# skeskinen/bert.cpp

Measured on AMD Instinct MI355X. Metric: sentences/sec (seq_len=128), higher is better.
Workload: dtype f16; 1 GPU; all-MiniLM-L6-v2 f16, batch=256 seq_len=128; per_gpu_batch=256, global_batch=256, seq_len=128, weights=f16, parallelism=dp1 (replicated weights, sharded sentences)

## Files before the change

bert.cpp_amd/csrc/engine.h:

```cpp
#pragma once
#include <hip/hip_runtime.h>

#include <cstdint>
#include <functional>
#include <memory>
#include <string>
#include <vector>

#include "kernels.h"
#include "model_file.h"
#include "options.h"
#include "profiler.h"
#include "weights.h"

namespace bert_hip {

class Engine {
public:
    static Engine *create(const ModelFile &mf, int device, std::string &err);
    ~Engine();

    int eval_packed_host(const int32_t *tokens, const int32_t *cu_seqlens, int n_sentences, float *embeddings,
                         std::string &err, float *d_embeddings = nullptr, int pool_mode = -1);
    int eval_packed_device(const int32_t *d_tokens, const int32_t *d_cu, int n_sentences, int n_tokens, int max_len,
                           float *d_out, hipStream_t stream, float *d_hidden, std::string &err,
                           const int2 *d_windows = nullptr, int n_windows = 0, int window_slots = 0,
                           int pool_mode = -1,
                           void *d_token_rows = nullptr, int token_flags = 0);
    int eval_packed_tokens_host(const int32_t *tokens, const int32_t *cu_seqlens, int n_sentences, int flags, float *rows, float *embeddings,
                                std::string &err);
    static void build_windows(const int32_t *cu_seqlens, int n_sentences, std::vector<int2> &windows, int slots);
    int eval_hidden(const int32_t *tokens, int n_tokens, float *hidden, float *embedding, std::string &err);

    int eval_packed_grouped_host(const int32_t *tokens, const int32_t *cu_seqlens, int n_sentences, const int32_t *group_cu, int n_groups,
                                 float *embeddings, float *d_embeddings, std::string &err, const float *h_raw_rows = nullptr, int pool_mode = -1);
    int eval_packed_grouped_device(const int32_t *d_tokens, const int32_t *d_cu, int n_sentences, int n_tokens, int max_len,
                                   const int32_t *d_group_cu, int n_groups, float *d_out, hipStream_t stream, std::string &err);

    bool reserve(int n_tokens, int n_sentences, std::string &err);
    int check(std::string &err);
    void set_option(const std::string &key, const std::string &value);
    void profile_enable(bool on) { prof_.enable(on); }
    std::string profile_report();
    void timed_launch(const char *name, double flops, hipStream_t s, const std::function<void()> &f);

    struct StreamOp { hipStream_t s = nullptr; hipEvent_t busy = nullptr; bool capturing = false; };
    bool op_begin(hipStream_t s, hipEvent_t busy, StreamOp &op, std::string &err);
    bool op_end(const StreamOp &op, std::string &err);

    const HParams &hparams() const { return hp_; }
    const EngineOptions &options() const { return opt_; }
    int device() const { return device_; }
    hipStream_t stream() const { return stream_; }

private:
    Engine() = default;
    bool ensure_workspace(int t_pad, int n_sentences, std::string &err);

    enum class Route { F32, LATENCY, ONE_LAUNCH, FOLDED, LAYERED };
    enum class Family { GEMM256, MFMA, NAIVE, F32 };
    struct LayerPlan {
        bool qkv2 = false;
        bool tail = false;
        bool planes = false;
        Family qkv = Family::NAIVE, o = Family::NAIVE, ffi = Family::NAIVE, ffo = Family::NAIVE;
    };
    struct Plan {
        const int32_t *tokens, *cu;
        int B, T, max_len, t_pad, slots, pool_mode;
        float *out, *hidden;
        void *token_rows;
        hipStream_t s;
        const int2 *windows;
        int n_windows;
        Route route = Route::LAYERED;
        bool build_windows = false;
        const int *n_windows_dev = nullptr;
        std::vector<LayerPlan> layers;
    };
    Plan plan(const int32_t *d_tokens, const int32_t *d_cu, int B, int T, int max_len, float *d_out, hipStream_t s, float *d_hidden,
              const int2 *d_windows, int n_windows, int slots, int pool_mode, void *d_token_rows = nullptr) const;
    bool forward_f32(const Plan &p, std::string &err);
    void forward_latency(const Plan &p);
    void forward_one_launch(const Plan &p);
    bool forward_folded(const Plan &p, std::string &err);
    bool forward_layers(const Plan &p, std::string &err);
    bool gemm(const Plan &p, const char *name, Family f, const GemmWeightStore &W, const void *A, const float *bias, const void *resid, void *C,
              int epi, std::string &err, const GemmLnFold *ln = nullptr);
    void attention(const Plan &p);
    void tap(const Plan &p, int idx);
    int group_pool(const int32_t *d_cu, int n_sentences, const int32_t *d_group_cu, int n_groups, float *d_out, int pool_mode, const StreamOp &op, std::string &err);
    template <class F> void timed(const char *name, double flops, hipStream_t s, F &&f) { prof_.timed(name, flops, s, f); }

    HParams hp_;
    int device_ = 0;
    EngineOptions opt_;
    std::unique_ptr<ModelWeights> w_;
    LaunchProfiler prof_;

    DevBuf x_, qkv_, ctx_, y_, ff_, v32_, d_tokens_, d_cu_, d_out_, d_hidden_, status_, windows_;
    DevBuf tok_in_, tok_rows_;
    DevBuf raw_rows_, group_in_, group_out_;
    DevBuf ln_stats1_, ln_stats2_, ln_rows1_, ln_rows2_;
    hipStream_t stream_ = nullptr;
    hipEvent_t busy_ = nullptr;
    struct HostSlot {
        char *h_in = nullptr, *d_in_host = nullptr;
        float *h_out = nullptr, *d_out_host = nullptr;
        size_t h_in_cap = 0, h_out_cap = 0;
        DevBuf d_in, d_out;
        hipEvent_t done = nullptr;
    } slot_[2];
};

}
```

bert.cpp_amd/csrc/engine.hip:

```cpp
#include "engine.h"

#include <algorithm>
#include <cstdio>
#include <cstdlib>
#include <chrono>
#include <cstring>
#include <system_error>
#include <thread>

namespace bert_hip {

Engine *Engine::create(const ModelFile &mf, int device, std::string &err) {
    int ndev = 0;
    if (hipGetDeviceCount(&ndev) != hipSuccess || ndev <= 0) {
        err = "no HIP device available (this library needs an AMD GPU; there is no CPU fallback)";
        return nullptr;
    }
    if (device < 0 || device >= ndev) { err = "HIP device ordinal " + std::to_string(device) + " out of range"; return nullptr; }
    std::unique_ptr<Engine> e(new Engine);
    e->hp_ = mf.hp;
    e->device_ = device;
    if (hipSetDevice(e->device_) != hipSuccess) { err = "hipSetDevice failed"; return nullptr; }
    hipDeviceProp_t prop;
    if (hipGetDeviceProperties(&prop, e->device_) != hipSuccess) { err = "hipGetDeviceProperties failed"; return nullptr; }
    if (strncmp(prop.gcnArchName, "gfx950", 6) != 0) {
        err = std::string("unsupported GPU architecture '") + prop.gcnArchName + "' (kernels are built for gfx950 / MI355X only)";
        return nullptr;
    }
    e->opt_ = EngineOptions::from_env(mf.hp);
    LoadOptions lo;
    lo.naive = e->opt_.gemm_naive; lo.expand_q4 = e->opt_.q4_expand; lo.ln_fold = e->opt_.ln_fold;
    e->w_ = ModelWeights::load(mf, lo, err);
    if (!e->w_ || !e->status_.alloc(16, err)) return nullptr;
    if (hipStreamCreateWithFlags(&e->stream_, hipStreamNonBlocking) != hipSuccess) { err = "hipStreamCreate failed"; return nullptr; }
    if (hipEventCreateWithFlags(&e->busy_, hipEventDisableTiming) != hipSuccess) { err = "hipEventCreate failed"; return nullptr; }
    return e.release();
}

Engine::~Engine() {
    (void)hipSetDevice(device_);
    (void)hipDeviceSynchronize();
    for (auto &sl : slot_) {
        if (sl.h_in) (void)hipHostFree(sl.h_in);
        if (sl.h_out) (void)hipHostFree(sl.h_out);
        if (sl.done) (void)hipEventDestroy(sl.done);
    }
    if (busy_) (void)hipEventDestroy(busy_);
    if (stream_) (void)hipStreamDestroy(stream_);
}

bool Engine::reserve(int n_tokens, int n_sentences, std::string &err) {
    HIP_OK(hipSetDevice(device_), err, false);
    if (n_tokens <= 0 || n_sentences <= 0) return true;
    return ensure_workspace((n_tokens + 255) / 256 * 256, n_sentences, err);
}

int Engine::check(std::string &err) {
    HIP_OK(hipSetDevice(device_), err, -1);
    HIP_OK(hipDeviceSynchronize(), err, -1);
    int st = 0;
    HIP_OK(hipMemcpy(&st, status_.p, sizeof(int), hipMemcpyDeviceToHost), err, -1);
    if (st) HIP_OK(hipMemset(status_.p, 0, sizeof(int)), err, -1);
    return st;
}

void Engine::set_option(const std::string &key, const std::string &value) {
    if (key == "profile_replay") { prof_.set_replay(value); return; }
    (void)hipSetDevice(device_);
    if (!test_poison_option(key, ctx_, y_, {&x_, &qkv_, &ctx_, &y_, &ff_, &v32_, &ln_stats1_, &ln_stats2_, &ln_rows1_, &ln_rows2_, &d_hidden_})) opt_.set(key, value, w_->naive_images(), w_->fold_images);
}

bool Engine::ensure_workspace(int t_pad, int n_sentences, std::string &err) {
    const size_t H = hp_.n_embd, I = hp_.n_intermediate, tp = (size_t)t_pad;
    const size_t es = w_->f32_file ? 4 : 2;
    return x_.ensure(tp * H * es, err) && qkv_.ensure(tp * 3 * H * es, err) && ctx_.ensure(tp * H * es, err) &&
           y_.ensure(tp * H * es, err) && ff_.ensure(tp * I * es, err) && v32_.ensure((size_t)std::max(128, std::min(t_pad, (opt_.latency_tokens + 255) / 256 * 256)) * H * 4, err) &&
           d_out_.ensure((size_t)n_sentences * H * 4, err) &&
           windows_.ensure((size_t)n_sentences * sizeof(int2), err) &&
           (!(H > 384 && H % 256 == 0) || (ln_stats1_.ensure(tp * (2 * H / 256) * 8, err) && ln_stats2_.ensure(tp * (2 * H / 256) * 8, err) &&
                                           ln_rows1_.ensure(tp * 16, err) && ln_rows2_.ensure(tp * 16, err)));
}

void Engine::timed_launch(const char *name, double flops, hipStream_t s, const std::function<void()> &f) { timed(name, flops, s, f); }

bool Engine::op_begin(hipStream_t s, hipEvent_t busy, StreamOp &op, std::string &err) {
    hipStreamCaptureStatus st = hipStreamCaptureStatusNone;
    HIP_OK(hipStreamIsCapturing(s, &st), err, false);
    op.s = s; op.busy = busy; op.capturing = st == hipStreamCaptureStatusActive;
    if (!op.capturing) {
        if (busy) HIP_OK(hipStreamWaitEvent(s, busy, 0), err, false);
        return true;
    }
    if (prof_.enabled()) { err = "the stream is capturing while the context profiles: a timed launch cannot be captured (bert_hip_profile_enable(ctx, 0) first)"; return false; }
    return true;
}

bool Engine::op_end(const StreamOp &op, std::string &err) {
    if (!op.capturing && op.busy) HIP_OK(hipEventRecord(op.busy, op.s), err, false);
    return true;
}

std::string Engine::profile_report() {
    (void)hipSetDevice(device_);
    (void)hipDeviceSynchronize();
    return prof_.report();
}

void Engine::build_windows(const int32_t *cu, int B, std::vector<int2> &windows, int slot) {
    windows.clear();
    int first = 0, fill = 0;
    for (int b = 0; b < B; ++b) {
        const int n = cu[b + 1] - cu[b];
        if (b > first && fill + n > 128) {
            windows.push_back(make_int2(first, b - first));
            first = b; fill = 0;
        }
        fill = (fill + n + slot - 1) & ~(slot - 1);
    }
    if (B > first) windows.push_back(make_int2(first, B - first));
}

int Engine::eval_packed_device(const int32_t *d_tokens, const int32_t *d_cu, int B, int T, int max_len, float *d_out,
                               hipStream_t s, float *d_hidden, std::string &err, const int2 *d_windows, int n_windows, int slots_in,
                               int pool_mode_in, void *d_token_rows, int token_flags) {
    if (B <= 0 || T <= 0) return 0;
    const int slots = slots_in ? slots_in : window_slots();
    const int pool_mode = pool_mode_in >= 0 ? pool_mode_in : opt_.pool_mode();
    HIP_OK(hipSetDevice(device_), err, -1);
    StreamOp op;
    if (!op_begin(s, busy_, op, err)) return -1;
    if (!ensure_workspace((T + 255) / 256 * 256, B, err)) return -1;
    prof_.begin_pass();
    if (!d_out) d_out = d_out_.as<float>();
    const Plan p = plan(d_tokens, d_cu, B, T, max_len, d_out, s, d_hidden, d_windows, n_windows, slots, pool_mode, d_token_rows);
    bool ok = true;
    if (p.route == Route::F32) ok = forward_f32(p, err);
    else {
        const int H = hp_.n_embd;
        timed("embed_ln", 0.0, s, [&] { launch_embed_ln(w_->word_emb.p, w_->type_emb.p, w_->pos_emb.p, w_->table_type, w_->ln_e_w.as<float>(), w_->ln_e_b.as<float>(),
                                                        d_tokens, d_cu, B, T, H, hp_.n_vocab, max_len, x_.as<half_t>(), s); });
        tap(p, 0);
        if (p.build_windows)
            timed("build_windows", 0.0, s, [&] { launch_build_windows(d_cu, B, windows_.as<int2>(), status_.as<int>() + 1, slots, s); });
        switch (p.route) {
            case Route::LATENCY: forward_latency(p); break;
            case Route::ONE_LAUNCH: forward_one_launch(p); break;
            case Route::FOLDED: ok = forward_folded(p, err); break;
            default: ok = forward_layers(p, err); break;
        }
        if (ok && p.route != Route::ONE_LAUNCH)
            timed("pool_normalize", 2.0 * T * H, s, [&] { launch_pool_normalize(x_.as<half_t>(), d_cu, B, H, max_len, status_.as<int>(), d_out, p.pool_mode, s); });
    }
    if (!ok) return -1;
    if (d_token_rows)
        timed("token_rows", 0.0, s, [&] { launch_token_rows(x_.p, p.route == Route::F32, T, hp_.n_embd, d_cu, B, max_len, token_flags, d_token_rows, s); });
    HIP_OK(hipGetLastError(), err, -1);
    return op_end(op, err) ? 0 : -1;
}

Engine::Plan Engine::plan(const int32_t *d_tokens, const int32_t *d_cu, int B, int T, int max_len, float *d_out, hipStream_t s,
                          float *d_hidden, const int2 *d_windows, int n_windows, int slots, int pool_mode, void *d_token_rows) const {
    Plan p{d_tokens, d_cu, B, T, max_len, (T + 255) / 256 * 256, slots, pool_mode, d_out, d_hidden, d_token_rows, s, d_windows, n_windows};
    if (w_->f32_file && opt_.f32_exact) { p.route = Route::F32; return p; }
    const int H = hp_.n_embd, nh = hp_.n_head, dh = H / nh, Lz = hp_.n_layer;
    auto family = [&](const GemmWeightStore &W) {
        if (W.mfma_ok && opt_.gemm256 && !opt_.gemm_naive && gemm256_supported(W.w, p.t_pad)) return Family::GEMM256;
        return W.mfma_ok && (!opt_.gemm_naive || !W.w.naive16) ? Family::MFMA : Family::NAIVE;
    };
    p.layers.resize(Lz);
    bool qkv2_shape0 = false, one_launch = true, fold = opt_.ln_fold && H > 384 && H % 256 == 0 && ln_rows2_.p;
    for (int il = 0; il < Lz; ++il) {
        const LayerWeights &L = w_->layers[il];
        LayerPlan &lp = p.layers[il];
        const bool qkv2_shape = qkv_attention2_supported(L.qkv.w, nh, dh, max_len), tail_shape = layer_tail_supported(L.o.w, L.ffi.w, L.ffo.w);
        if (il == 0) qkv2_shape0 = qkv2_shape;
        lp.qkv2 = opt_.qkv2 && !opt_.gemm_naive && !opt_.attn_naive && L.qkv.mfma_ok && qkv2_shape;
        lp.tail = opt_.tail && !opt_.gemm_naive && L.o.mfma_ok && L.ffi.mfma_ok && L.ffo.mfma_ok && tail_shape;
        lp.planes = L.qkv_q4.w.qs && family(L.qkv_q4) == Family::GEMM256;
        lp.qkv = family(lp.planes ? L.qkv_q4 : L.qkv), lp.o = family(L.o), lp.ffi = family(L.ffi), lp.ffo = family(L.ffo);
        one_launch = one_launch && L.qkv.mfma_ok && L.o.mfma_ok && L.ffi.mfma_ok && L.ffo.mfma_ok && L.ffi.w.w16p && L.ffo.w.w16p &&
                     model_kernel_supported(L.qkv.w, L.o.w, L.ffi.w, L.ffo.w, Lz, nh, dh, max_len);
        fold = fold && L.fold_ok && (il ? family(L.qkv_fold) : lp.qkv) == Family::GEMM256 && lp.o == Family::GEMM256 &&
               family(L.ffi_fold) == Family::GEMM256 && lp.ffo == Family::GEMM256 && !(opt_.qkv2 && qkv2_shape) && !(opt_.tail && tail_shape);
    }
    if (d_hidden) one_launch = fold = false;
    if (d_token_rows) one_launch = false;
    const bool fused_windows = p.layers[0].qkv2, latency_call = opt_.latency && T <= opt_.latency_tokens;
    one_launch = one_launch && fused_windows && opt_.one_launch && opt_.tail && !latency_call;
    const bool full_windows = (long long)B * 128 == T;
    const int spw = qkv_attention2_sentences_per_window(max_len, slots);
    if (!d_windows && fused_windows &&
        (4ll * ((B + spw - 1) / spw) * 128 > 5 * ((long long)T + (long long)(slots / 2) * B) || (one_launch && opt_.one_launch == 2 && spw > 1 && !full_windows))) {
        p.build_windows = true;
        p.windows = windows_.as<int2>();
        p.n_windows_dev = status_.as<int>() + 1;
        p.n_windows = qkv_attention2_max_windows(B, T, slots);
    }
    bool one_launch_pays = full_windows || opt_.one_launch == 2;
    if (!one_launch_pays && !p.build_windows) one_launch_pays = (d_windows || spw == 1) && 100ll * T >= 95ll * 128 * (d_windows ? n_windows : B);
    const LayerWeights &L0 = w_->layers[0];
    const bool skinny = latency_call && opt_.tail && opt_.qkv2 && !opt_.gemm_naive && !opt_.attn_naive && max_len <= 128 && (dh == 32 || dh == 64) &&
                        skinny_layer_supported(L0.qkv.w, L0.o.w, L0.ffi.w, L0.ffo.w) && qkv2_shape0;
    p.route = skinny ? Route::LATENCY : one_launch && one_launch_pays ? Route::ONE_LAUNCH : fold ? Route::FOLDED : Route::LAYERED;
    return p;
}

bool Engine::gemm(const Plan &p, const char *name, Family f, const GemmWeightStore &W, const void *A, const float *bias, const void *resid,
                  void *C, int epi, std::string &err, const GemmLnFold *ln) {
    static const char *const kernel[] = {"gemm256", "gemm_mfma", "gemm_naive", "gemm_f32"};
    prof_.count_family(std::string("family:") + kernel[(int)f] + (f == Family::GEMM256 || f == Family::MFMA ? (W.w.type == GW_F16 ? "_f16" : "_q4") : ""));
    const half_t *a = (const half_t *)A, *r = (const half_t *)resid;
    bool ok = !(ln && ln->flags) || f == Family::GEMM256;
    if (ok)
        timed(name, 2.0 * p.T * W.w.N * W.w.K, p.s, [&] {
            if (f == Family::F32) launch_f32_gemm((const float *)A, W.w.w32, bias, (const float *)resid, (float *)C, p.T, W.w.N, W.w.K, epi, p.s);
            else if (f == Family::GEMM256) ok = launch_gemm256(W.w, a, bias, r, (half_t *)C, p.t_pad, epi, p.s, ln);
            else if (f == Family::MFMA) launch_gemm_mfma(W.w, a, bias, r, (half_t *)C, p.t_pad, epi, p.s);
            else launch_gemm_naive(W.w, a, bias, r, (half_t *)C, p.T, epi, p.s);
        });
    if (!ok) err = std::string(name) + ": no " + kernel[(int)f] + " kernel for LayerNorm-folding flags " + std::to_string(ln->flags) + ", epilogue " + std::to_string(epi);
    return ok;
}

void Engine::attention(const Plan &p) {
    const int H = hp_.n_embd, nh = hp_.n_head, dh = H / nh;
    half_t *qkv = qkv_.as<half_t>(), *ctx = ctx_.as<half_t>();
    timed("attention", 4.0 * p.T * p.max_len * H, p.s, [&] {
        if (opt_.attn_naive || !launch_attention_mfma(qkv, p.cu, p.B, nh, dh, p.max_len, ctx, p.s)) launch_attention_naive(qkv, p.cu, p.B, nh, dh, p.max_len, ctx, p.s);
    });
}

void Engine::tap(const Plan &p, int idx) {
    const size_t n = (size_t)p.T * hp_.n_embd;
    if (p.hidden && p.route == Route::F32) (void)hipMemcpyAsync(p.hidden + idx * n, x_.p, n * 4, hipMemcpyDeviceToDevice, p.s);
    else if (p.hidden) launch_f16_to_f32(x_.as<half_t>(), p.hidden + idx * n, n, p.s);
}

void Engine::forward_latency(const Plan &p) {
    const int H = hp_.n_embd, I = hp_.n_intermediate, tb = (p.T + 31) / 32, Lz = hp_.n_layer;
    half_t *x = x_.as<half_t>(), *qkv = qkv_.as<half_t>(), *ctx = ctx_.as<half_t>(), *y = y_.as<half_t>(), *ff = ff_.as<half_t>();
    float *v32 = v32_.as<float>();
    for (int il = 0; il < Lz; ++il) {
        const LayerWeights &L = w_->layers[il];
        const LayerWeights *P = il ? &w_->layers[il - 1] : nullptr;
        timed("skinny_qkv", 2.0 * p.T * 3 * H * H, p.s, [&] {
            launch_skinny_gemm(0, L.qkv.w, x, P ? v32 : nullptr, P ? P->ln_out_w.as<float>() : nullptr, P ? P->ln_out_b.as<float>() : nullptr,
                               x, L.qkv_b.as<float>(), nullptr, qkv, nullptr, tb, p.s);
        });
        attention(p);
        timed("skinny_proj", 2.0 * p.T * H * H, p.s, [&] {
            launch_skinny_gemm(1, L.o.w, ctx, nullptr, nullptr, nullptr, nullptr, L.o_b.as<float>(), x, nullptr, v32, tb, p.s);
        });
        timed("skinny_ffn_up", 2.0 * p.T * H * I, p.s, [&] {
            launch_skinny_gemm(2, L.ffi.w, nullptr, v32, L.ln_att_w.as<float>(), L.ln_att_b.as<float>(), y, L.ffi_b.as<float>(), nullptr, ff, nullptr, tb, p.s);
        });
        timed("skinny_ffn_down", 2.0 * p.T * H * I, p.s, [&] {
            launch_skinny_gemm(3, L.ffo.w, ff, nullptr, nullptr, nullptr, nullptr, L.ffo_b.as<float>(), y, nullptr, v32, tb, p.s);
        });
        if (il + 1 == Lz || p.hidden)
            timed("skinny_layernorm", 0.0, p.s, [&] { launch_skinny_layernorm(v32, L.ln_out_w.as<float>(), L.ln_out_b.as<float>(), x, tb, H, p.s); });
        tap(p, il + 1);
    }
}

void Engine::forward_one_launch(const Plan &p) {
    const int H = hp_.n_embd, I = hp_.n_intermediate;
    ModelLayerWeights mw[MODEL_MAX_LAYERS];
    for (int il = 0; il < hp_.n_layer; ++il) {
        const LayerWeights &L = w_->layers[il];
        mw[il] = {&L.qkv.w, &L.o.w, &L.ffi.w, &L.ffo.w, L.qkv_b.as<float>(), L.o_b.as<float>(), L.ln_att_w.as<float>(), L.ln_att_b.as<float>(),
                  L.ffi_b.as<float>(), L.ffo_b.as<float>(), L.ln_out_w.as<float>(), L.ln_out_b.as<float>()};
    }
    timed("model_kernel", hp_.n_layer * (2.0 * p.T * 3 * H * H + 4.0 * p.T * p.max_len * H + 2.0 * p.T * H * H + 4.0 * p.T * H * I), p.s, [&] {
        launch_model_kernel(mw, hp_.n_layer, x_.as<half_t>(), ctx_.as<half_t>(), y_.as<half_t>(), p.cu, p.B, p.T, p.windows, p.n_windows, p.n_windows_dev, hp_.n_head,
                            p.out, p.max_len, status_.as<int>(), p.pool_mode, p.slots, p.s);
    });
}

bool Engine::forward_folded(const Plan &p, std::string &err) {
    const int H = hp_.n_embd, P = 2 * H / 256;
    const Family G = Family::GEMM256;
    half_t *x = x_.as<half_t>(), *qkv = qkv_.as<half_t>(), *ctx = ctx_.as<half_t>(), *y = y_.as<half_t>(), *ff = ff_.as<half_t>();
    float2 *st1 = ln_stats1_.as<float2>(), *st2 = ln_stats2_.as<float2>();
    float4 *rows1 = ln_rows1_.as<float4>(), *rows2 = ln_rows2_.as<float4>();
    for (int il = 0; il < hp_.n_layer; ++il) {
        const LayerWeights &L = w_->layers[il];
        GemmLnFold ln;
        if (il == 0) {
            if (!gemm(p, "gemm_qkv", G, p.layers[0].planes ? L.qkv_q4 : L.qkv, x, L.qkv_b.as<float>(), nullptr, qkv, EPI_BIAS, err)) return false;
        } else {
            ln.flags = GemmLnFold::IN; ln.rows_in = rows2; ln.waug = L.qkv_waug.as<half_t>();
            if (!gemm(p, "gemm_qkv", G, L.qkv_fold, x, nullptr, nullptr, qkv, EPI_BIAS, err, &ln)) return false;
        }
        attention(p);
        ln = GemmLnFold(); ln.flags = GemmLnFold::STATS | (il ? GemmLnFold::RES : 0); ln.stats = st1; ln.rows_res = rows2; ln.gb = L.o_gb.as<unsigned>();
        if (!gemm(p, "gemm_attn_out", G, L.o, ctx, L.o_b.as<float>(), x, y, EPI_BIAS_RESID, err, &ln)) return false;
        timed("ln_rows_finalize", 0.0, p.s, [&] { launch_ln_rows_finalize(st1, P, p.t_pad, H, rows1, p.s); });
        ln = GemmLnFold(); ln.flags = GemmLnFold::IN; ln.rows_in = rows1; ln.waug = L.ffi_waug.as<half_t>();
        if (!gemm(p, "gemm_ffn_up", G, L.ffi_fold, y, nullptr, nullptr, ff, EPI_BIAS_GELU, err, &ln)) return false;
        ln = GemmLnFold(); ln.flags = GemmLnFold::STATS | GemmLnFold::RES; ln.stats = st2; ln.rows_res = rows1; ln.gb = L.ffo_gb.as<unsigned>();
        if (!gemm(p, "gemm_ffn_down", G, L.ffo, ff, L.ffo_b.as<float>(), y, x, EPI_BIAS_RESID, err, &ln)) return false;
        timed("ln_rows_finalize", 0.0, p.s, [&] { launch_ln_rows_finalize(st2, P, p.t_pad, H, rows2, p.s); });
        if (il + 1 == hp_.n_layer)
            timed("layernorm", 0.0, p.s, [&] { launch_layernorm(x, L.ln_out_w.as<float>(), L.ln_out_b.as<float>(), p.T, H, p.s); });
    }
    return true;
}

bool Engine::forward_layers(const Plan &p, std::string &err) {
    const int H = hp_.n_embd, I = hp_.n_intermediate;
    half_t *x = x_.as<half_t>(), *qkv = qkv_.as<half_t>(), *ctx = ctx_.as<half_t>(), *y = y_.as<half_t>(), *ff = ff_.as<half_t>();
    for (int il = 0; il < hp_.n_layer; ++il) {
        const LayerWeights &L = w_->layers[il];
        const LayerPlan &lp = p.layers[il];
        if (lp.qkv2) {
            timed("qkv_attention2", 2.0 * p.T * L.qkv.w.N * L.qkv.w.K + 4.0 * p.T * p.max_len * H, p.s, [&] {
                launch_qkv_attention2(L.qkv.w, x, L.qkv_b.as<float>(), p.cu, p.B, p.windows, p.n_windows, p.n_windows_dev, p.max_len, hp_.n_head, p.slots, ctx, p.s);
            });
        } else {
            if (!gemm(p, "gemm_qkv", lp.qkv, lp.planes ? L.qkv_q4 : L.qkv, x, L.qkv_b.as<float>(), nullptr, qkv, EPI_BIAS, err)) return false;
            attention(p);
        }
        if (lp.tail) {
            timed("layer_tail", 2.0 * p.T * H * H + 4.0 * p.T * H * I, p.s, [&] {
                launch_layer_tail(L.o.w, L.ffi.w, L.ffo.w, ctx, x, L.o_b.as<float>(), L.ln_att_w.as<float>(), L.ln_att_b.as<float>(), L.ffi_b.as<float>(),
                                  L.ffo_b.as<float>(), L.ln_out_w.as<float>(), L.ln_out_b.as<float>(), x, p.t_pad, p.s);
            });
        } else {
            if (!gemm(p, "gemm_attn_out", lp.o, L.o, ctx, L.o_b.as<float>(), x, y, EPI_BIAS_RESID, err)) return false;
            timed("layernorm", 0.0, p.s, [&] { launch_layernorm(y, L.ln_att_w.as<float>(), L.ln_att_b.as<float>(), p.T, H, p.s); });
            if (!gemm(p, "gemm_ffn_up", lp.ffi, L.ffi, y, L.ffi_b.as<float>(), nullptr, ff, EPI_BIAS_GELU, err) ||
                !gemm(p, "gemm_ffn_down", lp.ffo, L.ffo, ff, L.ffo_b.as<float>(), y, x, EPI_BIAS_RESID, err)) return false;
            timed("layernorm", 0.0, p.s, [&] { launch_layernorm(x, L.ln_out_w.as<float>(), L.ln_out_b.as<float>(), p.T, H, p.s); });
        }
        tap(p, il + 1);
    }
    return true;
}

bool Engine::forward_f32(const Plan &p, std::string &err) {
    const int H = hp_.n_embd, nh = hp_.n_head, dh = H / nh;
    const Family F = Family::F32;
    float *x = x_.as<float>(), *qkv = qkv_.as<float>(), *ctx = ctx_.as<float>(), *y = y_.as<float>(), *ff = ff_.as<float>();
    timed("embed_ln", 0.0, p.s, [&] {
        launch_f32_embed_ln(w_->word_emb.as<float>(), w_->type_emb.as<float>(), w_->pos_emb.as<float>(), w_->ln_e_w.as<float>(), w_->ln_e_b.as<float>(), p.tokens,
                            p.cu, p.B, p.T, H, hp_.n_vocab, p.max_len, x, p.s);
    });
    tap(p, 0);
    for (int il = 0; il < hp_.n_layer; ++il) {
        const LayerWeights &L = w_->layers[il];
        if (!gemm(p, "gemm_qkv", F, L.qkv, x, L.qkv_b.as<float>(), nullptr, qkv, EPI_BIAS, err)) return false;
        bool launched = true;
        timed("attention", 4.0 * p.T * p.max_len * H, p.s, [&] { launched = launch_f32_attention(qkv, p.cu, p.B, nh, dh, p.max_len, ctx, p.s); });
        if (!launched) {
            err = "f32 route: the attention kernel keeps the scores of max_len = " + std::to_string(p.max_len) + " keys per wave in LDS, " +
                  std::to_string(f32_attention_lds_bytes(p.max_len)) + " bytes a workgroup; this device's limit is " +
                  std::to_string(f32_attention_lds_limit()) + " bytes (set_option \"f32\" = \"f16\" selects the f16 kernels)";
            return false;
        }
        if (!gemm(p, "gemm_attn_out", F, L.o, ctx, L.o_b.as<float>(), x, y, EPI_BIAS_RESID, err)) return false;
        timed("layernorm", 0.0, p.s, [&] { launch_f32_layernorm(y, L.ln_att_w.as<float>(), L.ln_att_b.as<float>(), p.T, H, p.s); });
        if (!gemm(p, "gemm_ffn_up", F, L.ffi, y, L.ffi_b.as<float>(), nullptr, ff, EPI_BIAS_GELU, err) ||
            !gemm(p, "gemm_ffn_down", F, L.ffo, ff, L.ffo_b.as<float>(), y, x, EPI_BIAS_RESID, err)) return false;
        timed("layernorm", 0.0, p.s, [&] { launch_f32_layernorm(x, L.ln_out_w.as<float>(), L.ln_out_b.as<float>(), p.T, H, p.s); });
        tap(p, il + 1);
    }
    timed("pool_normalize", 2.0 * p.T * H, p.s, [&] { launch_f32_pool_normalize(x, p.cu, p.B, H, p.max_len, status_.as<int>(), p.out, p.pool_mode, p.s); });
    return true;
}

static bool ensure_pinned(void **p, size_t *cap, size_t need, std::string &err) {
    if (need <= *cap) return true;
    if (*p) (void)hipHostFree(*p);
    *p = nullptr; *cap = 0;
    need += need / 4;
    HIP_OK(hipHostMalloc(p, need, hipHostMallocDefault), err, false);
    *cap = need;
    return true;
}

static void copy_rows_out(float *dst, const float *src, size_t bytes) {
    constexpr size_t PART_MIN = (size_t)1 << 20;
    constexpr int MAX_PARTS = 4;
    const int parts = (int)std::min<size_t>(MAX_PARTS, bytes / PART_MIN);
    if (parts <= 1) { memcpy(dst, src, bytes); return; }
    const size_t each = (bytes / parts + 4095) & ~(size_t)4095;
    std::thread helpers[MAX_PARTS - 1];
    size_t inline_from = each;
    for (int k = 1; k < parts; ++k) {
        const size_t off = (size_t)k * each, n = std::min(each, bytes - std::min(bytes, off));
        if (n == 0) break;
        try {
            helpers[k - 1] = std::thread([=] { memcpy((char *)dst + off, (const char *)src + off, n); });
            inline_from = off + n;
        } catch (const std::system_error &) {
            break;
        }
    }
    memcpy(dst, src, std::min(each, bytes));
    if (inline_from < bytes) memcpy((char *)dst + inline_from, (const char *)src + inline_from, bytes - inline_from);
    for (auto &h : helpers)
        if (h.joinable()) h.join();
}

int Engine::eval_packed_host(const int32_t *tokens, const int32_t *cu, int B, float *embeddings, std::string &err,
                             float *d_embeddings, int pool_mode_in) {
    if (B <= 0) return 0;
#ifdef BERT_HIP_HOST_TRACE
    auto now = [] { return std::chrono::duration<double, std::milli>(std::chrono::steady_clock::now().time_since_epoch()).count(); };
    const double t_call = now();
    double t_mark = t_call;
    auto lap = [&](const char *what, size_t i) { const double t = now(); fprintf(stderr, "[host] chunk %zu %-10s %.3f ms\n", i, what, t - t_mark); t_mark = t; };
#define HOST_LAP(what, i) lap(what, i)
#else
#define HOST_LAP(what, i) do { } while (0)
#endif
    HIP_OK(hipSetDevice(device_), err, -1);
    const int H = hp_.n_embd;
    struct Chunk { int b0, b1, max_len; };
    std::vector<Chunk> chunks;
    size_t max_T = 0, max_nb = 0;
    for (int b0 = 0; b0 < B;) {
        int b1 = b0 + 1, max_len = cu[b0 + 1] - cu[b0];
        while (b1 < B && cu[b1 + 1] - cu[b0] <= opt_.chunk_tokens) { max_len = std::max(max_len, cu[b1 + 1] - cu[b1]); ++b1; }
        chunks.push_back({b0, b1, max_len});
        max_T = std::max(max_T, (size_t)(cu[b1] - cu[b0]));
        max_nb = std::max(max_nb, (size_t)(b1 - b0));
        b0 = b1;
    }
    const int n_slots = chunks.size() > 1 ? 2 : 1;
    auto pad16 = [](size_t n) { return (n + 15) & ~(size_t)15; };
    const size_t in_bytes = pad16(max_T * 4) + pad16((max_nb + 1) * 4) + pad16(max_nb * sizeof(int2));
    for (int i = 0; i < n_slots; ++i) {
        HostSlot &sl = slot_[i];
        const size_t in_cap = sl.h_in_cap;
        if (!ensure_pinned((void **)&sl.h_in, &sl.h_in_cap, in_bytes + 16, err)) return -1;
        if (sl.h_in_cap != in_cap || !sl.d_in_host) HIP_OK(hipHostGetDevicePointer((void **)&sl.d_in_host, sl.h_in, 0), err, -1);
        const size_t out_cap = sl.h_out_cap;
        if (!ensure_pinned((void **)&sl.h_out, &sl.h_out_cap, max_nb * H * 4, err)) return -1;
        if (sl.h_out_cap != out_cap || !sl.d_out_host)
            HIP_OK(hipHostGetDevicePointer((void **)&sl.d_out_host, sl.h_out, 0), err, -1);
        if (!sl.d_in.ensure(in_bytes + 16, err) || (d_embeddings && !sl.d_out.ensure(max_nb * H * 4, err))) return -1;
        if (!sl.done) HIP_OK(hipEventCreateWithFlags(&sl.done, hipEventDisableTiming), err, -1);
    }
    if (!ensure_workspace((int)((max_T + 255) / 256 * 256), (int)max_nb, err)) return -1;
    HOST_LAP("prepared", (size_t)0);

    auto unpack = [&](size_t i) -> bool {
        HostSlot &sl = slot_[i & 1];
        if (hipEventSynchronize(sl.done) != hipSuccess) { err = "hipEventSynchronize failed"; return false; }
        HOST_LAP("wait", i);
        if (!d_embeddings) {
            const size_t bytes = (size_t)(chunks[i].b1 - chunks[i].b0) * H * 4;
            if (i + 1 == chunks.size()) copy_rows_out(embeddings + (size_t)chunks[i].b0 * H, sl.h_out, bytes);
            else memcpy(embeddings + (size_t)chunks[i].b0 * H, sl.h_out, bytes);
        }
        HOST_LAP("copy-out", i);
        return true;
    };
    auto fail = [&]() { (void)hipStreamSynchronize(stream_); return -1; };
    std::vector<int2> windows;
    const int slots = window_slots();
    const int pool_mode = pool_mode_in >= 0 ? pool_mode_in : opt_.pool_mode();
    for (size_t i = 0; i < chunks.size(); ++i) {
        HostSlot &sl = slot_[i & 1];
        const int b0 = chunks[i].b0, nb = chunks[i].b1 - b0, T = cu[chunks[i].b1] - cu[b0];
        const size_t off_cu = pad16((size_t)T * 4), off_w = off_cu + pad16((size_t)(nb + 1) * 4);
        int32_t *h_cu = (int32_t *)(sl.h_in + off_cu);
        memcpy(sl.h_in, tokens + cu[b0], (size_t)T * 4);
        for (int j = 0; j <= nb; ++j) h_cu[j] = cu[b0 + j] - cu[b0];
        int n_windows = 0;
        if (chunks[i].max_len <= 128) {
            build_windows(h_cu, nb, windows, slots);
            n_windows = (int)windows.size();
            memcpy(sl.h_in + off_w, windows.data(), windows.size() * sizeof(int2));
        }
        const size_t staged = off_w + (size_t)n_windows * sizeof(int2);
        HOST_LAP("staged", i);
        if (opt_.stage_kernel && staged <= ((size_t)256 << 10)) {
            launch_stage_copy(sl.d_in_host, sl.d_in.p, staged, stream_);
        } else if (hipMemcpyAsync(sl.d_in.p, sl.h_in, staged, hipMemcpyHostToDevice, stream_) != hipSuccess) {
            err = "hipMemcpyAsync (ids) failed";
            return fail();
        }
        const char *d_in = (const char *)sl.d_in.p;
        float *out = d_embeddings ? sl.d_out.as<float>() : sl.d_out_host;
        if (eval_packed_device((const int32_t *)d_in, (const int32_t *)(d_in + off_cu), nb, T, chunks[i].max_len, out, stream_, nullptr, err,
                               n_windows ? (const int2 *)(d_in + off_w) : nullptr, n_windows, slots, pool_mode) != 0)
            return fail();
        if ((d_embeddings && hipMemcpyAsync(d_embeddings + (size_t)b0 * H, sl.d_out.p, (size_t)nb * H * 4, hipMemcpyDeviceToDevice, stream_) != hipSuccess) ||
            hipEventRecord(sl.done, stream_) != hipSuccess) {
            err = "hipMemcpyAsync (embeddings) failed";
            return fail();
        }
        HOST_LAP("queued", i);
        if (i >= 1 && !unpack(i - 1)) return fail();
    }
    if (!unpack(chunks.size() - 1)) return fail();
#undef HOST_LAP
    return 0;
}

int Engine::group_pool(const int32_t *d_cu, int B, const int32_t *d_group_cu, int n_groups, float *d_out, int pool_mode, const StreamOp &op, std::string &err) {
    const int H = hp_.n_embd;
    const hipStream_t s = op.s;
    timed("group_pool", 2.0 * B * H, s, [&] {
// ... 97 lines not shown
```

bert.cpp_amd/csrc/kernels.h:

```cpp
#pragma once
#include <hip/hip_runtime.h>
#include <hip/hip_ext.h>

#include <atomic>
#include <cstdint>
#include <thread>

namespace bert_hip {

typedef _Float16 half_t;

constexpr int GEMM_BM = 128;
constexpr int GEMM_BN = 128;
constexpr int GEMM_BK = 64;

constexpr int GRID_YZ_MAX = 65535;

enum Epilogue : int { EPI_BIAS = 0, EPI_BIAS_GELU = 1, EPI_BIAS_RESID = 2 };
enum GemmWType : int { GW_F16 = 0, GW_Q4_0 = 1, GW_Q4_1 = 2 };

struct GemmWeight {
    int N = 0, K = 0, N_pad = 0;
    int type = GW_F16;
    const half_t *w16 = nullptr;
    const uint4 *qs = nullptr;
    const void *sc = nullptr;
    const half_t *naive16 = nullptr;
    const half_t *w16p = nullptr;
    const float *w32 = nullptr;
};

void launch_gemm_mfma(const GemmWeight &W, const half_t *A, const float *bias, const half_t *resid, half_t *C,
                      int M_pad, int epilogue, hipStream_t stream);
bool gemm256_supported(const GemmWeight &W, int M_pad);
struct GemmLnFold {
    enum : int { IN = 1, RES = 2, STATS = 4 };
    int flags = 0;
    const float4 *rows_in = nullptr;
    const half_t *waug = nullptr;
    const float4 *rows_res = nullptr;
    const unsigned *gb = nullptr;
    float2 *stats = nullptr;
};
bool launch_gemm256(const GemmWeight &W, const half_t *A, const float *bias, const half_t *resid, half_t *C, int M_pad,
                    int epilogue, hipStream_t stream, const GemmLnFold *ln = nullptr);
void launch_ln_rows_finalize(const float2 *stats, int P, int T, int H, float4 *rows, hipStream_t stream);
bool layer_tail_supported(const GemmWeight &Wo, const GemmWeight &W1, const GemmWeight &W2);
void launch_layer_tail(const GemmWeight &Wo, const GemmWeight &W1, const GemmWeight &W2, const half_t *ctx, const half_t *x,
                       const float *bo, const float *g1, const float *be1, const float *b1, const float *b2,
                       const float *g2, const float *be2, half_t *out, int M_pad, hipStream_t stream);
constexpr int MODEL_MAX_LAYERS = 12;
struct ModelLayerWeights {
    const GemmWeight *Wqkv, *Wo, *W1, *W2;
    const float *bqkv, *bo, *g1, *be1, *b1, *b2, *g2, *be2;
};
bool model_kernel_supported(const GemmWeight &Wqkv, const GemmWeight &Wo, const GemmWeight &W1, const GemmWeight &W2, int n_layer,
                            int n_head, int d_head, int max_len);
void launch_model_kernel(const ModelLayerWeights *layers, int n_layer, half_t *x, half_t *ctx, half_t *xres, const int32_t *cu_seqlens, int n_sentences,
                         int n_tokens, const int2 *groups, int n_groups, const int *n_groups_dev, int n_head, float *pooled, int max_len,
                         int *status, int pool_mode, int slots, hipStream_t stream);
bool skinny_layer_supported(const GemmWeight &Wqkv, const GemmWeight &Wo, const GemmWeight &W1, const GemmWeight &W2);
void launch_skinny_gemm(int mode, const GemmWeight &W, const half_t *A, const float *V, const float *gamma, const float *beta,
                        half_t *ln_out, const float *bias, const half_t *resid, half_t *out16, float *out32, int n_token_blocks,
                        hipStream_t stream);
void launch_skinny_layernorm(const float *v, const float *gamma, const float *beta, half_t *out, int n_token_blocks, int H,
                             hipStream_t stream);
void launch_gemm_naive(const GemmWeight &W, const half_t *A, const float *bias, const half_t *resid, half_t *C,
                       int M, int epilogue, hipStream_t stream);

void launch_embed_ln(const void *word, const void *type, const void *pos, int table_type, const float *gamma,
                     const float *beta, const int32_t *tokens, const int32_t *cu_seqlens, int n_sentences, int T,
                     int H, int n_vocab, int max_len, half_t *out, hipStream_t stream);

void launch_layernorm(half_t *x, const float *gamma, const float *beta, int T, int H, hipStream_t stream);

bool launch_attention_mfma(const half_t *qkv, const int32_t *cu_seqlens, int n_sentences, int n_head, int d_head,
                           int max_len, half_t *out, hipStream_t stream);
void launch_attention_naive(const half_t *qkv, const int32_t *cu_seqlens, int n_sentences, int n_head, int d_head,
                            int max_len, half_t *out, hipStream_t stream);

bool qkv_attention2_supported(const GemmWeight &Wqkv, int n_head, int d_head, int max_len);
int qkv_attention2_sentences_per_window(int max_len, int slots);
void launch_qkv_attention2(const GemmWeight &Wqkv, const half_t *x, const float *bias, const int32_t *cu_seqlens,
                           int n_sentences, const int2 *groups, int n_groups, const int *n_groups_dev, int max_len, int n_head,
                           int slots, half_t *out, hipStream_t stream);
void launch_build_windows(const int32_t *cu_seqlens, int n_sentences, int2 *windows, int *n_windows, int slots, hipStream_t stream);
int qkv_attention2_max_windows(int n_sentences, int n_tokens, int slots);
int window_slots();
void set_window_slots(int slots);

constexpr int POOL_CLS = 1, POOL_RAW = 2;
void launch_pool_normalize(const half_t *x, const int32_t *cu_seqlens, int n_sentences, int H, int max_len, int *status,
                           float *out, int pool_mode, hipStream_t stream);

void launch_group_pool(const float *rows, const int32_t *cu_seqlens, const int32_t *group_cu, int n_sentences, int n_groups, int H,
                       bool raw, int *status, float *out, hipStream_t stream);

constexpr int TOKEN_ROWS_NORMALIZE = 1, TOKEN_ROWS_F16 = 2;
void launch_token_rows(const void *x, bool x_is_f32, int T, int H, const int32_t *cu_seqlens, int n_sentences, int max_len, int flags,
                       void *out, hipStream_t stream);

constexpr int MAXSIM_MAX_H = 1024;
struct MaxsimArgs {
    const half_t *q, *d;
    const int32_t *qcu, *dcu, *pairs;
    float *scores;
    int n_q, n_d, H, n_pairs, mode;
};
size_t maxsim_lds_bytes(int H);
void launch_maxsim(const MaxsimArgs &a, hipStream_t stream);
void launch_f32_to_f16(const float *src, half_t *dst, size_t n, hipStream_t stream);

constexpr int MAX_HIP_DEVICES = 64;
typedef std::atomic<int> DeviceFlags[MAX_HIP_DEVICES];
inline int current_device_slot() {
    int d = 0;
    (void)hipGetDevice(&d);
    return d & (MAX_HIP_DEVICES - 1);
}
inline bool first_launch_on_device(DeviceFlags &seen) {
    std::atomic<int> &f = seen[current_device_slot()];
    int expected = 0;
    if (f.load(std::memory_order_acquire) == 2) return false;
    if (f.compare_exchange_strong(expected, 1, std::memory_order_acq_rel)) return true;
    while (f.load(std::memory_order_acquire) != 2) std::this_thread::yield();
    return false;
}
inline void mark_configured(DeviceFlags &seen) { seen[current_device_slot()].store(2, std::memory_order_release); }
template <class F>
inline void configure_once(DeviceFlags &seen, F &&opt_in) {
    if (first_launch_on_device(seen)) { opt_in(); mark_configured(seen); }
}

struct LaunchTiming { hipEvent_t start, stop; int launches; };
inline thread_local LaunchTiming *tl_launch_timing = nullptr;
#define BERT_LAUNCH(kernel, grid, block, lds, stream, ...)                                                                     \
    do {                                                                                                                      \
        if (::bert_hip::tl_launch_timing) {                                                                                   \
            ++::bert_hip::tl_launch_timing->launches;                                                                         \
            hipExtLaunchKernelGGL(kernel, grid, block, lds, stream, ::bert_hip::tl_launch_timing->start,                      \
                                  ::bert_hip::tl_launch_timing->stop, 0, __VA_ARGS__);                                        \
        } else hipLaunchKernelGGL(kernel, grid, block, lds, stream, __VA_ARGS__);                                             \
    } while (0)

void launch_f32_embed_ln(const float *word, const float *type, const float *pos, const float *gamma, const float *beta, const int32_t *tokens,
                         const int32_t *cu_seqlens, int n_sentences, int T, int H, int n_vocab, int max_len, float *out, hipStream_t stream);
void launch_f32_gemm(const float *A, const float *W, const float *bias, const float *resid, float *C, int M, int N, int K, int epilogue,
                     hipStream_t stream);
size_t f32_attention_lds_bytes(int max_len);
size_t f32_attention_lds_limit();
bool launch_f32_attention(const float *qkv, const int32_t *cu_seqlens, int n_sentences, int n_head, int d_head, int max_len, float *out,
                          hipStream_t stream);
void launch_f32_layernorm(float *x, const float *gamma, const float *beta, int T, int H, hipStream_t stream);
void launch_f32_pool_normalize(const float *x, const int32_t *cu_seqlens, int n_sentences, int H, int max_len, int *status, float *out,
                               int pool_mode, hipStream_t stream);

void launch_stage_copy(const void *mapped_src, void *dst, size_t bytes, hipStream_t stream);

void launch_f16_to_f32(const half_t *src, float *dst, size_t n, hipStream_t stream);

}
```

bert.cpp_amd/csrc/layer_tail.hip:

```cpp
#include "device.h"

namespace bert_hip {

namespace {

constexpr int LT_TILE = 16384;
#ifndef LT_ABLATE
#define LT_ABLATE 0
#endif
#ifndef LT_UPRIO
#define LT_UPRIO 1
#endif
#ifndef LT_GELU_BATCH
#define LT_GELU_BATCH 0
#endif
#ifndef LT_DMA_SPLIT
#define LT_DMA_SPLIT 1
#endif
#ifndef LT_DPRIO
#define LT_DPRIO 0
#endif

#ifdef BERT_HIP_TIMELINE
static __device__ unsigned long long g_tl_tail[256 * 512];
#define LT_STAMP(sel, i) do { const int tl_i = (i); if ((sel) && tl_i < 512) g_tl_tail[(blockIdx.x & 255) * 512 + tl_i] = __builtin_readcyclecounter(); } while (0)
#ifdef LT_FINE
#define LT_STAMP_FINE(sel, i) LT_STAMP(sel, i)
#else
#define LT_STAMP_FINE(sel, i) do { } while (0)
#endif
#else
#define LT_STAMP_FINE(sel, i) do { } while (0)
#define LT_STAMP(sel, i) do { } while (0)
#endif

struct TailArgs {
    const half_t *ctx, *x;
    const half_t *wo;
    const half_t *w1p;
    const half_t *w2p;
    const uint4 *wo_qs, *w1_qs, *w2_qs;
    const void *wo_sc, *w1_sc, *w2_sc;
    const float *bo, *g1, *be1, *b1, *b2, *g2, *be2;
    half_t *out;
    int I;
};

template <int N>
__device__ __forceinline__ void wait_frags(f16x8 (&f)[4]) {
    asm volatile("s_waitcnt lgkmcnt(%4)" : "+v"(f[0]), "+v"(f[1]), "+v"(f[2]), "+v"(f[3]) : "n"(N) : "memory");
}
template <int N>
__device__ __forceinline__ void wait_lgkm() {
    asm volatile("s_waitcnt lgkmcnt(%0)" : : "n"(N) : "memory");
}
template <int VM>
__device__ __forceinline__ void close_interval(f16x8 (&f)[4]) {
    asm volatile("s_waitcnt vmcnt(%4) lgkmcnt(0)\n\ts_barrier" : "+v"(f[0]), "+v"(f[1]), "+v"(f[2]), "+v"(f[3]) : "n"(VM) : "memory");
}
template <int OFF>
__device__ __forceinline__ f16x8 frag_read(unsigned addr) {
    if (LT_ABLATE & 4) { f16x8 z = (f16x8)(_Float16)0.f; asm volatile("" : "+v"(z) : "v"(addr)); return z; }
    return lds_read_b128<true, OFF>(addr);
}

__device__ __forceinline__ void dma_m0(unsigned lds) {
    if (LT_ABLATE & 1) return;
    asm volatile("s_mov_b32 m0, %0" : : "s"(lds) : "memory");
}
template <int PIECE>
__device__ __forceinline__ void dma_piece(const char *gbase, unsigned voff) {
    if (LT_ABLATE & 1) return;
    asm volatile("global_load_lds_dwordx4 %0, %1 offset:%2" : : "v"(voff), "s"(gbase - PIECE * 1024), "n"(PIECE * 1024) : "memory");
}

__device__ __forceinline__ f32x16 mfma16(const f16x8 &a, const f16x8 &b, const f32x16 &c) {
    if (LT_ABLATE & 8) { f32x16 r = c; asm volatile("" : "+v"(r[0]) : "v"(a), "v"(b)); return r; }
    return __builtin_amdgcn_mfma_f32_32x32x16_f16(a, b, c, 0, 0, 0);
}

}

template <int NT, int WT, bool RAGGED, bool HANDOVER, bool CTXREGS = false, bool XRES_IN = false, bool XRES_OUT = false>
__device__ __forceinline__ void layer_tail_body(const TailArgs &a, char *smem, const int tok0, const int rows, const int tid,
                                                [[maybe_unused]] f16x8 (&xnext)[8 * NT], [[maybe_unused]] const f16x8 *cf = nullptr,
                                                [[maybe_unused]] half_t *xres = nullptr, const bool lane_in = false, const bool lane_out = false) {
    static_assert(!(HANDOVER && RAGGED), "a ragged window's rows are packed: its lanes are not the window phase's slots");
    static_assert(!(CTXREGS && RAGGED), "a ragged window's rows are packed: its lanes are not the attention waves' queries");
    static_assert(!((XRES_IN || XRES_OUT) && (RAGGED || WT != GW_F16)), "lane order: full windows (a pair owns its 32 rows), f16 weights");
    const bool xres_out = XRES_OUT && lane_out;
    constexpr bool Q4 = WT != GW_F16;
    constexpr int VMQ = Q4 ? 63 : 0;
    constexpr int H = 128 * NT, NBH = 2 * NT, NB = 4 * NT, NQ = 8 * NT, NYH = 4 * NT;
    constexpr int P = NT * NT;
    constexpr int NG = NT;
    constexpr int LAGT = NT + NG;
    const int I = a.I, NC = I / 64;
    const int lane = tid & 63;
    const int wave = __builtin_amdgcn_readfirstlane(tid >> 6);
    const int t = wave & 3, role = wave >> 2;
    const int l31 = lane & 31, hi = lane >> 5;
    const int tok_w = tok0 + t * 32;
    const int row_l = RAGGED ? tok0 + min(t * 32 + l31, rows - 1) : tok_w + l31;

    char *ringU = smem;
    char *ringD = smem + 3 * LT_TILE;
    char *G = smem + 6 * LT_TILE;
    float *ST = (float *)(G + 32768);
    float *cbo = ST + 8 * 64;
    float *cg1 = cbo + H, *cbe1 = cg1 + H, *cb2 = cbe1 + H, *cg2 = cb2 + H, *cbe2 = cg2 + H, *cb1 = cbe2 + H;

    {
        constexpr int NPB = 4;
        const float *const src[6] = {a.bo, a.g1, a.be1, a.b2, a.g2, a.be2};
        float pv[6];
        f32x4 bq[NPB];
#pragma unroll
        for (int k = 0; k < 6; ++k) pv[k] = tid < H ? src[k][tid] : 0.f;
#pragma unroll
        for (int k = 0; k < NPB; ++k) {
            const int i4 = (k * 512 + tid) * 4;
            bq[k] = i4 < I ? *(const f32x4 *)(a.b1 + i4) : f32x4{0.f, 0.f, 0.f, 0.f};
        }
        if (tid < H) {
#pragma unroll
            for (int k = 0; k < 6; ++k) cbo[k * H + tid] = pv[k];
        }
#pragma unroll
        for (int k = 0; k < NPB; ++k) {
            const int i4 = (k * 512 + tid) * 4;
            if (i4 < I + 128) *(f32x4 *)(cb1 + i4) = bq[k];
        }
    }
    f32x16 accp[NBH];
    f16x4 xv[NBH][4];
    if constexpr (XRES_IN) {
        char *const xb = (char *)(xres + (size_t)tok_w * H);
        const unsigned xl = (unsigned)lane * 16u;
        if (!lane_in) {
            const half_t *xr = a.x + (size_t)row_l * H + role * 64 + 4 * hi;
#pragma unroll
            for (int b = 0; b < NBH; ++b)
#pragma unroll
                for (int s = 0; s < 2; ++s) {
                    const f16x4 lo = *(const f16x4 *)(xr + (b >> 1) * 128 + (b & 1) * 32 + 16 * s), up = *(const f16x4 *)(xr + (b >> 1) * 128 + (b & 1) * 32 + 16 * s + 8);
                    f16x8 v;
#pragma unroll
                    for (int e = 0; e < 4; ++e) { v[e] = lo[e]; v[4 + e] = up[e]; }
                    *(f16x8 *)(xb + (2 * (4 * (b >> 1) + 2 * role + (b & 1)) + s) * 1024 + xl) = v;
                }
            asm volatile("s_waitcnt vmcnt(0)" ::: "memory");
        }
#pragma unroll
        for (int b = 0; b < NBH; ++b)
#pragma unroll
            for (int s = 0; s < 2; ++s) {
                const f16x8 v = *(const f16x8 *)(xb + (2 * (4 * (b >> 1) + 2 * role + (b & 1)) + s) * 1024 + xl);
#pragma unroll
                for (int e = 0; e < 4; ++e) { xv[b][2 * s][e] = v[e]; xv[b][2 * s + 1][e] = v[4 + e]; }
            }
    } else {
        const half_t *xr = a.x + (size_t)row_l * H + role * 64 + 4 * hi;
#pragma unroll
        for (int b = 0; b < NBH; ++b)
#pragma unroll
            for (int gq = 0; gq < 4; ++gq) xv[b][gq] = *(const f16x4 *)(xr + (b >> 1) * 128 + (b & 1) * 32 + 8 * gq);
    }
    f16x8 bf[NQ];
    constexpr bool CTX_LATE = CTXREGS && ctx_edge_offset(NQ) >= 6 * LT_TILE && ctx_edge_offset(NQ) + 16384 <= 6 * LT_TILE + 32768;
    if constexpr (CTXREGS) {
        static_assert(ctx_edge_offset(NQ) >= 5 * LT_TILE && ctx_edge_offset(NQ) + 16384 <= 6 * LT_TILE + 32768,
                      "the edge area: ringD's third slot or G, where the prologue's DMA and parameter writes do not reach");
#pragma unroll
        for (int q = 0; q < NQ - 4; ++q) bf[q] = cf[q];
        const char *const er = smem + ctx_edge_offset(NQ) + t * 4096 + lane * 16;
#pragma unroll
        for (int q = 0; q < (CTX_LATE ? 0 : 4); ++q) bf[NQ - 4 + q] = *(const f16x8 *)(er + q * 1024);
    } else {
        const half_t *cw = a.ctx + (size_t)row_l * H + 8 * hi;
#pragma unroll
        for (int q = 0; q < NQ; ++q) bf[q] = *(const f16x8 *)(cw + 16 * q);
    }

    auto rows_offset = [&](int pitch) __attribute__((always_inline)) {
        int ln = lane;
        asm volatile("" : "+v"(ln));
        const int ch0 = (ln & 7) ^ (ln >> 4), row = t * 32 + (ln >> 3);
        return (unsigned)(row * pitch * 2 + ch0 * 16);
    };
    const half_t *const wo = a.wo, *const w1p = a.w1p, *const w2p = a.w2p;
    auto dma128 = [&](const half_t *base, unsigned oe, int row_bytes, unsigned tile) __attribute__((always_inline)) {
        const char *b = (const char *)base;
        dma_m0(tile + (unsigned)(t * 4096));
        dma_piece<0>(b, oe);
        dma_piece<1>(b + (size_t)8 * row_bytes, oe ^ 64u);
        dma_piece<2>(b + (size_t)16 * row_bytes, oe);
        dma_piece<3>(b + (size_t)24 * row_bytes, oe ^ 64u);
    };
    const unsigned ldsU = lds_addr(ringU), ldsD = lds_addr(ringD);
    const unsigned offH = rows_offset(H);
    auto up_offset = [&]() __attribute__((always_inline)) {
        int ln = lane;
        asm volatile("" : "+v"(ln));
        return (unsigned)((t * 16 + (ln >> 4)) * H * 2 + (((ln & 15) ^ (ln >> 4)) * 16));
    };
    auto dma_up_f16 = [&](int c, int j, unsigned offU, unsigned tile) __attribute__((always_inline)) {
        const char *b = (const char *)(w1p + (size_t)c * 64 * H + j * 128);
        dma_m0(tile + (unsigned)(t * 4096));
        dma_piece<0>(b, offU);
        dma_piece<1>(b + (size_t)4 * H * 2, offU ^ 64u);
        dma_piece<2>(b + (size_t)8 * H * 2, offU ^ 128u);
        dma_piece<3>(b + (size_t)12 * H * 2, offU ^ 192u);
    };

    [[maybe_unused]] RawBlock rawA, rawB;
    auto role_thread = [&]() __attribute__((always_inline)) {
        int ln = lane;
        asm volatile("" : "+v"(ln));
        return t * 64 + ln;
    };
    auto q4_request_rows = [&](const uint4 *qs, const void *sc, int tile_index) __attribute__((always_inline)) {
        if constexpr (Q4) rawA = q4_load_block<WT>(qs, sc, (size_t)tile_index * 256 + role_thread());
    };
    auto q4_request_up = [&](int c, int j) __attribute__((always_inline)) {
        if constexpr (Q4) {
            const int tidR = role_thread(), b_hi = tidR >> 7, rem = tidR & 127;
            const size_t idx = ((size_t)((c >> 1) * (H / 64) + 2 * j + b_hi) * 128 + (c & 1) * 64) * 2 + rem;
            rawB = q4_load_block<WT>(a.w1_qs, a.w1_sc, idx);
        }
    };
    auto q4_expand_rows = [&](auto perm_tag, char *tile) __attribute__((always_inline)) {
        if constexpr (Q4) {
            const int tidR = role_thread(), row = tidR >> 1, blk = tidR & 1;
            const int o = row * 128 + (((4 * blk) ^ ((row >> 1) & 7)) << 4);
            q4_expand_block<WT, decltype(perm_tag)::value>(rawA, [&](int k) __attribute__((always_inline)) { return tile + (o ^ (k << 4)); });
        }
    };
    auto q4_expand_up = [&](char *tile) __attribute__((always_inline)) {
        if constexpr (Q4) {
            const int tidR = role_thread(), b_hi = tidR >> 7, rem = tidR & 127, r = rem >> 1, blk = rem & 1;
            const int o = r * 256 + (((4 * (2 * b_hi + blk)) ^ (r & 15)) << 4);
            q4_expand_block<WT, true>(rawB, [&](int k) __attribute__((always_inline)) { return tile + (o ^ (k << 4)); });
        }
    };
    auto dma_proj = [&](int n3, int kt, unsigned tile) __attribute__((always_inline)) {
        if constexpr (Q4) q4_request_rows(a.wo_qs, a.wo_sc, n3 * (H / 64) + kt);
        else dma128(wo + (size_t)n3 * 128 * H + kt * 64, offH, H * 2, tile);
    };
    auto dma_up = [&](int c, int j, unsigned offU, unsigned tile) __attribute__((always_inline)) {
        if constexpr (Q4) q4_request_up(c, j);
        else dma_up_f16(c, j, offU, tile);
    };

    const unsigned aR = lds_addr(ringU) + (unsigned)off64(l31, hi);
    const unsigned aUp = lds_addr(ringU) + (unsigned)(l31 * 256 + ((hi ^ (l31 & 15)) << 4));

    int slot = 0;
    [[maybe_unused]] int tl = 1;
    [[maybe_unused]] const bool tlU = tid == 0, tlD = tid == 256;
    LT_STAMP(tlU, 0);
    auto pre_close = [&]() __attribute__((always_inline)) { LT_STAMP_FINE(tlU, 128 + tl); LT_STAMP_FINE(tlD, 256 + tl); };
    auto next_slot = [&]() __attribute__((always_inline)) { slot = slot == 2 ? 0 : slot + 1; LT_STAMP(tlU, tl); ++tl; };
    auto slot_plus2 = [&]() __attribute__((always_inline)) { return slot == 0 ? 2 : slot - 1; };
    [[maybe_unused]] auto slot_plus1 = [&]() __attribute__((always_inline)) { return slot == 2 ? 0 : slot + 1; };
    using PLAIN = std::false_type; using PERMUTED = std::true_type;

    auto proj_request = [&](int p, int s) __attribute__((always_inline)) {
        const int n3 = p / NT, q = p % NT;
        if (role == 0) dma_proj(n3, 2 * q, ldsU + s * LT_TILE);
        else dma_proj(n3, 2 * q + 1, ldsD + s * LT_TILE);
    };
    proj_request(0, 0);
    q4_expand_rows(PLAIN{}, role ? ringD : ringU);
    proj_request(1, 1);
    LT_STAMP(tlU, 384);
    asm volatile("s_waitcnt vmcnt(0) lgkmcnt(0)\n\ts_barrier" ::: "memory");
    LT_STAMP(tlU, 385);
#pragma unroll
    for (int b = 0; b < NBH; ++b)
#pragma unroll
        for (int gq = 0; gq < 4; ++gq) {
            const f32x4 bv = *(const f32x4 *)(cbo + (b >> 1) * 128 + role * 64 + (b & 1) * 32 + 8 * gq + 4 * hi);
#pragma unroll
            for (int e = 0; e < 4; ++e) accp[b][4 * gq + e] = (float)xv[b][gq][e] + bv[e];
        }
#pragma unroll
    for (int b = 0; b < NBH; ++b) asm volatile("" : "+v"(accp[b]));
    if constexpr (CTXREGS) {
#pragma unroll
        for (int q = 0; q < (CTX_LATE ? NQ - 4 : NQ); ++q) asm volatile("" : "+v"(bf[q]));
    }
    [[maybe_unused]] const unsigned aEdge = CTX_LATE ? lds_addr(smem) + (unsigned)(ctx_edge_offset(NQ) + t * 4096 + lane * 16) : 0u;
    __builtin_amdgcn_s_waitcnt(0xc07f);
    static_for<P>([&](auto p_tag) __attribute__((always_inline)) {
        constexpr int p = decltype(p_tag)::value, n3 = p / NT, q = p % NT, p2 = p + 2;
        const unsigned bA = aR + (unsigned)(slot * LT_TILE + role * 8192), bB = bA + 3 * LT_TILE;
        f16x8 Fa[4], Fb[4];
        auto rd = [&](unsigned base, int g2, f16x8 (&F)[4]) __attribute__((always_inline)) {
            const unsigned a0 = base ^ (unsigned)((2 * g2) << 5), a1 = base ^ (unsigned)((2 * g2 + 1) << 5);
            F[0] = frag_read<0>(a0); F[1] = frag_read<4096>(a0);
            F[2] = frag_read<0>(a1); F[3] = frag_read<4096>(a1);
        };
        auto mm = [&](f16x8 (&F)[4], int ks) __attribute__((always_inline)) {
            accp[n3 * 2 + 0] = mfma16(F[0], bf[ks], accp[n3 * 2 + 0]);
            accp[n3 * 2 + 1] = mfma16(F[1], bf[ks], accp[n3 * 2 + 1]);
            accp[n3 * 2 + 0] = mfma16(F[2], bf[ks + 1], accp[n3 * 2 + 0]);
            accp[n3 * 2 + 1] = mfma16(F[3], bf[ks + 1], accp[n3 * 2 + 1]);
        };
        auto q4_turn = [&]() __attribute__((always_inline)) {
            if constexpr (p + 1 < P) q4_expand_rows(PLAIN{}, (role ? ringD : ringU) + slot_plus1() * LT_TILE);
            else if (role == 1) q4_expand_up(ringU + slot_plus1() * LT_TILE);
            const int s2 = slot_plus2();
            if constexpr (p2 < P) proj_request(p2, s2);
            else if (role == 1) dma_up(0, p2 - P, up_offset(), ldsU + s2 * LT_TILE);
        };
        constexpr int QW = Q4 && p + 1 < P ? 4 : 0;
        if constexpr (LT_ABLATE & 64) {
            if constexpr (Q4) q4_turn();
            else {
                const int s2 = slot_plus2();
                if constexpr (p2 < P) proj_request(p2, s2);
                else if (role == 1) dma_up(0, p2 - P, up_offset(), ldsU + s2 * LT_TILE);
            }
            pre_close();
            if (p2 < P || role == 1) dma_barrier<Q4 ? 63 : 4>(); else dma_barrier<VMQ>();
            next_slot();
            return;
        }
        rd(bA, 0, Fa);
        rd(bA, 1, Fb);
        if constexpr (!Q4) {
            const int s2 = slot_plus2();
            if constexpr (p2 < P) proj_request(p2, s2);
            else if (role == 1) dma_up(0, p2 - P, up_offset(), ldsU + s2 * LT_TILE);
        }
        wait_frags<4>(Fa);
        mm(Fa, 8 * q + 0);
        __builtin_amdgcn_sched_barrier(0);
        if constexpr (CTX_LATE && q == NT - 1) {
            bf[NQ - 4] = lds_read_b128<true, 0>(aEdge);
            bf[NQ - 3] = lds_read_b128<true, 1024>(aEdge);
        }
        rd(bB, 0, Fa);
        wait_frags<4>(Fb);
        if constexpr (CTX_LATE && q == NT - 1) { landed(bf[NQ - 4]); landed(bf[NQ - 3]); }
        mm(Fb, 8 * q + 2);
        __builtin_amdgcn_sched_barrier(0);
        if constexpr (CTX_LATE && q == NT - 1) {
            bf[NQ - 2] = lds_read_b128<true, 2048>(aEdge);
            bf[NQ - 1] = lds_read_b128<true, 3072>(aEdge);
        }
        rd(bB, 1, Fb);
        if constexpr (Q4) { q4_turn(); __builtin_amdgcn_sched_barrier(0); }
        wait_frags<4 + QW>(Fa);
        mm(Fa, 8 * q + 4);
        __builtin_amdgcn_sched_barrier(0);
        wait_frags<0>(Fb);
        if constexpr (CTX_LATE && q == NT - 1) { landed(bf[NQ - 2]); landed(bf[NQ - 1]); }
        mm(Fb, 8 * q + 6);
        __builtin_amdgcn_sched_barrier(0);
        pre_close();
        if (p2 < P || role == 1) dma_barrier<Q4 ? 63 : 4>(); else dma_barrier<VMQ>();
        next_slot();
    });

    if (role == 1) q4_expand_up(ringU + slot_plus1() * LT_TILE);
    LT_STAMP(tlU, 386); LT_STAMP(tlD, 396);
    float ln_rstd, ln_nmr;
    {
        float s1 = 0.f, s2 = 0.f;
#pragma unroll
        for (int b = 0; b < ((LT_ABLATE & 32) ? 0 : NBH); ++b)
#pragma unroll
            for (int r = 0; r < 16; ++r) { s1 += accp[b][r]; s2 = __builtin_fmaf(accp[b][r], accp[b][r], s2); }
        s1 += __shfl_xor(s1, 32);
        s2 += __shfl_xor(s2, 32);
        if (hi == 0) *(f32x2 *)(ST + wave * 64 + l31 * 2) = f32x2{s1, s2};
        LT_STAMP(tlU, 387); LT_STAMP(tlD, 397);
        asm volatile("s_waitcnt lgkmcnt(0)\n\ts_barrier" ::: "memory");
        LT_STAMP(tlU, 388);
        const f32x2 o = *(const f32x2 *)(ST + (wave ^ 4) * 64 + l31 * 2);
        s1 += o[0]; s2 += o[1];
        layernorm_scale(s1, s2, 1.0f / H, ln_rstd, ln_nmr);
    }
    auto normalise_block = [&](auto b_tag, f16x8 &y0, f16x8 &y1) __attribute__((always_inline)) {
        constexpr int b = decltype(b_tag)::value;
        const int f0 = (b >> 1) * 128 + role * 64 + (b & 1) * 32 + 4 * hi;
        if constexpr (LT_ABLATE & 32) {
#pragma unroll
            for (int e = 0; e < 8; ++e) { y0[e] = (_Float16)accp[b][e]; y1[e] = (_Float16)accp[b][8 + e]; }
            return;
        }
        f32x4 gv[4], bv[4];
#pragma unroll
        for (int gq = 0; gq < 4; ++gq) { gv[gq] = *(const f32x4 *)(cg1 + f0 + 8 * gq); bv[gq] = *(const f32x4 *)(cbe1 + f0 + 8 * gq); }
#pragma unroll
        for (int gq = 0; gq < 4; ++gq)
#pragma unroll
            for (int e = 0; e < 4; ++e) {
                const _Float16 y = (_Float16)rounded_f32(__builtin_fmaf(accp[b][4 * gq + e], gv[gq][e] * ln_rstd, __builtin_fmaf(gv[gq][e], ln_nmr, bv[gq][e])));
                if (gq < 2) y0[4 * gq + e] = y; else y1[4 * (gq - 2) + e] = y;
            }
        asm volatile("" ::: "memory");
    };
    char *const xch = ringD + t * (NYH * 1024) + lane * 16;
    LT_STAMP(tlU, 389); LT_STAMP(tlD, 399);

    auto store_rows = [&]() __attribute__((always_inline)) {
        LT_STAMP(tlU, 394);
        const char *S = smem + t * (64 * H);
        int lane = (int)__builtin_amdgcn_mbcnt_hi(~0u, __builtin_amdgcn_mbcnt_lo(~0u, 0u));
        asm volatile("" : "+v"(lane));
        half_t *ow = a.out + (size_t)tok_w * H;
        [[maybe_unused]] const __amdgpu_buffer_rsrc_t out_rows =
            __builtin_amdgcn_make_buffer_rsrc(ow, 0, max(min(rows - t * 32, 32), 0) * H * 2, 0x00020000);
#pragma unroll
        for (int st2 = 0; st2 < H / 32; ++st2) {
            const int st = 2 * st2 + role;
            const int v = st * 64 + lane, tok = v / (H / 8), c8 = v - tok * (H / 8), q = c8 >> 1, h2 = c8 & 1;
            const char *row = S + q * 1024 + h2 * 8;
            const f16x4 lo = *(const f16x4 *)(row + ((tok + 2 * q) & 63) * 16);
            const f16x4 hi4 = *(const f16x4 *)(row + ((tok + 32 + 2 * q) & 63) * 16);
            f16x8 o;
#pragma unroll
            for (int e = 0; e < 4; ++e) { o[e] = lo[e]; o[4 + e] = hi4[e]; }
            if constexpr (RAGGED) __builtin_amdgcn_raw_buffer_store_b128(__builtin_bit_cast(u32x4, o), out_rows, (tok * H + c8 * 8) * 2, 0, 0);
            else *(f16x8 *)(ow + (size_t)tok * H + c8 * 8) = o;
        }
#ifdef BERT_HIP_TIMELINE
        asm volatile("s_waitcnt vmcnt(0)" ::: "memory");
        LT_STAMP(tlU, 395);
#endif
    };

    if (role == 0) {
        f16x8 Y[NQ];
        static_for<NBH>([&](auto b_tag) __attribute__((always_inline)) {
            constexpr int b = decltype(b_tag)::value;
            normalise_block(b_tag, Y[8 * (b >> 1) + 2 * (b & 1)], Y[8 * (b >> 1) + 2 * (b & 1) + 1]);
        });
        LT_STAMP(tlU, 390);
        asm volatile("s_waitcnt lgkmcnt(0)\n\ts_barrier" ::: "memory");
        LT_STAMP(tlU, 391);
#pragma unroll
        for (int m = 0; m < NYH; ++m) Y[8 * (m >> 2) + 4 + (m & 3)] = *(const f16x8 *)(xch + m * 1024);
        __builtin_amdgcn_s_waitcnt(0xc07f);
        LT_STAMP(tlU, 392);
        f32x16 accU[2][2];
#pragma unroll
        for (int pp = 0; pp < 2; ++pp)
#pragma unroll
            for (int fb = 0; fb < 2; ++fb)
#pragma unroll
                for (int r = 0; r < 16; ++r)
                    accU[pp][fb][r] = cb1[pp * 64 + 32 * fb + (r & 3) + 8 * (r >> 2) + 4 * hi];
        __builtin_amdgcn_s_waitcnt(0xc07f);
        f16x8 Fc[4];
#pragma unroll
        for (int j = 0; j < 4; ++j) Fc[j] = (f16x8)(_Float16)0;
        const unsigned aB = lds_addr(cb1) + hi * 16;
        char *const Gw = G + t * 8192 + lane * 16;

        auto gelu_pair = [&](auto pg_tag, auto jf_tag, auto p_tag, const f32x4 &b0, const f32x4 &b1, f16x8 &o) __attribute__((always_inline)) {
            constexpr int PG = decltype(pg_tag)::value, jf = decltype(jf_tag)::value, fb = jf >> 1, s8 = 8 * (jf & 1), p = decltype(p_tag)::value;
            const float x0 = accU[PG][fb][s8 + 2 * p], x1 = accU[PG][fb][s8 + 2 * p + 1];
            if constexpr (LT_ABLATE & 2) {
                o[2 * p] = (_Float16)x0; o[2 * p + 1] = (_Float16)x1;
            } else {
                const f16x2 gv = gelu_pk16(x0, x1);
                o[2 * p] = gv[0]; o[2 * p + 1] = gv[1];
            }
            accU[PG][fb][s8 + 2 * p] = p < 2 ? b0[2 * p] : b1[2 * p - 4];
            accU[PG][fb][s8 + 2 * p + 1] = p < 2 ? b0[2 * p + 1] : b1[2 * p - 3];
            if constexpr (p == 3 && !(LT_ABLATE & 16)) *(f16x8 *)(Gw + PG * 4096 + jf * 1024) = o;
        };
        auto fstart = [](int jg) constexpr { return (4 * jg + NG - 1) / NG; };
        constexpr int MAXF = (4 + NG - 1) / NG;

        auto u_interval = [&](auto par_tag, auto j_tag, auto mma_tag, auto gelu_tag, auto carry_tag, int c) __attribute__((always_inline)) {
            constexpr int PAR = decltype(par_tag)::value, j = decltype(j_tag)::value;
            constexpr bool MMA = decltype(mma_tag)::value, GELU = decltype(gelu_tag)::value, CARRY = decltype(carry_tag)::value;
            constexpr int f0 = GELU ? fstart(j) : 0, nf = GELU ? fstart(j + 1) - fstart(j) : 0;
            constexpr int PG = PAR ^ 1;
            f16x8 Fa[4], Fb[4];
            [[maybe_unused]] const bool fine = tlU && tl >= 40 && tl < 46;
            [[maybe_unused]] const int fb0 = 402 + (tl - 40) * 10;
            LT_STAMP_FINE(fine, fb0 + 0);
            unsigned bU = aUp + (unsigned)(slot * LT_TILE);
            asm volatile("" : "+v"(bU));
            auto rd = [&](int g4, f16x8 (&F)[4]) __attribute__((always_inline)) {
                unsigned a0 = bU ^ (unsigned)((2 * g4) << 5), a1 = bU ^ (unsigned)((2 * g4 + 1) << 5);
                asm volatile("" : "+v"(a0), "+v"(a1));
                F[0] = frag_read<0>(a0); F[1] = frag_read<8192>(a0);
                F[2] = frag_read<0>(a1); F[3] = frag_read<8192>(a1);
            };
            f32x4 Bv[MAXF][2];
            if constexpr (GELU) {
                const unsigned aBc = aB + (unsigned)(c + 1) * 256u;
                static_for<nf>([&](auto k_tag) __attribute__((always_inline)) {
                    constexpr int k = decltype(k_tag)::value, jf = f0 + k, off = 4 * (32 * (jf >> 1) + 16 * (jf & 1));
                    Bv[k][0] = lds_read_b128<true, off, f32x4>(aBc);
                    Bv[k][1] = lds_read_b128<true, off + 32, f32x4>(aBc);
                });
            }
            if constexpr (MMA) { rd(0, Fa); rd(1, Fb); }
            LT_STAMP_FINE(fine, fb0 + 1);
            f16x8 og[MAXF];
            auto gslot = [](int q) constexpr { return LT_GELU_BATCH ? 7 + 4 * (q / 4) : 4 + (q * 12) / (4 * (nf > 0 ? nf : 1)); };
            auto fill = [&](auto slot_tag) __attribute__((always_inline)) {
                constexpr int sl = decltype(slot_tag)::value;
                static_for<4 * nf>([&](auto q_tag) __attribute__((always_inline)) {
                    constexpr int q = decltype(q_tag)::value, k = q / 4;
                    if constexpr (gslot(q) == sl)
                        gelu_pair(std::integral_constant<int, PG>{}, std::integral_constant<int, f0 + k>{}, std::integral_constant<int, q % 4>{}, Bv[k][0], Bv[k][1], og[k]);
                });
            };
            if constexpr (CARRY) {
                constexpr int jp = j == 0 ? NT - 1 : j - 1, PC = j == 0 ? PAR ^ 1 : PAR;
                accU[PC][0] = mfma16(Fc[0], Y[8 * jp + 6], accU[PC][0]);
                accU[PC][1] = mfma16(Fc[1], Y[8 * jp + 6], accU[PC][1]);
                accU[PC][0] = mfma16(Fc[2], Y[8 * jp + 7], accU[PC][0]);
                accU[PC][1] = mfma16(Fc[3], Y[8 * jp + 7], accU[PC][1]);
                __builtin_amdgcn_sched_barrier(0);
                LT_STAMP_FINE(fine, fb0 + 2);
            }
            auto mm = [&](f16x8 (&F)[4], auto g4_tag) __attribute__((always_inline)) {
                constexpr int g4 = decltype(g4_tag)::value, sb = 4 + 4 * g4;
                accU[PAR][0] = mfma16(F[0], Y[8 * j + 2 * g4], accU[PAR][0]);
                fill(std::integral_constant<int, sb + 0>{});
                accU[PAR][1] = mfma16(F[1], Y[8 * j + 2 * g4], accU[PAR][1]);
                fill(std::integral_constant<int, sb + 1>{});
                accU[PAR][0] = mfma16(F[2], Y[8 * j + 2 * g4 + 1], accU[PAR][0]);
                fill(std::integral_constant<int, sb + 2>{});
                accU[PAR][1] = mfma16(F[3], Y[8 * j + 2 * g4 + 1], accU[PAR][1]);
                fill(std::integral_constant<int, sb + 3>{});
                __builtin_amdgcn_sched_barrier(0);
            };
            auto bias_landed = [&]() __attribute__((always_inline)) {
                static_for<nf>([&](auto k_tag) __attribute__((always_inline)) { landed(Bv[decltype(k_tag)::value][0]); landed(Bv[decltype(k_tag)::value][1]); });
            };
            using I0 = std::integral_constant<int, 0>; using I1 = std::integral_constant<int, 1>; using I2 = std::integral_constant<int, 2>;
            if constexpr (MMA) {
                wait_frags<4>(Fa);
                bias_landed();
                LT_STAMP_FINE(fine, fb0 + 3);
                mm(Fa, I0{});
                LT_STAMP_FINE(fine, fb0 + 4);
                rd(2, Fa);
                wait_frags<4>(Fb);
                LT_STAMP_FINE(fine, fb0 + 5);
                mm(Fb, I1{});
                LT_STAMP_FINE(fine, fb0 + 6);
                rd(3, Fc);
                wait_frags<4>(Fa);
                LT_STAMP_FINE(fine, fb0 + 7);
                mm(Fa, I2{});
                LT_STAMP_FINE(fine, fb0 + 8);
            } else {
                wait_lgkm<0>();
                bias_landed();
                static_for<12>([&](auto s_tag) __attribute__((always_inline)) { fill(std::integral_constant<int, 4 + decltype(s_tag)::value>{}); });
            }
            static_assert(MAXF <= 2, "two GELU batches per interval at most");
            pre_close();
            if constexpr (MMA) close_interval<VMQ>(Fc); else dma_barrier<VMQ>();
            next_slot();
        };
        using TT = std::true_type; using FF = std::false_type;
        LT_STAMP(tlU, 393);
        __builtin_amdgcn_s_setprio(LT_UPRIO);
        auto u_chunk = [&](auto par_tag, auto first_tag, int c) __attribute__((always_inline)) {
            constexpr bool FIRST = decltype(first_tag)::value;
            static_for<NT>([&](auto j_tag) __attribute__((always_inline)) {
                constexpr int j = decltype(j_tag)::value;
                constexpr bool carry = !(FIRST && j == 0), gelu = !FIRST && j < NG;
                u_interval(par_tag, j_tag, TT{}, std::integral_constant<bool, gelu>{}, std::integral_constant<bool, carry>{}, c);
            });
        };
        u_chunk(std::integral_constant<int, 0>{}, TT{}, 0);
        for (int c = 1; c + 1 < NC; c += 2) {
            u_chunk(std::integral_constant<int, 1>{}, FF{}, c);
            u_chunk(std::integral_constant<int, 0>{}, FF{}, c + 1);
        }
        u_chunk(std::integral_constant<int, 1>{}, FF{}, NC - 1);
        static_for<LAGT>([&](auto k_tag) __attribute__((always_inline)) {
            constexpr int k = decltype(k_tag)::value;
            if constexpr (k < NG)
                u_interval(std::integral_constant<int, 0>{}, std::integral_constant<int, k>{}, FF{}, TT{}, std::integral_constant<bool, k == 0>{}, NC);
            else {
                if constexpr (k == NG) {
                    char *const xu = ringU + t * (NYH * 1024) + lane * 16;
#pragma unroll
                    for (int m = 0; m < NYH; ++m) *(f16x8 *)(xu + m * 1024) = Y[8 * (m >> 2) + (m & 3)];
                }
                pre_close(); dma_barrier<VMQ>(); next_slot();
            }
        });
        static_assert(LAGT > NG, "U needs an idle interval to hand its half of y over");
        if (!xres_out) {
            asm volatile("s_barrier" ::: "memory");
            asm volatile("s_barrier" ::: "memory");
            store_rows();
        }
        if constexpr (HANDOVER) {
#pragma unroll
            for (int q = 0; q < NQ; ++q) asm volatile("" : "=v"(xnext[q]));
        }
        return;
    } else {
        f16x8 yh[NYH];
        static_for<NBH>([&](auto b_tag) __attribute__((always_inline)) {
            constexpr int b = decltype(b_tag)::value;
            normalise_block(b_tag, yh[2 * b], yh[2 * b + 1]);
            *(f16x8 *)(xch + (2 * b) * 1024) = yh[2 * b];
            *(f16x8 *)(xch + (2 * b + 1) * 1024) = yh[2 * b + 1];
        });
        LT_STAMP(tlD, 400);
        asm volatile("s_waitcnt lgkmcnt(0)\n\ts_barrier" ::: "memory");
        f32x16 acc2[NB];
        static_for<NBH>([&](auto b_tag) __attribute__((always_inline)) {
            constexpr int b = decltype(b_tag)::value, n3 = b >> 1, obp = b & 1;
            f32x4 bu[4], bd[4];
#pragma unroll
            for (int gq = 0; gq < 4; ++gq) {
                bu[gq] = *(const f32x4 *)(cb2 + n3 * 128 + obp * 32 + 8 * gq + 4 * hi);
                bd[gq] = *(const f32x4 *)(cb2 + n3 * 128 + 64 + obp * 32 + 8 * gq + 4 * hi);
            }
#pragma unroll
            for (int gq = 0; gq < 4; ++gq)
#pragma unroll
                for (int e = 0; e < 4; ++e) {
                    acc2[4 * n3 + obp][4 * gq + e] = bu[gq][e];
                    acc2[4 * n3 + 2 + obp][4 * gq + e] = (float)yh[2 * b + (gq >> 1)][4 * (gq & 1) + e] + bd[gq][e];
                }
            asm volatile("" ::: "memory");
        });
        __builtin_amdgcn_s_waitcnt(0xc07f);
        const unsigned aD = aR + 3 * LT_TILE;
        const unsigned offI = rows_offset(I);
        auto dma_down = [&](int c, int n3, unsigned tile) __attribute__((always_inline)) {
            if constexpr (Q4) q4_request_rows(a.w2_qs, a.w2_sc, n3 * (I / 64) + c);
            else dma128(w2p + (size_t)n3 * 128 * I + c * 64, offI, I * 2, tile);
        };
        const unsigned aG = lds_addr(G) + (unsigned)(t * 8192 + lane * 16);
        const unsigned offU = up_offset();
        const int NUP = NC * NT;
        auto request = [&](auto up_tag, auto down_tag, int iu, int id) __attribute__((always_inline)) {
            const int s2 = slot_plus2();
            if constexpr (decltype(up_tag)::value) dma_up(iu / NT, iu % NT, offU, ldsU + s2 * LT_TILE);
            if constexpr (decltype(down_tag)::value) dma_down(id / NT, id % NT, ldsD + s2 * LT_TILE);
        };
        using TT = std::true_type; using FF = std::false_type;
        if (LT_DPRIO) __builtin_amdgcn_s_setprio(LT_DPRIO);
        static_for<LAGT>([&](auto k_tag) __attribute__((always_inline)) {
            constexpr int k = decltype(k_tag)::value;
// ... 239 lines not shown
```

bert.cpp_amd/csrc/misc_kernels.hip:

```cpp
#include "device.h"
#include "pool_normalize.h"

#include <algorithm>

namespace bert_hip {

__device__ __forceinline__ float table_elem(const void *tab, int type, int H, int r, int e) {
    if (type == 0) return ((const float *)tab)[(size_t)r * H + e];
    if (type == 1) return (float)((const half_t *)tab)[(size_t)r * H + e];
    const int bs = type == 2 ? 18 : 20;
    const unsigned char *blk = (const unsigned char *)tab + ((size_t)r * (H / 32) + e / 32) * bs;
    const int i = e & 31;
    const float d = (float)*(const half_t *)blk;
    const unsigned char byte = blk[(type == 2 ? 2 : 4) + (i & 15)];
    const int q = i < 16 ? (byte & 0x0F) : (byte >> 4);
    if (type == 2) return (float)(q - 8) * d;
    const float m = (float)*(const half_t *)(blk + 2);
    return (float)q * d + m;
}

__device__ __forceinline__ void table_pair(const void *tab, int type, int H, int r, int e, float &a, float &b) {
    if (type == 0) {
        const float2 v = *(const float2 *)((const float *)tab + (size_t)r * H + e);
        a = v.x; b = v.y;
    } else if (type == 1) {
        const f16x2 v = *(const f16x2 *)((const half_t *)tab + (size_t)r * H + e);
        a = (float)v[0]; b = (float)v[1];
    } else {
        a = table_elem(tab, type, H, r, e);
        b = table_elem(tab, type, H, r, e + 1);
    }
}

template <int NJ>
__global__ __launch_bounds__(256) void embed_ln_kernel(const void *word, const void *type, const void *pos,
                                                       int table_type, const float *gamma, const float *beta,
                                                       const int32_t *__restrict__ tokens,
                                                       const int32_t *__restrict__ cu_seqlens, int n_sentences,
                                                       int T, int H, int n_vocab, int max_len, half_t *__restrict__ out) {
    const int t = blockIdx.x * 4 + __builtin_amdgcn_readfirstlane(threadIdx.x >> 6), lane = threadIdx.x & 63;
    if (t >= T) return;
    int lo = 0, hi = n_sentences;
    while (hi - lo > 1) {
        const int mid = (lo + hi) >> 1;
        if (cu_seqlens[mid] <= t) lo = mid; else hi = mid;
    }
    const int p = min(t - cu_seqlens[lo], max_len - 1);
    int id = tokens[t];
    id = id < 0 ? 0 : (id >= n_vocab ? n_vocab - 1 : id);

    float v[NJ][2];
    float sum = 0.f;
#pragma unroll
    for (int j = 0; j < NJ; ++j) {
        const int e = 2 * lane + 128 * j;
        v[j][0] = v[j][1] = 0.f;
        if (e < H) {
            float w0, w1, t0, t1, p0, p1;
            table_pair(word, table_type, H, id, e, w0, w1);
            table_pair(type, table_type, H, 0, e, t0, t1);
            table_pair(pos, table_type, H, p, e, p0, p1);
            v[j][0] = p0 + (t0 + w0);
            v[j][1] = p1 + (t1 + w1);
            sum += v[j][0] + v[j][1];
        }
    }
    const float mean = wave_sum_f32(sum) / H;
    float sq = 0.f;
#pragma unroll
    for (int j = 0; j < NJ; ++j) {
        const int e = 2 * lane + 128 * j;
        if (e < H) {
            v[j][0] -= mean; v[j][1] -= mean;
            sq += v[j][0] * v[j][0] + v[j][1] * v[j][1];
        }
    }
    const float rstd = 1.0f / sqrtf(wave_sum_f32(sq) / H + 1e-5f);
#pragma unroll
    for (int j = 0; j < NJ; ++j) {
        const int e = 2 * lane + 128 * j;
        if (e < H) {
            f16x2 o;
            o[0] = (_Float16)(gamma[e] * (v[j][0] * rstd) + beta[e]);
            o[1] = (_Float16)(gamma[e + 1] * (v[j][1] * rstd) + beta[e + 1]);
            *(f16x2 *)(out + (size_t)t * H + e) = o;
        }
    }
}

template <int TT>
__device__ __forceinline__ void table_run8(const void *tab, int H, int r, int e0, float (&v)[8]) {
    if (TT == 0) {
        const float4 a = *(const float4 *)((const float *)tab + (size_t)r * H + e0);
        const float4 b = *(const float4 *)((const float *)tab + (size_t)r * H + e0 + 4);
        v[0] = a.x; v[1] = a.y; v[2] = a.z; v[3] = a.w; v[4] = b.x; v[5] = b.y; v[6] = b.z; v[7] = b.w;
    } else if (TT == 1) {
        const f16x8 h = *(const f16x8 *)((const half_t *)tab + (size_t)r * H + e0);
#pragma unroll
        for (int i = 0; i < 8; ++i) v[i] = (float)h[i];
    } else {
        constexpr int bs = TT == 2 ? 18 : 20, qo = TT == 2 ? 2 : 4;
        const unsigned char *blk = (const unsigned char *)tab + ((size_t)r * (H / 32) + (e0 >> 5)) * bs;
        const int off = e0 & 31;
        const float d = (float)*(const half_t *)blk;
        const float m = TT == 3 ? (float)*(const half_t *)(blk + 2) : 0.f;
        unsigned short q16[4];
#pragma unroll
        for (int i = 0; i < 4; ++i) q16[i] = *(const unsigned short *)(blk + qo + (off & 15) + 2 * i);
#pragma unroll
        for (int i = 0; i < 8; ++i) {
            const int byte = (q16[i >> 1] >> (8 * (i & 1))) & 0xff, q = off < 16 ? (byte & 0x0F) : (byte >> 4);
            v[i] = TT == 2 ? (float)(q - 8) * d : (float)q * d + m;
        }
    }
}
template <int TT, int NC, bool SEARCH>
__global__ __launch_bounds__(256) void embed_ln_rows_kernel(const void *word, const void *type, const void *pos,
                                                            const float *__restrict__ gamma, const float *__restrict__ beta,
                                                            const int32_t *__restrict__ tokens,
                                                            const int32_t *__restrict__ cu_seqlens, int n_sentences, int T,
                                                            int H, int n_vocab, int max_len, half_t *__restrict__ out) {
    const int lane = threadIdx.x & 63;
    int p = blockIdx.x * 4 + __builtin_amdgcn_readfirstlane(threadIdx.x >> 6);
    int t;
    if constexpr (SEARCH) {
        t = p;
        if (t >= T) return;
        int lo = 0, hi = n_sentences;
        while (hi - lo > 1) {
            const int mid = (lo + hi) >> 1;
            if (cu_seqlens[mid] <= t) lo = mid; else hi = mid;
        }
        p = t - cu_seqlens[lo];
    } else {
        const int b = blockIdx.y;
        const int tok0 = cu_seqlens[b], n = cu_seqlens[b + 1] - tok0;
        if (p >= n) return;
        t = tok0 + p;
    }
    p = min(p, max_len - 1);
    int id = tokens[t];
    id = id < 0 ? 0 : (id >= n_vocab ? n_vocab - 1 : id);
    float v[NC][8];
    float sum = 0.f;
#pragma unroll
    for (int j = 0; j < NC; ++j) {
        const int e0 = 8 * (lane + 64 * j);
#pragma unroll
        for (int i = 0; i < 8; ++i) v[j][i] = 0.f;
        if (e0 < H) {
            float w[8], ty[8], ps[8];
            table_run8<TT>(word, H, id, e0, w);
            table_run8<TT>(type, H, 0, e0, ty);
            table_run8<TT>(pos, H, p, e0, ps);
#pragma unroll
            for (int i = 0; i < 8; ++i) { v[j][i] = ps[i] + (ty[i] + w[i]); sum += v[j][i]; }
        }
    }
    const float mean = wave_sum_f32(sum) / H;
    float sq = 0.f;
#pragma unroll
    for (int j = 0; j < NC; ++j)
        if (8 * (lane + 64 * j) < H)
#pragma unroll
            for (int i = 0; i < 8; ++i) { v[j][i] -= mean; sq += v[j][i] * v[j][i]; }
    const float rstd = 1.0f / sqrtf(wave_sum_f32(sq) / H + 1e-5f);
#pragma unroll
    for (int j = 0; j < NC; ++j) {
        const int e0 = 8 * (lane + 64 * j);
        if (e0 < H) {
            const float4 g0 = *(const float4 *)(gamma + e0), g1 = *(const float4 *)(gamma + e0 + 4);
            const float4 b0 = *(const float4 *)(beta + e0), b1 = *(const float4 *)(beta + e0 + 4);
            const float gg[8] = {g0.x, g0.y, g0.z, g0.w, g1.x, g1.y, g1.z, g1.w};
            const float bb[8] = {b0.x, b0.y, b0.z, b0.w, b1.x, b1.y, b1.z, b1.w};
            f16x8 o;
#pragma unroll
            for (int i = 0; i < 8; ++i) o[i] = (_Float16)(gg[i] * (v[j][i] * rstd) + bb[i]);
            *(f16x8 *)(out + (size_t)t * H + e0) = o;
        }
    }
}

void launch_embed_ln(const void *word, const void *type, const void *pos, int table_type, const float *gamma,
                     const float *beta, const int32_t *tokens, const int32_t *cu_seqlens, int n_sentences, int T,
                     int H, int n_vocab, int max_len, half_t *out, hipStream_t stream) {
    if (T <= 0) return;
    if ((table_type <= 1 ? H % 8 == 0 : H % 32 == 0) && table_type <= 3 && H <= 1024 && max_len > 0) {
        const bool search = n_sentences > GRID_YZ_MAX || 2ll * ((max_len + 3) / 4) * n_sentences > 3ll * ((T + 3) / 4);
        const dim3 g2 = search ? dim3((T + 3) / 4) : dim3((max_len + 3) / 4, n_sentences), b2(256);
#define EMBR(TT, NC) do { \
            if (search) BERT_LAUNCH((embed_ln_rows_kernel<TT, NC, true>), g2, b2, 0, stream, word, type, pos, gamma, beta, tokens, \
                                           cu_seqlens, n_sentences, T, H, n_vocab, max_len, out); \
            else BERT_LAUNCH((embed_ln_rows_kernel<TT, NC, false>), g2, b2, 0, stream, word, type, pos, gamma, beta, tokens, \
                                    cu_seqlens, n_sentences, T, H, n_vocab, max_len, out); } while (0)
        if (table_type == 0) { if (H <= 512) EMBR(0, 1); else EMBR(0, 2); }
        else if (table_type == 1) { if (H <= 512) EMBR(1, 1); else EMBR(1, 2); }
        else if (table_type == 2) { if (H <= 512) EMBR(2, 1); else EMBR(2, 2); }
        else { if (H <= 512) EMBR(3, 1); else EMBR(3, 2); }
#undef EMBR
        return;
    }
    const dim3 grid((T + 3) / 4), block(256);
    const int nj = (H + 127) / 128;
    const int pos_rows = max_len > 0 ? max_len : T;
#define EMB(NJ) BERT_LAUNCH(embed_ln_kernel<NJ>, grid, block, 0, stream, word, type, pos, table_type, gamma, \
                                   beta, tokens, cu_seqlens, n_sentences, T, H, n_vocab, pos_rows, out)
    if (nj <= 1) EMB(1); else if (nj <= 3) EMB(3); else if (nj <= 6) EMB(6); else if (nj <= 8) EMB(8); else EMB(32);
#undef EMB
}

template <int NJ>
__global__ __launch_bounds__(256) void layernorm_kernel(half_t *x, const float *gamma, const float *beta, int T, int H) {
    const int t = blockIdx.x * 4 + (threadIdx.x >> 6), lane = threadIdx.x & 63;
    if (t >= T) return;
    half_t *row = x + (size_t)t * H;
    float v[NJ][2];
    float sum = 0.f;
#pragma unroll
    for (int j = 0; j < NJ; ++j) {
        const int e = 2 * lane + 128 * j;
        if (e < H) {
            const f16x2 h2 = *(const f16x2 *)(row + e);
            v[j][0] = (float)h2[0]; v[j][1] = (float)h2[1];
        } else { v[j][0] = 0.f; v[j][1] = 0.f; }
        sum += v[j][0] + v[j][1];
    }
    const float mean = wave_sum_f32(sum) / H;
    float sq = 0.f;
#pragma unroll
    for (int j = 0; j < NJ; ++j) {
        const int e = 2 * lane + 128 * j;
        if (e < H) {
            v[j][0] -= mean; v[j][1] -= mean;
            sq += v[j][0] * v[j][0] + v[j][1] * v[j][1];
        }
    }
    const float rstd = 1.0f / sqrtf(wave_sum_f32(sq) / H + 1e-5f);
#pragma unroll
    for (int j = 0; j < NJ; ++j) {
        const int e = 2 * lane + 128 * j;
        if (e < H) {
            f16x2 o;
            o[0] = (_Float16)(gamma[e] * (v[j][0] * rstd) + beta[e]);
            o[1] = (_Float16)(gamma[e + 1] * (v[j][1] * rstd) + beta[e + 1]);
            *(f16x2 *)(row + e) = o;
        }
    }
}

template <int NC>
__global__ __launch_bounds__(256) void layernorm_rows_kernel(half_t *x, const float *__restrict__ gamma,
                                                             const float *__restrict__ beta, int T, int H) {
    const int t = blockIdx.x * 4 + (threadIdx.x >> 6), lane = threadIdx.x & 63;
    if (t >= T) return;
    half_t *row = x + (size_t)t * H;
    f16x8 h[NC];
#pragma unroll
    for (int j = 0; j < NC; ++j) {
        const int e0 = 8 * (lane + 64 * j);
#pragma unroll
        for (int i = 0; i < 8; ++i) h[j][i] = (_Float16)0.f;
        if (e0 < H) h[j] = *(const f16x8 *)(row + e0);
    }
    float v[NC][8];
    float sum = 0.f;
#pragma unroll
    for (int j = 0; j < NC; ++j)
#pragma unroll
        for (int i = 0; i < 8; ++i) { v[j][i] = (float)h[j][i]; sum += v[j][i]; }
    const float mean = wave_sum_f32(sum) / H;
    float sq = 0.f;
#pragma unroll
    for (int j = 0; j < NC; ++j)
        if (8 * (lane + 64 * j) < H)
#pragma unroll
            for (int i = 0; i < 8; ++i) { v[j][i] -= mean; sq += v[j][i] * v[j][i]; }
    const float rstd = 1.0f / sqrtf(wave_sum_f32(sq) / H + 1e-5f);
#pragma unroll
    for (int j = 0; j < NC; ++j) {
        const int e0 = 8 * (lane + 64 * j);
        if (e0 < H) {
            const float4 g0 = *(const float4 *)(gamma + e0), g1 = *(const float4 *)(gamma + e0 + 4);
            const float4 b0 = *(const float4 *)(beta + e0), b1 = *(const float4 *)(beta + e0 + 4);
            const float gg[8] = {g0.x, g0.y, g0.z, g0.w, g1.x, g1.y, g1.z, g1.w};
            const float bb[8] = {b0.x, b0.y, b0.z, b0.w, b1.x, b1.y, b1.z, b1.w};
            f16x8 o;
#pragma unroll
            for (int i = 0; i < 8; ++i) o[i] = (_Float16)(gg[i] * (v[j][i] * rstd) + bb[i]);
            *(f16x8 *)(row + e0) = o;
        }
    }
}

void launch_layernorm(half_t *x, const float *gamma, const float *beta, int T, int H, hipStream_t stream) {
    if (T <= 0) return;
    if (H % 8 == 0 && H <= 2048) {
        const dim3 grid((T + 3) / 4), block(256);
        if (H <= 512) BERT_LAUNCH(layernorm_rows_kernel<1>, grid, block, 0, stream, x, gamma, beta, T, H);
        else if (H <= 1024) BERT_LAUNCH(layernorm_rows_kernel<2>, grid, block, 0, stream, x, gamma, beta, T, H);
        else BERT_LAUNCH(layernorm_rows_kernel<4>, grid, block, 0, stream, x, gamma, beta, T, H);
        return;
    }
    const dim3 grid((T + 3) / 4), block(256);
    const int nj = (H + 127) / 128;
    if (nj <= 1) BERT_LAUNCH(layernorm_kernel<1>, grid, block, 0, stream, x, gamma, beta, T, H);
    else if (nj <= 3) BERT_LAUNCH(layernorm_kernel<3>, grid, block, 0, stream, x, gamma, beta, T, H);
    else if (nj <= 6) BERT_LAUNCH(layernorm_kernel<6>, grid, block, 0, stream, x, gamma, beta, T, H);
    else if (nj <= 8) BERT_LAUNCH(layernorm_kernel<8>, grid, block, 0, stream, x, gamma, beta, T, H);
    else BERT_LAUNCH(layernorm_kernel<32>, grid, block, 0, stream, x, gamma, beta, T, H);
}

__global__ __launch_bounds__(256) void ln_rows_finalize_kernel(const float2 *__restrict__ stats, int P, int T, float inv_h, float4 *__restrict__ rows) {
    const int t = blockIdx.x * 256 + threadIdx.x;
    if (t >= T) return;
    float s1 = 0.f, s2 = 0.f;
    for (int p = 0; p < P; ++p) { const float2 v = stats[(size_t)t * P + p]; s1 += v.x; s2 += v.y; }
    const float mean = s1 * inv_h, var = fmaxf(s2 * inv_h - mean * mean, 0.f) + 1e-5f;
    const float sd = sqrtf(var), rstd = 1.0f / sd;
    rows[t] = make_float4(rstd, -mean * rstd, -mean, sd);
}

void launch_ln_rows_finalize(const float2 *stats, int P, int T, int H, float4 *rows, hipStream_t stream) {
    if (T <= 0) return;
    BERT_LAUNCH(ln_rows_finalize_kernel, dim3((T + 255) / 256), dim3(256), 0, stream, stats, P, T, 1.0f / H, rows);
}

__global__ __launch_bounds__(256) void pool_normalize_kernel(const half_t *x, const int32_t *cu_seqlens, int H,
                                                             int max_len, int *status, float *out, int pool_mode) {
    extern __shared__ float part[];
    const int b = blockIdx.x;
    const int tok0 = cu_seqlens[b], n = cu_seqlens[b + 1] - tok0;
    pool_normalize_sentence(x, tok0, n, b, H, max_len, status, out, part, (int)threadIdx.x, true, pool_mode);
}

void launch_pool_normalize(const half_t *x, const int32_t *cu_seqlens, int n_sentences, int H, int max_len, int *status,
                           float *out, int pool_mode, hipStream_t stream) {
    if (n_sentences <= 0) return;
    BERT_LAUNCH(pool_normalize_kernel, dim3(n_sentences), dim3(256), (4 * H + 4) * sizeof(float), stream, x,
                       cu_seqlens, H, max_len, status, out, pool_mode);
}

template <bool RAW>
__global__ __launch_bounds__(256) void group_pool_kernel(const float *__restrict__ rows, const int32_t *__restrict__ cu_seqlens,
                                                         const int32_t *__restrict__ group_cu, int n_sentences, int H, int *status,
                                                         float *out) {
    __shared__ float red[4];
    const int g = blockIdx.x, tid = threadIdx.x;
    const int s0 = group_cu[g], s1 = group_cu[g + 1];
    float *o = out + (size_t)g * H;
    if (s0 < 0 || s1 <= s0 || s1 > n_sentences) {
        for (int e = tid; e < H; e += 256) o[e] = __builtin_nanf("");
        if (tid == 0 && status) atomicOr(status, 1);
        return;
    }
    const bool one = s1 - s0 == 1;
    float inv = 0.f;
    if (!one) {
        int wsum = s1 - s0;
        if (cu_seqlens) wsum = cu_seqlens[s1] - cu_seqlens[s0];
        inv = 1.0f / (float)wsum;
    }
    float sq = 0.f;
    for (int e = tid; e < H; e += 256) {
        float a;
        if (one) a = rows[(size_t)s0 * H + e];
        else {
            float acc = 0.f;
            for (int s = s0; s < s1; ++s) {
                const int w = cu_seqlens ? cu_seqlens[s + 1] - cu_seqlens[s] : 1;
                acc = fmaf((float)w, rows[(size_t)s * H + e], acc);
            }
            a = acc * inv;
        }
        o[e] = a;
        if constexpr (!RAW) sq += a * a;
    }
    if constexpr (!RAW) {
        sq = wave_sum_f32(sq);
        if ((tid & 63) == 0) red[tid >> 6] = sq;
        __syncthreads();
        const float scale = 1.0f / sqrtf((red[0] + red[1]) + (red[2] + red[3]));
        for (int e = tid; e < H; e += 256) o[e] = o[e] * scale;
    }
}

void launch_group_pool(const float *rows, const int32_t *cu_seqlens, const int32_t *group_cu, int n_sentences, int n_groups, int H,
                       bool raw, int *status, float *out, hipStream_t stream) {
    if (n_groups <= 0) return;
    if (raw) BERT_LAUNCH(group_pool_kernel<true>, dim3(n_groups), dim3(256), 0, stream, rows, cu_seqlens, group_cu, n_sentences, H, status, out);
    else BERT_LAUNCH(group_pool_kernel<false>, dim3(n_groups), dim3(256), 0, stream, rows, cu_seqlens, group_cu, n_sentences, H, status, out);
}

template <class S, int VW>
__device__ __forceinline__ void token_run_load(const S *p, float (&v)[VW]) {
    if constexpr (VW == 1) v[0] = (float)p[0];
    else if constexpr (std::is_same_v<S, float>) {
        const float4 a = *(const float4 *)p, b = *(const float4 *)(p + 4);
        v[0] = a.x; v[1] = a.y; v[2] = a.z; v[3] = a.w; v[4] = b.x; v[5] = b.y; v[6] = b.z; v[7] = b.w;
    } else {
        const f16x8 hv = *(const f16x8 *)p;
#pragma unroll
        for (int i = 0; i < 8; ++i) v[i] = (float)hv[i];
    }
}
template <class O, int VW>
__device__ __forceinline__ void token_run_store(O *p, const float (&v)[VW]) {
    if constexpr (VW == 1) p[0] = (O)v[0];
    else if constexpr (std::is_same_v<O, float>) {
        *(float4 *)p = make_float4(v[0], v[1], v[2], v[3]);
        *(float4 *)(p + 4) = make_float4(v[4], v[5], v[6], v[7]);
    } else {
        f16x8 hv;
#pragma unroll
        for (int i = 0; i < 8; ++i) hv[i] = (_Float16)v[i];
        *(f16x8 *)p = hv;
    }
}
template <class S, class O, int VW, bool NORM>
__global__ __launch_bounds__(256) void token_rows_kernel(const S *__restrict__ x, int T, int H, const int32_t *__restrict__ cu_seqlens,
                                                         int n_sentences, int max_len, O *__restrict__ out) {
    const int t = blockIdx.x * 4 + __builtin_amdgcn_readfirstlane(threadIdx.x >> 6), lane = threadIdx.x & 63;
    if (t >= T) return;
    int lo = 0, hi = n_sentences;
    while (hi - lo > 1) {
        const int mid = (lo + hi) >> 1;
        if (cu_seqlens[mid] <= t) lo = mid; else hi = mid;
    }
    const int n = cu_seqlens[lo + 1] - cu_seqlens[lo];
    const bool bad = n < 1 || n > max_len || t < cu_seqlens[lo] || t >= cu_seqlens[lo + 1];
    const S *row = x + (size_t)t * H;
    O *orow = out + (size_t)t * H;
    float scale = 1.f;
    if (NORM && !bad) {
        float sq = 0.f;
        for (int e0 = lane * VW; e0 < H; e0 += 64 * VW) {
            float v[VW];
            token_run_load<S, VW>(row + e0, v);
#pragma unroll
            for (int i = 0; i < VW; ++i) sq += v[i] * v[i];
        }
        scale = 1.0f / sqrtf(wave_sum_f32(sq));
    }
    for (int e0 = lane * VW; e0 < H; e0 += 64 * VW) {
        float v[VW];
        if (bad) {
#pragma unroll
            for (int i = 0; i < VW; ++i) v[i] = __builtin_nanf("");
        } else {
            token_run_load<S, VW>(row + e0, v);
            if (NORM) {
#pragma unroll
                for (int i = 0; i < VW; ++i) v[i] = v[i] * scale;
            }
        }
        token_run_store<O, VW>(orow + e0, v);
    }
}

void launch_token_rows(const void *x, bool x_is_f32, int T, int H, const int32_t *cu_seqlens, int n_sentences, int max_len, int flags,
                       void *out, hipStream_t stream) {
    if (T <= 0 || n_sentences <= 0) return;
    const dim3 grid((T + 3) / 4), block(256);
    const bool norm = flags & TOKEN_ROWS_NORMALIZE, o16 = flags & TOKEN_ROWS_F16, vec = H % 8 == 0;
#define TOKR(S, O, VW, NORM) BERT_LAUNCH((token_rows_kernel<S, O, VW, NORM>), grid, block, 0, stream, (const S *)x, T, H, cu_seqlens, n_sentences, max_len, (O *)out)
#define TOKR_N(S, O, VW) do { if (norm) TOKR(S, O, VW, true); else TOKR(S, O, VW, false); } while (0)
#define TOKR_V(S, O) do { if (vec) TOKR_N(S, O, 8); else TOKR_N(S, O, 1); } while (0)
    if (x_is_f32) { if (o16) TOKR_V(float, half_t); else TOKR_V(float, float); }
    else { if (o16) TOKR_V(half_t, half_t); else TOKR_V(half_t, float); }
#undef TOKR_V
#undef TOKR_N
#undef TOKR
}

__global__ __launch_bounds__(256) void stage_copy_kernel(const uint4 *__restrict__ src, uint4 *__restrict__ dst, int n16) {
    for (int i = blockIdx.x * 256 + threadIdx.x; i < n16; i += gridDim.x * 256) dst[i] = src[i];
}

void launch_stage_copy(const void *mapped_src, void *dst, size_t bytes, hipStream_t stream) {
    const int n16 = (int)((bytes + 15) / 16);
    if (n16 <= 0) return;
    BERT_LAUNCH(stage_copy_kernel, dim3(std::min(64, (n16 + 255) / 256)), dim3(256), 0, stream, (const uint4 *)mapped_src, (uint4 *)dst, n16);
}

__global__ void f16_to_f32_kernel(const half_t *src, float *dst, size_t n) {
    const size_t i = (size_t)blockIdx.x * 256 + threadIdx.x;
    if (i < n) dst[i] = (float)src[i];
}

void launch_f16_to_f32(const half_t *src, float *dst, size_t n, hipStream_t stream) {
    if (!n) return;
    BERT_LAUNCH(f16_to_f32_kernel, dim3((unsigned)((n + 255) / 256)), dim3(256), 0, stream, src, dst, n);
}

}
```

bert.cpp_amd/csrc/model_kernel.hip:

```cpp
#define BERT_HIP_PHASES_ONLY
#include "qkv_attention2.hip"
#include "layer_tail.hip"
#undef BERT_HIP_PHASES_ONLY
#include "pool_normalize.h"

#include <cstdlib>

namespace bert_hip {

#ifdef BERT_HIP_MODEL_TIMELINE
static __device__ unsigned long long g_tl_model[1024 * 32];
#define MK_STAMP(i) do { const int mk_i = (i); if (threadIdx.x == 0 && mk_i < 32) g_tl_model[(blockIdx.x & 1023) * 32 + mk_i] = __builtin_amdgcn_s_memrealtime(); } while (0)
#else
#define MK_STAMP(i) do { } while (0)
#endif

namespace {

struct ModelLayerArgs {
    const half_t *wqkv, *wo, *w1p, *w2p;
    const float *bqkv, *bo, *g1, *be1, *b1, *b2, *g2, *be2;
};
struct ModelArgs {
    half_t *x, *ctx;
    const int32_t *cu;
    const int2 *groups;
    const int *n_groups;
    int n_layer, n_head, n_sent, I, slot_mask;
    float *pooled;
    int *status;
    int max_len, pool_mode;
    ModelLayerArgs layer[MODEL_MAX_LAYERS];
    half_t *xres;
};

}

template <int NT, bool RAGGED, bool POOL_MODES>
__global__ __launch_bounds__(512, 2) void model_kernel(ModelArgs m) {
    extern __shared__ __attribute__((aligned(16))) char smem[];
    const int window = (int)blockIdx.x;
    int tok0 = window * 128, rows = 128, first = window, count = 1;
    if constexpr (RAGGED) {
        if (m.groups) {
            if (m.n_groups && window >= *m.n_groups) return;
            const int2 g = m.groups[window];
            first = g.x; count = g.y;
        }
        if (count <= 0 || first >= m.n_sent) return;
        tok0 = m.cu[first];
        rows = min(m.cu[first + count] - tok0, 128);
    }
    const int wave_index = __builtin_amdgcn_readfirstlane((int)threadIdx.x >> 6);
    auto thread_id = [&]() __attribute__((always_inline)) {
        int ln = (int)__builtin_amdgcn_mbcnt_hi(~0u, __builtin_amdgcn_mbcnt_lo(~0u, 0u)), w = wave_index;
        asm volatile("" : "+v"(ln), "+s"(w));
        return w * 64 + ln;
    };
    MK_STAMP(0);
    const int n_layer = rows > 0 ? m.n_layer : 0;
    auto window_phase = [&](const ModelLayerArgs &L, auto xregs_tag, const f16x8 *xf, f16x8 *cf) __attribute__((always_inline)) {
        const int tid = thread_id();
        Qkv2Args q;
        q.x = m.x; q.w = L.wqkv; q.qs = nullptr; q.sc = nullptr; q.bias = L.bqkv; q.cu = m.cu; q.groups = RAGGED ? m.groups : nullptr; q.n_groups = nullptr;
        q.out = m.ctx; q.n_head = m.n_head; q.n_sent = m.n_sent; q.spw = 1; q.slot_mask = m.slot_mask;
        qkv_attention2_body<2 * NT, NT, GW_F16, !RAGGED, decltype(xregs_tag)::value, !RAGGED>(q, smem, window, tid, xf, cf);
    };
    auto tail_phase = [&](const ModelLayerArgs &L, f16x8 (&xf)[8 * NT], const f16x8 *cf, [[maybe_unused]] const bool lane_in,
                          [[maybe_unused]] const bool lane_out) __attribute__((always_inline)) {
        const int tid = thread_id();
        TailArgs t;
        t.ctx = m.ctx; t.x = m.x; t.wo = L.wo; t.w1p = L.w1p; t.w2p = L.w2p;
        t.wo_qs = t.w1_qs = t.w2_qs = nullptr; t.wo_sc = t.w1_sc = t.w2_sc = nullptr;
        t.bo = L.bo; t.g1 = L.g1; t.be1 = L.be1; t.b1 = L.b1; t.b2 = L.b2; t.g2 = L.g2; t.be2 = L.be2; t.out = m.x; t.I = m.I;
        if constexpr (RAGGED) layer_tail_body<NT, GW_F16, true, false, false>(t, smem, tok0, rows, tid, xf, cf);
        else layer_tail_body<NT, GW_F16, false, true, true, true, true>(t, smem, tok0, rows, tid, xf, cf, m.xres, lane_in, lane_out);
    };
    auto hand_over = [&]() __attribute__((always_inline)) {
        __builtin_amdgcn_fence(__ATOMIC_RELEASE, "workgroup");
        asm volatile("s_waitcnt vmcnt(0) lgkmcnt(0)\n\ts_barrier" ::: "memory");
        __builtin_amdgcn_fence(__ATOMIC_ACQUIRE, "workgroup");
    };
    if constexpr (RAGGED) {
        for (int l = 0; l < n_layer; ++l) {
            f16x8 none[8 * NT];
            window_phase(m.layer[l], std::false_type{}, nullptr, nullptr);
            hand_over();
            MK_STAMP(1 + 2 * l);
            tail_phase(m.layer[l], none, nullptr, false, false);
            hand_over();
            MK_STAMP(2 + 2 * l);
        }
    } else {
        f16x8 cf[8 * NT];
        if (n_layer > 0) window_phase(m.layer[0], std::false_type{}, nullptr, cf);
        for (int l = 0; l < n_layer; ++l) {
            hand_over();
            MK_STAMP(1 + 2 * l);
            f16x8 xf[8 * NT];
            tail_phase(m.layer[l], xf, cf, l > 0, l + 1 < n_layer);
            hand_over();
            MK_STAMP(2 + 2 * l);
            if (l + 1 < n_layer) window_phase(m.layer[l + 1], std::true_type{}, xf, cf);
            else {
#pragma unroll
                for (int q = 0; q < 8 * NT; ++q) asm volatile("" : "=v"(cf[q]));
            }
        }
    }
    if (m.pooled) {
        const int tid = thread_id();
        for (int j = 0; j < count; ++j) {
            const int b = first + j, t0 = m.cu[b];
            int n = m.cu[b + 1] - t0;
            if (!RAGGED && (t0 != tok0 || n != 128)) n = -1;
            if constexpr (POOL_MODES) pool_normalize_sentence(m.x, t0, n, b, 128 * NT, m.max_len, m.status, m.pooled, (float *)smem, tid, tid < 256, m.pool_mode);
            else pool_normalize_sentence<false, false>(m.x, t0, n, b, 128 * NT, m.max_len, m.status, m.pooled, (float *)smem, tid, tid < 256);
            __syncthreads();
        }
    }
    MK_STAMP(1 + 2 * n_layer);
}

bool model_kernel_supported(const GemmWeight &Wqkv, const GemmWeight &Wo, const GemmWeight &W1, const GemmWeight &W2, int n_layer,
                            int n_head, int d_head, int max_len) {
    const int H = n_head * d_head;
    return n_layer <= MODEL_MAX_LAYERS && (H == 256 || H == 384) && max_len >= 1 && max_len <= 128 &&
           Wqkv.type == GW_F16 && Wo.type == GW_F16 && qkv_attention2_supported(Wqkv, n_head, d_head, max_len) && layer_tail_supported(Wo, W1, W2);
}

void launch_model_kernel(const ModelLayerWeights *layers, int n_layer, half_t *x, half_t *ctx, half_t *xres, const int32_t *cu_seqlens, int n_sentences,
                         int n_tokens, const int2 *groups, int n_groups, const int *n_groups_dev, int n_head, float *pooled, int max_len,
                         int *status, int pool_mode, int slots, hipStream_t stream) {
    ModelArgs m;
    m.pooled = pooled; m.status = status; m.max_len = max_len; m.pool_mode = pool_mode;
    m.x = x; m.ctx = ctx; m.xres = xres; m.cu = cu_seqlens; m.groups = groups; m.n_groups = n_groups_dev;
    m.n_layer = n_layer; m.n_head = n_head; m.n_sent = n_sentences; m.I = layers[0].W1->N; m.slot_mask = slots - 1;
    for (int l = 0; l < n_layer; ++l) {
        const ModelLayerWeights &s = layers[l];
        ModelLayerArgs &d = m.layer[l];
        d.wqkv = s.Wqkv->w16; d.wo = s.Wo->w16; d.w1p = s.W1->w16p; d.w2p = s.W2->w16p;
        d.bqkv = s.bqkv; d.bo = s.bo; d.g1 = s.g1; d.be1 = s.be1; d.b1 = s.b1; d.b2 = s.b2; d.g2 = s.g2; d.be2 = s.be2;
    }
    const int H = layers[0].W1->K, KT = H / 64, GB = KT / 2;
    const size_t lds_q = (size_t)3 * GB * Q2_TILE + 2 * (2 * Q2_WIN * 64 + 32 * Q2_VT_LD * 2) + (size_t)2 * H * sizeof(float);
    const size_t lds = std::max(lds_q, layer_tail_lds(H, m.I));
    const bool full = (long long)n_sentences * 128 == n_tokens;
    if (n_head * 32 != H) { fprintf(stderr, "launch_model_kernel: n_head %d x 32 != H %d\n", n_head, H); abort(); }
    const int grid = full || !groups ? n_sentences : n_groups;
    static DeviceFlags configured[8];
    auto go = [&](auto kernel, int which) {
        configure_once(configured[which], [&] { (void)hipFuncSetAttribute((const void *)kernel, hipFuncAttributeMaxDynamicSharedMemorySize, 160 * 1024); });
        BERT_LAUNCH(kernel, dim3(grid), dim3(512), lds, stream, m);
#ifdef BERT_HIP_MODEL_TIMELINE
        static int shots = 0;
        if (grid >= 256 && shots++ == 30) {
            (void)hipDeviceSynchronize();
            static unsigned long long h[1024 * 32];
            (void)hipMemcpyFromSymbol(h, HIP_SYMBOL(g_tl_model), sizeof(h));
            const int nw = grid < 1024 ? grid : 1024, ns = 2 + 2 * n_layer;
            unsigned long long t0 = ~0ull;
            for (int w = 0; w < nw; ++w) t0 = h[w * 32] < t0 ? h[w * 32] : t0;
            fprintf(stderr, "model_kernel timeline, %d workgroups (us after the first workgroup's start: min mean max):\n", nw);
            for (int i = 0; i < ns; ++i) {
                double lo = 1e30, hi = 0, sum = 0;
                for (int w = 0; w < nw; ++w) { const double v = (double)(h[w * 32 + i] - t0) * 0.01; lo = v < lo ? v : lo; hi = v > hi ? v : hi; sum += v; }
                fprintf(stderr, "  stamp %2d: %8.2f %8.2f %8.2f\n", i, lo, sum / nw, hi);
            }
            fprintf(stderr, "  mean phase durations (window, tail) per layer:");
            for (int l = 0; l < n_layer; ++l) {
                double a = 0, b = 0;
                for (int w = 0; w < nw; ++w) { a += (double)(h[w * 32 + 1 + 2 * l] - h[w * 32 + 2 * l]) * 0.01; b += (double)(h[w * 32 + 2 + 2 * l] - h[w * 32 + 1 + 2 * l]) * 0.01; }
                fprintf(stderr, " (%.1f, %.1f)", a / nw, b / nw);
            }
            fprintf(stderr, "\n  mean end per XCD:");
            for (int x = 0; x < 8; ++x) {
                double e = 0; int c = 0;
                for (int w = x; w < nw; w += 8) { e += (double)(h[w * 32 + ns - 1] - t0) * 0.01; ++c; }
                fprintf(stderr, " %.1f", e / c);
            }
            fprintf(stderr, "\n  mean end per eighth of the grid:");
            for (int x = 0; x < 8; ++x) {
                double e = 0; int c = 0;
                for (int w = x * nw / 8; w < (x + 1) * nw / 8; ++w) { e += (double)(h[w * 32 + ns - 1] - t0) * 0.01; ++c; }
                fprintf(stderr, " %.1f", e / c);
            }
            double pl = 0;
            for (int w = 0; w < nw; ++w) pl += (double)(h[w * 32 + 1 + 2 * n_layer] - h[w * 32 + 2 * n_layer]) * 0.01;
            fprintf(stderr, "; pooling %.2f\n", pl / nw);
        }
#endif
    };
    if (pool_mode == 0) {
        if (full) { if (H == 256) go(model_kernel<2, false, false>, 0); else go(model_kernel<3, false, false>, 1); }
        else { if (H == 256) go(model_kernel<2, true, false>, 2); else go(model_kernel<3, true, false>, 3); }
    } else {
        if (full) { if (H == 256) go(model_kernel<2, false, true>, 4); else go(model_kernel<3, false, true>, 5); }
        else { if (H == 256) go(model_kernel<2, true, true>, 6); else go(model_kernel<3, true, true>, 7); }
    }
}

}
```

bert.cpp_amd/csrc/qkv_attention2.hip:

```cpp
#include "device.h"

#ifndef Q2_PM
#define Q2_PM 3
#endif
#ifndef Q2_PRIO
#define Q2_PRIO 0
#endif

namespace bert_hip {

namespace {

constexpr int Q2_WIN = 128;
constexpr int Q2_TILE = 12288;
constexpr int Q2_VT_LD = Q2_WIN + 4;

struct Qkv2Args {
    const half_t *x;
    const half_t *w;
    const uint4 *qs;
    const void *sc;
    const float *bias;
    const int32_t *cu;
    const int2 *groups;
    const int *n_groups;
    half_t *out;
    int n_head, n_sent, spw;
    int slot_mask;
};

__device__ __forceinline__ int q2_off32(int row, int chunk) { return row * 64 + ((chunk ^ ((row >> 2) & 3)) << 4); }

__device__ __forceinline__ void q2_wait6(f16x8 (&f)[2][3]) {
    asm volatile("s_waitcnt lgkmcnt(6)"
                 : "+v"(f[0][0]), "+v"(f[0][1]), "+v"(f[0][2]), "+v"(f[1][0]), "+v"(f[1][1]), "+v"(f[1][2]) : : "memory");
}
template <int VM>
__device__ __forceinline__ void q2_slab_barrier(f16x8 (&f)[2][3]) {
    asm volatile("s_waitcnt vmcnt(%6) lgkmcnt(0)\n\ts_barrier"
                 : "+v"(f[0][0]), "+v"(f[0][1]), "+v"(f[0][2]), "+v"(f[1][0]), "+v"(f[1][1]), "+v"(f[1][2]) : "n"(VM) : "memory");
}
__device__ __forceinline__ void q2_wait14(f16x8 (&f)[2][3]) {
    asm volatile("s_waitcnt lgkmcnt(14)"
                 : "+v"(f[0][0]), "+v"(f[0][1]), "+v"(f[0][2]), "+v"(f[1][0]), "+v"(f[1][1]), "+v"(f[1][2]) : : "memory");
}
__device__ __forceinline__ void q2_wait0_bias(f16x8 (&f)[2][3], f32x4 (&bq)[4], f32x4 (&bk)[4]) {
    asm volatile("s_waitcnt lgkmcnt(0)"
                 : "+v"(f[0][0]), "+v"(f[0][1]), "+v"(f[0][2]), "+v"(f[1][0]), "+v"(f[1][1]), "+v"(f[1][2]),
                   "+v"(bq[0]), "+v"(bq[1]), "+v"(bq[2]), "+v"(bq[3]), "+v"(bk[0]), "+v"(bk[1]), "+v"(bk[2]), "+v"(bk[3]) : : "memory");
}

}

template <int KT, int GB, int WT, bool FULL = false, bool XREGS = false, bool CTXREGS = false>
__device__ __forceinline__ void qkv_attention2_body(const Qkv2Args &a, char *smem, const int window, const int tid,
                                                    [[maybe_unused]] const f16x8 *xf = nullptr,
                                                    [[maybe_unused]] f16x8 *cf = nullptr) {
    static_assert(FULL || !XREGS, "fragments handed over in registers: full windows only");
    static_assert(!CTXREGS || (FULL && WT == GW_F16), "the context in registers: full windows, f16 weights");
    constexpr int NCF = 4 * KT;
    constexpr bool Q4 = WT != GW_F16;
    constexpr int H = 64 * KT, NBAR = KT / GB, SLAB = GB * Q2_TILE, PPS = 3 * GB;
    static_assert(KT == 2 * GB && NBAR == 2, "");
    constexpr int QKV_BYTES = 2 * Q2_WIN * 64 + 32 * Q2_VT_LD * 2;
    char *RING = smem;
    char *QKV = smem + 3 * SLAB;
    float *BS = (float *)(QKV + 2 * QKV_BYTES);

    const int lane = tid & 63;
    const int wave = __builtin_amdgcn_readfirstlane(tid >> 6);
    const int l31 = lane & 31, hi = lane >> 5;
    const int blk = wave & 3;
    const int n_head = a.n_head;
    if constexpr (CTXREGS) {
        static_assert(NCF * 4096 <= 3 * SLAB && ctx_edge_offset(NCF) >= NCF * 4096 && ctx_edge_offset(NCF) + 16384 <= 3 * SLAB + QKV_BYTES &&
                      ((2 * KT - 1) & 1) == 1, "the context exchange does not fit the window phase's LDS map");
    }
    TL_STAMP_AT(tid == 256, 120);
    TL_REALTIME_AT(tid == 256, 121);
    TL_STAMP_AT(tid == 0, 250);
    TL_REALTIME_AT(tid == 0, 251);

    const int wp = blk;
    const unsigned loff = (unsigned)(((wp * 8 + (lane >> 3)) * H + (((lane & 7) ^ (((wp & 1) << 2) | ((lane >> 4) & 3))) * 8)) * 2);
    auto dma_piece = [&](const char *hbase, auto j_tag, int dslot, auto i_tag) __attribute__((always_inline)) {
        constexpr int i = decltype(i_tag)::value, j = decltype(j_tag)::value, t = i / 3, rb = i % 3;
        const char *src = hbase + ((size_t)rb * H * H + (size_t)(j * GB + t) * 64) * 2;
        __builtin_amdgcn_global_load_lds(AS_GLOBAL(src + loff), AS_LDS(RING + dslot * SLAB + t * Q2_TILE + rb * 4096 + wp * 1024), 16, 0, 0);
    };
    const char *const wbase = (const char *)a.w;
    if constexpr (!Q4) {
        if (wave >= 4) static_for<PPS>([&](auto i) __attribute__((always_inline)) { dma_piece(wbase, std::integral_constant<int, 0>{}, 0, i); });
    }

    int first, count;
    if constexpr (FULL) { first = window; count = 1; }
    else {
        if (a.groups) {
            if (a.n_groups && window >= *a.n_groups) {
                asm volatile("s_waitcnt vmcnt(0)" ::: "memory");
                return;
            }
            const int2 g = a.groups[window];
            first = g.x; count = g.y;
        }
        else { first = window * a.spw; count = min(a.spw, a.n_sent - first); }
        if (count <= 0) {
            asm volatile("s_waitcnt vmcnt(0)" ::: "memory");
            return;
        }
    }
    const int slot = blk * 32 + l31;
    int gtok = -1, k0 = 0, k1 = 0;
    if constexpr (FULL) { gtok = window * Q2_WIN + slot; k1 = Q2_WIN; }
    else {
        const int place = a.groups ? 128 : 128 / a.spw;
        int off = 0;
        for (int j = 0; j < count; ++j) {
            const int t0 = a.cu[first + j], n = min(a.cu[first + j + 1] - t0, place);
            if (slot >= off && slot < off + n) { gtok = t0 + slot - off; k0 = off; k1 = off + n; }
            off = (off + n + a.slot_mask) & ~a.slot_mask;
        }
    }

    if (wave >= 4) {
        f16x8 bf[4 * KT];
        if constexpr (XREGS) {
#pragma unroll
            for (int ks = 0; ks < 4 * KT; ++ks) bf[ks] = xf[ks];
        } else {
            const int gt = FULL || gtok >= 0 ? gtok : a.cu[first];
            const half_t *xr = a.x + (size_t)gt * H + 8 * hi;
#pragma unroll
            for (int ks = 0; ks < 4 * KT; ++ks) asm volatile("global_load_dwordx4 %0, %1, off" : "=v"(bf[ks]) : "v"(xr + 16 * ks));
        }
        if constexpr (!Q4) static_for<PPS>([&](auto i) __attribute__((always_inline)) { dma_piece(wbase, std::integral_constant<int, NBAR - 1>{}, 1, i); });

        constexpr int NRAW = GB;
        [[maybe_unused]] RawBlock raw[NRAW];
        auto q4_image_of_lane = [&]() __attribute__((always_inline)) {
            int ln = (int)__builtin_amdgcn_mbcnt_hi(~0u, __builtin_amdgcn_mbcnt_lo(~0u, 0u));
            asm volatile("" : "+v"(ln));
            return (ln >> 1) * 128 + (((4 * (ln & 1)) ^ ((ln >> 2) & 7)) << 4);
        };
        auto q4_rb = [&](int hq, int j, int i) __attribute__((always_inline)) { return (blk + i + 2 * hq + j) & 3; };
        auto q4_request = [&](int hq, int j, int i) __attribute__((always_inline)) {
            if constexpr (Q4) {
                const int rb = q4_rb(hq, j, i);
                if (rb == 3) return;
                const int sbase = ((rb * (H / 128) + (hq >> 2)) * (H / 64) + j * GB + i) * 256 + (hq & 3) * 64;
                raw[i] = q4_load_block<WT>(a.qs + sbase, WT == GW_Q4_0 ? (const void *)((const unsigned short *)a.sc + sbase) : (const void *)((const unsigned *)a.sc + sbase), (size_t)lane);
            }
        };
        auto q4_expand = [&](int hq, int j, int dslot, int i) __attribute__((always_inline)) {
            if constexpr (Q4) {
                const int rb = q4_rb(hq, j, i);
                if (rb == 3) return;
                char *const base = RING + dslot * SLAB + i * Q2_TILE + rb * 4096;
                const int q4_image = q4_image_of_lane();
                q4_expand_block<WT, false>(raw[i], [&](int k) __attribute__((always_inline)) { return base + (q4_image ^ (k << 4)); });
            }
        };
        if constexpr (Q4) {
            RawBlock first[2][NRAW];
#pragma unroll
            for (int j = 0; j < 2; ++j)
#pragma unroll
                for (int i = 0; i < NRAW; ++i) {
                    q4_request(0, j, i);
                    first[j][i] = raw[i];
                }
#pragma unroll
            for (int j = 0; j < 2; ++j)
#pragma unroll
                for (int i = 0; i < NRAW; ++i) {
                    raw[i] = first[j][i];
                    q4_expand(0, j, j, i);
                }
        }
        const unsigned aX0 = lds_addr(RING) + off64(l31, hi);
        unsigned aS[4];
        int rslot = 0;
        auto set_slot = [&]() __attribute__((always_inline)) {
#pragma unroll
            for (int kk = 0; kk < 4; ++kk) aS[kk] = (aX0 ^ (unsigned)(kk << 5)) + (unsigned)rslot * SLAB;
        };
        set_slot();
        f16x8 F[2][2][3];
        f32x16 acc[3];
        auto read_half = [&](auto par_tag, auto tt_tag, auto half_tag) __attribute__((always_inline)) {
            constexpr int par = decltype(par_tag)::value, tt = decltype(tt_tag)::value, half = decltype(half_tag)::value;
#pragma unroll
            for (int i = 0; i < 2; ++i) {
                F[par][i][0] = lds_read_b128<false, tt * Q2_TILE>(aS[2 * half + i]);
                F[par][i][1] = lds_read_b128<false, tt * Q2_TILE + 4096>(aS[2 * half + i]);
                F[par][i][2] = lds_read_b128<false, tt * Q2_TILE + 8192>(aS[2 * half + i]);
            }
        };
        [[maybe_unused]] const bool tl_sel = tid == 256;
        TL_STAMP_AT(tl_sel, 0);
        asm volatile("s_waitcnt vmcnt(%0) lgkmcnt(0)\n\ts_barrier" : : "n"(Q4 ? 0 : PPS) : "memory");
#pragma unroll
        for (int ks = 0; ks < 4 * KT; ++ks) asm volatile("" : "+v"(bf[ks]));
        if constexpr (Q4) {
#pragma unroll
            for (int i = 0; i < NRAW; ++i) q4_request(min(1, n_head - 1), 0, i);
        }
        TL_STAMP_AT(tl_sel, 1);
        read_half(std::integral_constant<int, 0>{}, std::integral_constant<int, 0>{}, std::integral_constant<int, 0>{});

        const unsigned aBias = lds_addr(BS) + 16 * hi;
        for (int h = 0; h < n_head; ++h) {
            char *QS = QKV + (h & 1) * QKV_BYTES, *KS = QS + Q2_WIN * 64;
            half_t *VT = (half_t *)(KS + Q2_WIN * 64);
            float bv;
            if constexpr (Q4) bv = a.bias[2 * H + h * 32 + l31];
            else asm volatile("global_load_dword %0, %1, off" : "=v"(bv) : "v"(a.bias + 2 * H + h * 32 + l31));
            f32x4 bq[4], bk[4];
            const char *const hnext = wbase + (size_t)min(h + 1, n_head - 1) * 32 * H * 2;
#pragma unroll
            for (int m = 0; m < 3; ++m)
#pragma unroll
                for (int r = 0; r < 16; ++r) acc[m][r] = 0.f;
            constexpr int LT0 = 2 * KT - 2, LT1 = 2 * KT - 1;
            auto pieces = [&](auto hh_tag, auto m_tag) __attribute__((always_inline)) {
                constexpr int hh = decltype(hh_tag)::value, m = decltype(m_tag)::value, hs = hh % (2 * GB);
                constexpr int i0 = (3 * hs + 1) / 2, i1 = (3 * (hs + 1) + 1) / 2;
                const int dslot = (hh == 2 * GB - 1) ? (rslot == 2 ? 0 : rslot + 1) : (rslot == 0 ? 2 : rslot - 1);
                if constexpr (Q4) {
                    constexpr int j = (hh >> 1) / GB;
                    if constexpr (m == 1) {
                        if constexpr (hs < GB) { if (h + 1 < n_head) q4_expand(h + 1, j, dslot, hs); }
                        else q4_request(min(j == 0 ? h + 1 : h + 2, n_head - 1), j ^ 1, hs - GB);
                    }
                } else {
                if constexpr (m == 1) dma_piece(hnext, std::integral_constant<int, (hh >> 1) / GB>{}, dslot, std::integral_constant<int, i0>{});
                if constexpr (m == 4 && i1 - i0 == 2) dma_piece(hnext, std::integral_constant<int, (hh >> 1) / GB>{}, dslot, std::integral_constant<int, i0 + 1>{});
                }
            };
            auto mma = [&](auto par_tag, auto i_tag, auto rb_tag, auto ks_tag) __attribute__((always_inline)) {
                constexpr int par = decltype(par_tag)::value, i = decltype(i_tag)::value, rb = decltype(rb_tag)::value, ks = decltype(ks_tag)::value;
                if constexpr (rb < 2) acc[rb] = __builtin_amdgcn_mfma_f32_32x32x16_f16(F[par][i][rb], bf[ks], acc[rb], 0, 0, 0);
                else acc[2] = __builtin_amdgcn_mfma_f32_32x32x16_f16(bf[ks], F[par][i][2], acc[2], 0, 0, 0);
            };
            static_for<2 * KT>([&](auto hh_tag) __attribute__((always_inline)) {
                constexpr int hh = decltype(hh_tag)::value, par = hh & 1;
                constexpr int nhh = hh + 1, ntt = (nhh >> 1) % GB, nhalf = nhh & 1;
                using PAR = std::integral_constant<int, par>;
                if constexpr (hh == 2 * GB - 1) {
                    if (h < 8) TL_STAMP_AT(tl_sel, 2 + 6 * h);
                    q2_slab_barrier<Q4 ? 63 : PPS - 1>(F[par]);
                    if (h < 8) TL_STAMP_AT(tl_sel, 2 + 6 * h + 1);
                    landed(bv);
                    rslot = rslot == 2 ? 0 : rslot + 1;
                    set_slot();
                }
                if constexpr (hh < LT1) read_half(std::integral_constant<int, par ^ 1>{}, std::integral_constant<int, ntt>{}, std::integral_constant<int, nhalf>{});
                if constexpr (hh < LT0) {
                    q2_wait6(F[par]);
                    static_for<6>([&](auto m_tag) __attribute__((always_inline)) {
                        constexpr int m = decltype(m_tag)::value;
                        mma(PAR{}, std::integral_constant<int, m / 3>{}, std::integral_constant<int, m % 3>{}, std::integral_constant<int, 2 * hh + m / 3>{});
                        pieces(hh_tag, m_tag);
                    });
                } else if constexpr (hh == LT0) {
                    const unsigned ab = aBias + (unsigned)h * 128u;
                    bq[0] = lds_read_b128<false, 0, f32x4>(ab); bq[1] = lds_read_b128<false, 32, f32x4>(ab); bq[2] = lds_read_b128<false, 64, f32x4>(ab); bq[3] = lds_read_b128<false, 96, f32x4>(ab);
                    bk[0] = lds_read_b128<false, H * 4, f32x4>(ab); bk[1] = lds_read_b128<false, H * 4 + 32, f32x4>(ab);
                    bk[2] = lds_read_b128<false, H * 4 + 64, f32x4>(ab); bk[3] = lds_read_b128<false, H * 4 + 96, f32x4>(ab);
                    q2_wait14(F[par]);
                    static_for<6>([&](auto m_tag) __attribute__((always_inline)) {
                        constexpr int m = decltype(m_tag)::value;
                        mma(PAR{}, std::integral_constant<int, m % 2>{}, std::integral_constant<int, m / 2>{}, std::integral_constant<int, 2 * hh + m % 2>{});
                        pieces(hh_tag, m_tag);
                    });
                } else {
                    q2_wait0_bias(F[par], bq, bk);
                    static_for<2>([&](auto i) __attribute__((always_inline)) { mma(PAR{}, i, std::integral_constant<int, 0>{}, std::integral_constant<int, 2 * hh + decltype(i)::value>{}); });
                    pieces(hh_tag, std::integral_constant<int, 1>{});
                    static_for<2>([&](auto i) __attribute__((always_inline)) { mma(PAR{}, i, std::integral_constant<int, 1>{}, std::integral_constant<int, 2 * hh + decltype(i)::value>{}); });
#pragma unroll
                    for (int gg = 0; gg < 4; ++gg) {
                        f16x4 oq;
#pragma unroll
                        for (int e = 0; e < 4; ++e) oq[e] = (_Float16)(acc[0][4 * gg + e] + bq[gg][e]);
                        *(f16x4 *)(QS + q2_off32(slot, gg) + hi * 8) = oq;
                    }
                    static_for<2>([&](auto i) __attribute__((always_inline)) { mma(PAR{}, i, std::integral_constant<int, 2>{}, std::integral_constant<int, 2 * hh + decltype(i)::value>{}); });
                    pieces(hh_tag, std::integral_constant<int, 4>{});
#pragma unroll
                    for (int gg = 0; gg < 4; ++gg) {
                        f16x4 ok;
#pragma unroll
                        for (int e = 0; e < 4; ++e) ok[e] = (_Float16)(acc[1][4 * gg + e] + bk[gg][e]);
                        *(f16x4 *)(KS + q2_off32(slot, gg) + hi * 8) = ok;
                    }
#pragma unroll
                    for (int gg = 0; gg < 4; ++gg) {
                        f16x4 ov;
#pragma unroll
                        for (int e = 0; e < 4; ++e) ov[e] = (_Float16)(acc[2][4 * gg + e] + bv);
                        *(f16x4 *)(VT + l31 * Q2_VT_LD + blk * 32 + 8 * gg + 4 * hi) = ov;
                    }
                }
            });
            if (h < 8) TL_STAMP_AT(tl_sel, 2 + 6 * h + 4);
            if constexpr (CTXREGS) {
                if (h + 1 == n_head) dma_barrier<0>(); else dma_barrier<PPS>();
            } else
            dma_barrier<Q4 ? 63 : PPS>();
            if (h < 8) TL_STAMP_AT(tl_sel, 2 + 6 * h + 5);
            if constexpr (CTXREGS) {
                if (h + 1 < n_head) {
                    rslot = rslot == 2 ? 0 : rslot + 1;
                    set_slot();
                    read_half(std::integral_constant<int, 0>{}, std::integral_constant<int, 0>{}, std::integral_constant<int, 0>{});
                }
            } else {
            rslot = rslot == 2 ? 0 : rslot + 1;
            set_slot();
            read_half(std::integral_constant<int, 0>{}, std::integral_constant<int, 0>{}, std::integral_constant<int, 0>{});
            }
        }
        TL_STAMP_AT(tl_sel, 60);
        if constexpr (!CTXREGS) asm volatile("s_waitcnt vmcnt(0)" ::: "memory");
        if constexpr (CTXREGS) {
            asm volatile("s_waitcnt lgkmcnt(0)\n\ts_barrier" ::: "memory");
            const char *const xr = smem + blk * (NCF * 1024) + lane * 16;
#pragma unroll
            for (int q = 0; q < NCF - 4; ++q) cf[q] = *(const f16x8 *)(xr + q * 1024);
            __builtin_amdgcn_s_waitcnt(0xc07f);
        }
    } else {
        unsigned need = 0, inner = 0;
#pragma unroll
        for (int kt = 0; kt < 4; ++kt) {
            const bool nd = gtok >= 0 && k0 < 32 * kt + 32 && k1 > 32 * kt;
            const bool in = gtok < 0 || (k0 <= 32 * kt && k1 >= 32 * kt + 32);
            if (__any(nd)) need |= 1u << kt;
            if (__all(in)) inner |= 1u << kt;
        }
        need = __builtin_amdgcn_readfirstlane(need);
        inner = __builtin_amdgcn_readfirstlane(inner);
        const unsigned klen = (unsigned)(k1 - k0);
        const int kbase = 4 * hi - k0;
        const float sc = 1.44269504088896340736f / __builtin_sqrtf(32.0f);
        for (int i = tid; i < 2 * H; i += 256) BS[i] = a.bias[i];
        asm volatile("s_waitcnt vmcnt(0) lgkmcnt(0)\n\ts_barrier" ::: "memory");

        if constexpr (Q2_PRIO > 0) __builtin_amdgcn_s_setprio(Q2_PRIO);
        [[maybe_unused]] const bool tl_sel = tid == 0;
        if constexpr (CTXREGS) {
#pragma unroll
            for (int q = 0; q < NCF - 4; ++q) asm volatile("" : "=v"(cf[q]));
        }
        [[maybe_unused]] f16x8 pen0, pen1;
        auto attend = [&](int hh, auto wb_tag, auto fast_tag, int tb, [[maybe_unused]] auto to_tag) __attribute__((always_inline)) {
            constexpr bool WB = decltype(wb_tag)::value, FAST = decltype(fast_tag)::value;
            [[maybe_unused]] constexpr int TO = decltype(to_tag)::value;
            const char *QS = QKV + (hh & 1) * QKV_BYTES, *KS = QS + Q2_WIN * 64;
            const half_t *VT = (const half_t *)(KS + Q2_WIN * 64);
            f32x16 s[4];
            f16x8 qf[2];
#pragma unroll
            for (int kk = 0; kk < 2; ++kk) qf[kk] = *(const f16x8 *)(QS + q2_off32(slot, kk * 2 + hi));
            float mx = -INFINITY;
            int kb = kbase;
            unsigned kl = klen;
            if constexpr (!FAST) asm volatile("" : "+v"(kb), "+v"(kl));
#pragma unroll
            for (int kt = 0; kt < 4; ++kt) {
                if (FAST || (need & (1u << kt))) {
#pragma unroll
                    for (int r = 0; r < 16; ++r) s[kt][r] = 0.f;
#pragma unroll
                    for (int kk = 0; kk < 2; ++kk) {
                        const f16x8 kf = *(const f16x8 *)(KS + q2_off32(kt * 32 + l31, kk * 2 + hi));
                        s[kt] = __builtin_amdgcn_mfma_f32_32x32x16_f16(kf, qf[kk], s[kt], 0, 0, 0);
                    }
                    if (FAST || (inner & (1u << kt))) {
#pragma unroll
                        for (int r = 0; r < 16; ++r) mx = fmaxf(mx, s[kt][r]);
                    } else {
#pragma unroll
                        for (int r = 0; r < 16; ++r) {
                            const bool ok = (unsigned)(kt * 32 + (r & 3) + 8 * (r >> 2) + kb) < kl;
                            const float v = ok ? s[kt][r] : -INFINITY;
                            s[kt][r] = v;
                            mx = fmaxf(mx, v);
                        }
                    }
                }
                if constexpr (WB) {
                    if (kt == Q2_PM) {
                        if (tb < 8) TL_STAMP_AT(tl_sel, 128 + 6 * tb + 1);
                        asm volatile("s_barrier" ::: "memory");
                        if (tb < 8) TL_STAMP_AT(tl_sel, 128 + 6 * tb + 2);
                    }
                }
            }
            mx = xor32_max(mx) * sc;
            mx = fmaxf(mx, -3.0e38f);
            float psum = 0.f;
            f32x16 o;
#pragma unroll
            for (int r = 0; r < 16; ++r) o[r] = 0.f;
#pragma unroll
            for (int kt = 0; kt < 4; ++kt) {
                if (FAST || (need & (1u << kt))) {
#pragma unroll
                    for (int st = 0; st < 2; ++st) {
                        const f16x8 pf = softmax_p8(s[kt][8 * st], s[kt][8 * st + 1], s[kt][8 * st + 2], s[kt][8 * st + 3], s[kt][8 * st + 4],
                                                    s[kt][8 * st + 5], s[kt][8 * st + 6], s[kt][8 * st + 7], sc, mx, psum);
                        const int key0 = kt * 32 + 16 * st + 4 * hi;
                        const half_t *vr = VT + l31 * Q2_VT_LD + key0;
                        const f16x4 v0 = *(const f16x4 *)vr, v1 = *(const f16x4 *)(vr + 8);
                        f16x8 vf;
#pragma unroll
                        for (int e = 0; e < 4; ++e) { vf[e] = v0[e]; vf[4 + e] = v1[e]; }
                        o = __builtin_amdgcn_mfma_f32_32x32x16_f16(vf, pf, o, 0, 0, 0);
                    }
                }
                if constexpr (WB) {
                    if (kt + 4 == Q2_PM) {
                        if (tb < 8) TL_STAMP_AT(tl_sel, 128 + 6 * tb + 1);
                        asm volatile("s_barrier" ::: "memory");
                        if (tb < 8) TL_STAMP_AT(tl_sel, 128 + 6 * tb + 2);
                    }
                }
            }
            psum = xor32_sum(psum);
            if constexpr (CTXREGS) {
                const float inv = 1.0f / psum;
                f16x8 r0, r1;
#pragma unroll
                for (int e = 0; e < 8; ++e) { r0[e] = (_Float16)rounded_f32(o[e] * inv); r1[e] = (_Float16)rounded_f32(o[8 + e] * inv); }
                r0 = result_to_operand_fragment(r0);
                r1 = result_to_operand_fragment(r1);
                if constexpr (TO == 0)
                    static_for<2 * KT - 2>([&](auto i_tag) __attribute__((always_inline)) {
                        constexpr int i = decltype(i_tag)::value;
                        if (hh == i) {
                            cf[2 * i] = r0; cf[2 * i + 1] = r1;
                            asm volatile("" : "+v"(cf[2 * i]), "+v"(cf[2 * i + 1]));
                        }
                    });
                else if constexpr (TO == 1) { pen0 = r0; pen1 = r1; }
                else {
                    char *const ew = smem + ctx_edge_offset(NCF) + blk * 4096 + lane * 16;
                    *(f16x8 *)(ew + 2048) = r0;
                    *(f16x8 *)(ew + 3072) = r1;
                }
            } else
            if (gtok >= 0) {
                const float inv = 1.0f / psum;
                half_t *op = a.out + (size_t)gtok * H + hh * 32;
#pragma unroll
                for (int gq = 0; gq < 4; ++gq) {
                    f16x4 ov;
#pragma unroll
                    for (int e = 0; e < 4; ++e) ov[e] = (_Float16)rounded_f32(o[4 * gq + e] * inv);
                    *(f16x4 *)(op + 8 * gq + 4 * hi) = ov;
                }
            }
        };
        const bool fast = FULL || (need == 0xFu && inner == 0xFu);
        asm volatile("s_barrier" ::: "memory");
        asm volatile("s_barrier" ::: "memory");
        using TO0 = std::integral_constant<int, 0>;
        for (int h = 1; h < (CTXREGS ? n_head - 1 : n_head); ++h) {
            if (h < 8) TL_STAMP_AT(tl_sel, 128 + 6 * h);
            if (FULL || fast) attend(h - 1, std::true_type{}, std::true_type{}, h, TO0{});
            else if constexpr (!FULL) attend(h - 1, std::true_type{}, std::false_type{}, h, TO0{});
            if (h < 8) TL_STAMP_AT(tl_sel, 128 + 6 * h + 5);
            asm volatile("s_barrier" ::: "memory");
        }
        if constexpr (CTXREGS) {
            if (n_head - 1 < 8) TL_STAMP_AT(tl_sel, 128 + 6 * (n_head - 1));
            attend(n_head - 2, std::true_type{}, std::true_type{}, n_head - 1, std::integral_constant<int, 1>{});
            if (n_head - 1 < 8) TL_STAMP_AT(tl_sel, 128 + 6 * (n_head - 1) + 5);
            asm volatile("s_barrier" ::: "memory");
        }
        TL_STAMP_AT(tl_sel, 190);
        if constexpr (CTXREGS) {
            char *const xw = smem + blk * (NCF * 1024) + lane * 16;
#pragma unroll
            for (int q = 0; q < NCF - 4; ++q) *(f16x8 *)(xw + q * 1024) = cf[q];
            char *const ew = smem + ctx_edge_offset(NCF) + blk * 4096 + lane * 16;
            *(f16x8 *)ew = pen0;
            *(f16x8 *)(ew + 1024) = pen1;
            asm volatile("s_waitcnt lgkmcnt(0)\n\ts_barrier" ::: "memory");
        }
        if constexpr (CTXREGS) attend(n_head - 1, std::false_type{}, std::true_type{}, 0, std::integral_constant<int, 2>{});
        else if (FULL || fast) attend(n_head - 1, std::false_type{}, std::true_type{}, 0, TO0{});
        else if constexpr (!FULL) attend(n_head - 1, std::false_type{}, std::false_type{}, 0, TO0{});
        TL_STAMP_AT(tl_sel, 192);
        TL_STAMP_AT(tl_sel, 252);
        TL_REALTIME_AT(tl_sel, 253);
    }
}

template <int KT, int GB, int WT>
__global__ __launch_bounds__(512, 2) void qkv_attention2_kernel(Qkv2Args a) {
    extern __shared__ __attribute__((aligned(16))) char smem[];
    qkv_attention2_body<KT, GB, WT>(a, smem, (int)blockIdx.x, (int)threadIdx.x);
}
// ... 111 lines not shown
```

bert.cpp_amd/pybert.py:

```python
from __future__ import annotations

import contextlib
import ctypes as C
import os
import subprocess
from typing import List, Optional, Sequence

import numpy as np

_HERE = os.path.dirname(os.path.abspath(__file__))
LIB_PATH = os.environ.get("BERT_HIP_LIB") or os.path.join(_HERE, "libbert.so")

BERT_H_SYMBOLS = [
    "bert_params_parse", "bert_load_from_file", "bert_free", "bert_encode", "bert_encode_batch", "bert_tokenize",
    "bert_eval", "bert_eval_batch", "bert_n_embd", "bert_n_max_tokens", "bert_vocab_id_to_token",
]
BERT_HIP_H_SYMBOLS = [
    "bert_hip_load_tokenizer", "bert_hip_tokenize_batch", "bert_hip_n_layer", "bert_hip_n_head", "bert_hip_n_intermediate", "bert_hip_n_vocab",
    "bert_hip_ftype", "bert_hip_device", "bert_hip_n_devices", "bert_hip_pooling", "bert_hip_normalize", "bert_hip_encode_batch", "bert_hip_eval_packed", "bert_hip_eval_packed_gather",
    "bert_hip_eval_packed_device", "bert_hip_reserve", "bert_hip_check", "bert_hip_eval_hidden",
    "bert_hip_profile_enable", "bert_hip_profile_report", "bert_hip_set_option", "bert_hip_version",
    "bert_hip_index_create", "bert_hip_index_free", "bert_hip_index_size", "bert_hip_index_reserve", "bert_hip_index_add",
    "bert_hip_index_add_device", "bert_hip_index_add_texts", "bert_hip_index_search", "bert_hip_index_search_device",
    "bert_hip_index_search_texts", "bert_hip_index_remove", "bert_hip_index_n_live", "bert_hip_index_search_filtered",
    "bert_hip_index_search_filtered_device", "bert_hip_index_compact", "bert_hip_index_save", "bert_hip_index_load",
    "bert_hip_index_rescore", "bert_hip_index_rescore_device", "bert_hip_index_search_rescored", "bert_hip_index_search_rescored_device",
    "bert_hip_index_get_rows", "bert_hip_index_partition", "bert_hip_index_n_lists", "bert_hip_index_partition_centroids",
    "bert_hip_index_partition_lists", "bert_hip_index_kmeans", "bert_hip_index_search_probed", "bert_hip_index_search_probed_device",
    "bert_hip_index_search_probed_filtered", "bert_hip_index_search_probed_filtered_device", "bert_hip_index_search_rescored_probed",
    "bert_hip_index_search_rescored_probed_device", "bert_hip_index_partition_save", "bert_hip_index_partition_load",
    "bert_hip_eval_packed_grouped", "bert_hip_eval_packed_grouped_device", "bert_hip_tokenize_long", "bert_hip_plan_windows",
    "bert_hip_encode_long_batch", "bert_hip_index_add_long_texts",
    "bert_hip_eval_packed_tokens_device", "bert_hip_eval_packed_tokens", "bert_hip_encode_tokens_batch", "bert_hip_maxsim_device", "bert_hip_maxsim",
]
BERT_HIP_TEST_H_SYMBOLS = [
    "bert_hip_test_gemm", "bert_hip_test_gemm_lnfold", "bert_hip_test_attention", "bert_hip_test_qkv_attention",
    "bert_hip_test_layer_tail", "bert_hip_test_skinny_tail", "bert_hip_test_skinny_qkv", "bert_hip_test_shard_bounds", "bert_hip_test_build_windows",
    "bert_hip_test_build_windows_device", "bert_hip_test_max_windows", "bert_hip_test_set_window_slots", "bert_hip_test_set_pad",
    "bert_hip_test_dispatch", "bert_hip_test_shard_threads_created", "bert_hip_test_embed_ln", "bert_hip_test_pool_normalize",
    "bert_hip_test_pool", "bert_hip_test_layernorm",
    "bert_hip_test_f32_gemm", "bert_hip_test_f32_attention", "bert_hip_test_f32_layernorm", "bert_hip_test_f32_embed_ln", "bert_hip_test_f32_pool",
    "bert_hip_test_model_digest", "bert_hip_test_pack_weight", "bert_hip_test_parse_devices", "bert_hip_test_gather_runs",
    "bert_hip_test_encode_groups", "bert_hip_test_tokenize_pack", "bert_hip_test_index_header",
    "bert_hip_test_build_lists", "bert_hip_test_partition_header", "bert_hip_test_group_pool", "bert_hip_test_token_rows",
]
TEST_LIB_PATH = LIB_PATH[:-3] + "_test.so"


def build(force: bool = False, jobs: int = 8) -> str:
    args = ["make", "-C", _HERE, f"-j{jobs}", "-s"]
    if force:
        args.append("-B")
    subprocess.check_call(args)
    return LIB_PATH


_lib = None


def _declare_product_abi(L):
    vp, i32, f32p, i32p = C.c_void_p, C.c_int32, C.POINTER(C.c_float), C.POINTER(C.c_int32)
    L.bert_load_from_file.restype = vp; L.bert_load_from_file.argtypes = [C.c_char_p]
    L.bert_hip_load_tokenizer.restype = vp; L.bert_hip_load_tokenizer.argtypes = [C.c_char_p]
    L.bert_free.restype = None; L.bert_free.argtypes = [vp]
    for fn in ("bert_n_embd", "bert_n_max_tokens", "bert_hip_n_layer", "bert_hip_n_head", "bert_hip_n_intermediate",
               "bert_hip_n_vocab", "bert_hip_ftype", "bert_hip_device", "bert_hip_pooling", "bert_hip_normalize"):
        getattr(L, fn).restype = i32; getattr(L, fn).argtypes = [vp]
    L.bert_vocab_id_to_token.restype = C.c_char_p; L.bert_vocab_id_to_token.argtypes = [vp, i32]
    L.bert_tokenize.restype = None; L.bert_tokenize.argtypes = [vp, C.c_char_p, i32p, i32p, i32]
    L.bert_eval.restype = None; L.bert_eval.argtypes = [vp, i32, i32p, i32, f32p]
    L.bert_eval_batch.restype = None
    L.bert_eval_batch.argtypes = [vp, i32, i32, C.POINTER(i32p), i32p, C.POINTER(f32p)]
    L.bert_encode.restype = None; L.bert_encode.argtypes = [vp, i32, C.c_char_p, f32p]
    L.bert_encode_batch.restype = None
    L.bert_encode_batch.argtypes = [vp, i32, i32, i32, C.POINTER(C.c_char_p), C.POINTER(f32p)]
    L.bert_hip_eval_packed.restype = i32; L.bert_hip_eval_packed.argtypes = [vp, i32p, i32p, i32, f32p]
    L.bert_hip_eval_packed_device.restype = i32
    L.bert_hip_eval_packed_device.argtypes = [vp, vp, vp, i32, i32, i32, vp, vp]
    L.bert_hip_eval_hidden.restype = i32; L.bert_hip_eval_hidden.argtypes = [vp, i32p, i32, f32p, f32p]
    L.bert_hip_profile_enable.restype = None; L.bert_hip_profile_enable.argtypes = [vp, i32]
    L.bert_hip_profile_report.restype = i32; L.bert_hip_profile_report.argtypes = [vp, C.c_char_p, i32]
    L.bert_hip_set_option.restype = None; L.bert_hip_set_option.argtypes = [vp, C.c_char_p, C.c_char_p]
    L.bert_hip_n_devices.restype = i32; L.bert_hip_n_devices.argtypes = [vp]
    L.bert_hip_encode_batch.restype = i32
    L.bert_hip_encode_batch.argtypes = [vp, i32, i32, C.POINTER(C.c_char_p), C.POINTER(f32p)]
    L.bert_hip_eval_packed_gather.restype = i32
    L.bert_hip_eval_packed_gather.argtypes = [vp, i32p, i32p, i32, C.POINTER(vp)]
    L.bert_hip_reserve.restype = i32; L.bert_hip_reserve.argtypes = [vp, i32, i32]
    L.bert_hip_check.restype = i32; L.bert_hip_check.argtypes = [vp]
    L.bert_hip_tokenize_batch.restype = i32
    L.bert_hip_tokenize_batch.argtypes = [vp, i32, i32, C.POINTER(C.c_char_p), i32p, i32p]
    L.bert_hip_version.restype = C.c_char_p
    L.bert_hip_index_create.restype = vp; L.bert_hip_index_create.argtypes = [vp, i32, i32]
    L.bert_hip_index_free.restype = None; L.bert_hip_index_free.argtypes = [vp]
    L.bert_hip_index_size.restype = i32; L.bert_hip_index_size.argtypes = [vp]
    L.bert_hip_index_reserve.restype = i32; L.bert_hip_index_reserve.argtypes = [vp, i32, i32, i32]
    L.bert_hip_index_add.restype = i32; L.bert_hip_index_add.argtypes = [vp, i32, f32p]
    L.bert_hip_index_add_device.restype = i32; L.bert_hip_index_add_device.argtypes = [vp, i32, vp, vp]
    L.bert_hip_index_add_texts.restype = i32; L.bert_hip_index_add_texts.argtypes = [vp, i32, i32, C.POINTER(C.c_char_p)]
    L.bert_hip_index_search.restype = i32; L.bert_hip_index_search.argtypes = [vp, i32, f32p, i32, i32p, f32p]
    L.bert_hip_index_search_device.restype = i32; L.bert_hip_index_search_device.argtypes = [vp, i32, vp, i32, vp, vp, vp]
    L.bert_hip_index_search_texts.restype = i32
    L.bert_hip_index_search_texts.argtypes = [vp, i32, i32, C.POINTER(C.c_char_p), i32, i32p, f32p]
    L.bert_hip_index_remove.restype = i32; L.bert_hip_index_remove.argtypes = [vp, i32, i32p]
    L.bert_hip_index_n_live.restype = i32; L.bert_hip_index_n_live.argtypes = [vp]
    L.bert_hip_index_search_filtered.restype = i32; L.bert_hip_index_search_filtered.argtypes = [vp, i32, f32p, i32, vp, i32, i32p, f32p]
    L.bert_hip_index_search_filtered_device.restype = i32
    L.bert_hip_index_search_filtered_device.argtypes = [vp, i32, vp, i32, vp, i32, vp, vp, vp]
    L.bert_hip_index_compact.restype = i32; L.bert_hip_index_compact.argtypes = [vp, i32p]
    L.bert_hip_index_save.restype = i32; L.bert_hip_index_save.argtypes = [vp, C.c_char_p]
    L.bert_hip_index_load.restype = vp; L.bert_hip_index_load.argtypes = [vp, C.c_char_p]
    L.bert_hip_index_rescore.restype = i32; L.bert_hip_index_rescore.argtypes = [vp, i32, f32p, i32, i32p, i32, i32p, f32p]
    L.bert_hip_index_rescore_device.restype = i32; L.bert_hip_index_rescore_device.argtypes = [vp, i32, vp, i32, vp, i32, vp, vp, vp]
    L.bert_hip_index_search_rescored.restype = i32; L.bert_hip_index_search_rescored.argtypes = [vp, vp, i32, f32p, i32, i32, i32p, f32p]
    L.bert_hip_index_search_rescored_device.restype = i32
    L.bert_hip_index_search_rescored_device.argtypes = [vp, vp, i32, vp, i32, i32, vp, vp, vp]
    L.bert_hip_index_get_rows.restype = i32; L.bert_hip_index_get_rows.argtypes = [vp, i32, i32p, f32p]
    L.bert_hip_index_partition.restype = i32; L.bert_hip_index_partition.argtypes = [vp, i32, f32p]
    L.bert_hip_index_n_lists.restype = i32; L.bert_hip_index_n_lists.argtypes = [vp]
    L.bert_hip_index_partition_centroids.restype = i32; L.bert_hip_index_partition_centroids.argtypes = [vp, f32p]
    L.bert_hip_index_partition_lists.restype = i32; L.bert_hip_index_partition_lists.argtypes = [vp, i32p]
    L.bert_hip_index_kmeans.restype = i32; L.bert_hip_index_kmeans.argtypes = [vp, i32, i32, f32p]
    L.bert_hip_index_search_probed.restype = i32; L.bert_hip_index_search_probed.argtypes = [vp, i32, f32p, i32, i32, i32p, f32p]
    L.bert_hip_index_search_probed_device.restype = i32; L.bert_hip_index_search_probed_device.argtypes = [vp, i32, vp, i32, i32, vp, vp, vp]
    L.bert_hip_index_search_probed_filtered.restype = i32
    L.bert_hip_index_search_probed_filtered.argtypes = [vp, i32, f32p, i32, i32, vp, i32, i32p, f32p]
    L.bert_hip_index_search_probed_filtered_device.restype = i32
    L.bert_hip_index_search_probed_filtered_device.argtypes = [vp, i32, vp, i32, i32, vp, i32, vp, vp, vp]
    L.bert_hip_index_search_rescored_probed.restype = i32
    L.bert_hip_index_search_rescored_probed.argtypes = [vp, vp, i32, f32p, i32, i32, i32, vp, i32, i32p, f32p]
    L.bert_hip_index_search_rescored_probed_device.restype = i32
    L.bert_hip_index_search_rescored_probed_device.argtypes = [vp, vp, i32, vp, i32, i32, i32, vp, i32, vp, vp, vp]
    L.bert_hip_index_partition_save.restype = i32; L.bert_hip_index_partition_save.argtypes = [vp, C.c_char_p]
    L.bert_hip_index_partition_load.restype = i32; L.bert_hip_index_partition_load.argtypes = [vp, C.c_char_p]
    L.bert_hip_eval_packed_grouped.restype = i32; L.bert_hip_eval_packed_grouped.argtypes = [vp, i32p, i32p, i32, i32p, i32, f32p]
    L.bert_hip_eval_packed_grouped_device.restype = i32
    L.bert_hip_eval_packed_grouped_device.argtypes = [vp, vp, vp, i32, i32, i32, vp, i32, vp, vp]
    L.bert_hip_tokenize_long.restype = i32; L.bert_hip_tokenize_long.argtypes = [vp, C.c_char_p, i32p, i32]
    L.bert_hip_plan_windows.restype = i32; L.bert_hip_plan_windows.argtypes = [i32, i32, i32, i32p, i32]
    L.bert_hip_encode_long_batch.restype = i32
    L.bert_hip_encode_long_batch.argtypes = [vp, i32, i32, C.POINTER(C.c_char_p), i32, i32, C.POINTER(f32p), i32p]
    L.bert_hip_index_add_long_texts.restype = i32; L.bert_hip_index_add_long_texts.argtypes = [vp, i32, i32, C.POINTER(C.c_char_p), i32, i32]
    L.bert_hip_eval_packed_tokens_device.restype = i32
    L.bert_hip_eval_packed_tokens_device.argtypes = [vp, vp, vp, i32, i32, i32, i32, vp, vp, vp]
    L.bert_hip_eval_packed_tokens.restype = i32; L.bert_hip_eval_packed_tokens.argtypes = [vp, i32p, i32p, i32, i32, f32p, f32p]
    L.bert_hip_encode_tokens_batch.restype = C.c_int64
    L.bert_hip_encode_tokens_batch.argtypes = [vp, i32, i32, C.POINTER(C.c_char_p), i32, i32p, f32p, C.c_int64]
    L.bert_hip_maxsim_device.restype = i32; L.bert_hip_maxsim_device.argtypes = [vp, vp, vp, i32, vp, vp, i32, i32, vp, i32, i32, vp, vp]
    L.bert_hip_maxsim.restype = i32; L.bert_hip_maxsim.argtypes = [vp, f32p, i32p, i32, f32p, i32p, i32, i32, i32p, i32, i32, f32p]


def lib() -> C.CDLL:
    global _lib
    if _lib is not None:
        return _lib
    if not os.path.exists(LIB_PATH):
        raise RuntimeError(f"{LIB_PATH} not found: build the HIP extension first "
                           f"(python -c 'import __graft_entry__ as g; g.build()' or make -C bert.cpp_amd)")
    L = C.CDLL(LIB_PATH)
    _declare_product_abi(L)
    _lib = L
    return L


_test_lib = None


def test_lib() -> C.CDLL:
    global _test_lib
    if _test_lib is not None:
        return _test_lib
    if not os.path.exists(TEST_LIB_PATH):
        raise RuntimeError(f"{TEST_LIB_PATH} not found: build it first (make -C bert.cpp_amd)")
    L = C.CDLL(TEST_LIB_PATH)
    _declare_product_abi(L)
    vp, i32, i32p = C.c_void_p, C.c_int32, C.POINTER(C.c_int32)
    L.bert_hip_test_gemm.restype = i32
    L.bert_hip_test_gemm.argtypes = [i32, i32, i32, vp, vp, i32, vp, vp, i32, i32, vp]
    L.bert_hip_test_gemm_lnfold.restype = i32
    L.bert_hip_test_gemm_lnfold.argtypes = [i32, i32, i32, i32] + [vp] * 10 + [i32, vp, vp, vp]
    L.bert_hip_test_attention.restype = i32
    L.bert_hip_test_attention.argtypes = [i32, i32p, i32, i32, vp, i32, vp]
    L.bert_hip_test_qkv_attention.restype = i32
    L.bert_hip_test_qkv_attention.argtypes = [i32, i32p, i32, i32, vp, vp, i32, vp, i32, vp]
    L.bert_hip_test_layer_tail.restype = i32
    L.bert_hip_test_layer_tail.argtypes = [i32, i32, i32, vp, vp, vp, vp, vp, i32, vp, vp, vp, vp, vp, vp, vp, i32, vp]
    L.bert_hip_test_skinny_tail.restype = i32
    L.bert_hip_test_skinny_tail.argtypes = [i32, i32, i32, vp, vp, vp, vp, vp, i32, vp, vp, vp, vp, vp, vp, vp, C.c_uint32, vp, vp, vp, vp, vp]
    L.bert_hip_test_skinny_qkv.restype = i32
    L.bert_hip_test_skinny_qkv.argtypes = [i32, i32, vp, vp, vp, vp, vp, i32, vp, C.c_uint32, vp, vp]
    L.bert_hip_test_embed_ln.restype = i32
    L.bert_hip_test_embed_ln.argtypes = [i32, i32, i32, i32, vp, vp, vp, vp, vp, i32p, i32p, i32, i32, vp]
    L.bert_hip_test_layernorm.restype = i32
    L.bert_hip_test_layernorm.argtypes = [i32, i32, vp, vp, vp, vp]
    L.bert_hip_test_pool_normalize.restype = i32
    L.bert_hip_test_pool_normalize.argtypes = [i32, vp, i32p, i32, i32, vp, i32p]
    L.bert_hip_test_pool.restype = i32
    L.bert_hip_test_pool.argtypes = [i32, vp, i32p, i32, i32, i32, i32, vp, i32p]
    L.bert_hip_test_f32_gemm.restype = i32
    L.bert_hip_test_f32_gemm.argtypes = [i32, i32, i32, vp, vp, vp, vp, i32, vp]
    L.bert_hip_test_f32_attention.restype = i32
    L.bert_hip_test_f32_attention.argtypes = [i32, i32p, i32, i32, i32, vp, vp]
    L.bert_hip_test_f32_layernorm.restype = i32
    L.bert_hip_test_f32_layernorm.argtypes = [i32, i32, vp, vp, vp, vp]
    L.bert_hip_test_f32_embed_ln.restype = i32
    L.bert_hip_test_f32_embed_ln.argtypes = [i32, i32, i32, vp, vp, vp, vp, vp, i32p, i32p, i32, i32, vp]
    L.bert_hip_test_f32_pool.restype = i32
    L.bert_hip_test_f32_pool.argtypes = [i32, vp, i32p, i32, i32, i32, i32, vp, i32p]
    L.bert_hip_test_model_digest.restype = i32
    L.bert_hip_test_model_digest.argtypes = [C.c_char_p, i32p, C.POINTER(C.c_uint64)]
    L.bert_hip_test_pack_weight.restype = i32
    L.bert_hip_test_pack_weight.argtypes = [vp, i32, i32, i32, i32, vp, vp, vp, vp, C.c_int64]
    L.bert_hip_test_shard_bounds.restype = None
    L.bert_hip_test_shard_bounds.argtypes = [i32p, i32, i32, i32p]
    L.bert_hip_test_build_windows.restype = i32
    L.bert_hip_test_build_windows.argtypes = [i32p, i32, i32p]
    L.bert_hip_test_max_windows.restype = i32
    L.bert_hip_test_max_windows.argtypes = [i32, i32]
    L.bert_hip_test_set_window_slots.restype = i32
    L.bert_hip_test_set_window_slots.argtypes = [i32]
    L.bert_hip_test_set_pad.restype = None
    L.bert_hip_test_set_pad.argtypes = [C.c_uint32, C.c_uint32]
    L.bert_hip_test_build_windows_device.restype = i32
    L.bert_hip_test_build_windows_device.argtypes = [i32p, i32, i32p]
    L.bert_hip_test_shard_threads_created.restype = C.c_int64
    L.bert_hip_test_shard_threads_created.argtypes = []
    L.bert_hip_test_dispatch.restype = i32
    L.bert_hip_test_dispatch.argtypes = [i32p, i32p, i32, i32, i32, C.POINTER(C.c_float)]
    L.bert_hip_test_parse_devices.restype = i32
    L.bert_hip_test_parse_devices.argtypes = [C.c_char_p, i32, i32, i32p, C.c_char_p, i32]
    L.bert_hip_test_gather_runs.restype = i32
    L.bert_hip_test_gather_runs.argtypes = [i32p, i32, C.c_int64, i32p]
    L.bert_hip_test_encode_groups.restype = i32
    L.bert_hip_test_encode_groups.argtypes = [i32, i32p, i32]
    L.bert_hip_test_tokenize_pack.restype = i32
    L.bert_hip_test_tokenize_pack.argtypes = [vp, i32, i32, C.POINTER(C.c_char_p), i32p, i32p, i32p, i32p, i32]
    L.bert_hip_test_index_header.restype = i32
    L.bert_hip_test_index_header.argtypes = [C.c_char_p, i32, C.c_int64, C.POINTER(C.c_uint32), C.c_char_p, i32]
    L.bert_hip_test_partition_header.restype = i32
    L.bert_hip_test_partition_header.argtypes = [C.c_char_p, i32, C.c_int64, C.POINTER(C.c_uint32), C.c_char_p, i32]
    L.bert_hip_test_build_lists.restype = i32
    L.bert_hip_test_build_lists.argtypes = [i32p, i32, i32, i32p, i32p]
    L.bert_hip_test_group_pool.restype = i32
    L.bert_hip_test_group_pool.argtypes = [vp, i32, i32p, i32p, i32, i32, i32, vp, i32p]
    L.bert_hip_test_token_rows.restype = i32
    L.bert_hip_test_token_rows.argtypes = [vp, i32, i32, i32, i32p, i32, i32, i32, vp]
    _test_lib = L
    return L


def test_embed_ln(table_type: int, word_bytes, type_bytes, pos_bytes, H: int, gamma, beta, tokens, cu_seqlens, max_len: int = 0) -> np.ndarray:
    wb, tb, pb = (np.ascontiguousarray(a) for a in (word_bytes, type_bytes, pos_bytes))
    rb = {0: 4 * H, 1: 2 * H, 2: H // 32 * 18, 3: H // 32 * 20}[table_type]
    g = np.ascontiguousarray(gamma, dtype=np.float32); b = np.ascontiguousarray(beta, dtype=np.float32)
    toks = np.ascontiguousarray(tokens, dtype=np.int32); cu = np.ascontiguousarray(cu_seqlens, dtype=np.int32)
    assert len(toks) == int(cu[-1]) and tb.nbytes == 2 * rb and g.shape == (H,) and b.shape == (H,)
    out = np.zeros((len(toks), H), dtype=np.float16)
    r = test_lib().bert_hip_test_embed_ln(table_type, H, wb.nbytes // rb, pb.nbytes // rb, wb.ctypes.data, tb.ctypes.data, pb.ctypes.data,
                                          g.ctypes.data, b.ctypes.data, _i32p(toks), _i32p(cu), len(cu) - 1, max_len, out.ctypes.data)
    if r != 0:
        raise RuntimeError(f"bert_hip_test_embed_ln failed: {r}")
    return out


def test_layernorm(x: np.ndarray, gamma, beta) -> np.ndarray:
    x = np.ascontiguousarray(x, dtype=np.float16)
    g = np.ascontiguousarray(gamma, dtype=np.float32); b = np.ascontiguousarray(beta, dtype=np.float32)
    assert g.shape == (x.shape[1],) and b.shape == (x.shape[1],)
    out = np.zeros_like(x)
    r = test_lib().bert_hip_test_layernorm(x.shape[0], x.shape[1], x.ctypes.data, g.ctypes.data, b.ctypes.data, out.ctypes.data)
    if r != 0:
        raise RuntimeError(f"bert_hip_test_layernorm failed: {r}")
    return out


def test_pool_normalize(x: np.ndarray, cu_seqlens, max_len: int):
    x = np.ascontiguousarray(x, dtype=np.float16); cu = np.ascontiguousarray(cu_seqlens, dtype=np.int32)
    out = np.zeros((len(cu) - 1, x.shape[1]), dtype=np.float32)
    st = np.zeros(1, dtype=np.int32)
    r = test_lib().bert_hip_test_pool_normalize(x.shape[1], x.ctypes.data, _i32p(cu), len(cu) - 1, max_len, out.ctypes.data, _i32p(st))
    if r != 0:
        raise RuntimeError(f"bert_hip_test_pool_normalize failed: {r}")
    return out, int(st[0])


def test_pool(x: np.ndarray, cu_seqlens, max_len: int, pooling: str = "mean", normalize: bool = True):
    x = np.ascontiguousarray(x, dtype=np.float16); cu = np.ascontiguousarray(cu_seqlens, dtype=np.int32)
    out = np.zeros((len(cu) - 1, x.shape[1]), dtype=np.float32)
    st = np.zeros(1, dtype=np.int32)
    r = test_lib().bert_hip_test_pool(x.shape[1], x.ctypes.data, _i32p(cu), len(cu) - 1, max_len, {"mean": 0, "cls": 1}[pooling],
                                      int(bool(normalize)), out.ctypes.data, _i32p(st))
    if r != 0:
        raise RuntimeError(f"bert_hip_test_pool failed: {r}")
    return out, int(st[0])


def test_group_pool(rows: np.ndarray, weights, group_cu, raw: bool, out: Optional[np.ndarray] = None):
    rows = np.ascontiguousarray(rows, dtype=np.float32); g = np.ascontiguousarray(group_cu, dtype=np.int32)
    w = None if weights is None else np.ascontiguousarray(weights, dtype=np.int32)
    assert rows.ndim == 2 and (w is None or w.shape == (rows.shape[0],))
    if out is None:
        out = np.full((len(g) - 1, rows.shape[1]), np.nan, dtype=np.float32)
    assert out.dtype == np.float32 and out.flags.c_contiguous and out.shape == (len(g) - 1, rows.shape[1])
    st = np.zeros(1, dtype=np.int32)
    r = test_lib().bert_hip_test_group_pool(rows.ctypes.data, rows.shape[0], None if w is None else _i32p(w), _i32p(g), len(g) - 1, rows.shape[1],
                                            int(bool(raw)), out.ctypes.data, _i32p(st))
    if r != 0:
        raise RuntimeError(f"bert_hip_test_group_pool failed: {r}")
    return out, int(st[0])


def test_token_rows(x: np.ndarray, cu_seqlens, max_len: int, normalize: bool = True, f16_out: bool = False) -> np.ndarray:
    assert x.dtype in (np.float16, np.float32) and x.ndim == 2
    x = np.ascontiguousarray(x); cu = np.ascontiguousarray(cu_seqlens, dtype=np.int32)
    out = np.zeros(x.shape, dtype=np.float16 if f16_out else np.float32)
    r = test_lib().bert_hip_test_token_rows(x.ctypes.data, int(x.dtype == np.float32), x.shape[0], x.shape[1], _i32p(cu), len(cu) - 1, max_len,
                                            int(bool(normalize)) | 2 * int(bool(f16_out)), out.ctypes.data)
    if r != 0:
        raise RuntimeError(f"bert_hip_test_token_rows failed: {r}")
    return out


def plan_windows(n_tokens: int, window: int, stride: int) -> List[int]:
    n = lib().bert_hip_plan_windows(n_tokens, window, stride, None, 0)
    if n < 0:
        raise ValueError(f"bert_hip_plan_windows({n_tokens}, {window}, {stride}) = {n}")
    starts = np.zeros(n, dtype=np.int32)
    assert lib().bert_hip_plan_windows(n_tokens, window, stride, _i32p(starts), n) == n
    return starts.tolist()


def model_digest(path: str):
    leg = C.c_int32(0)
    dig = C.c_uint64(0)
    n = test_lib().bert_hip_test_model_digest(path.encode(), C.byref(leg), C.byref(dig))
    if n < 0:
        raise RuntimeError("model file rejected (see stderr)")
    return n, bool(leg.value), int(dig.value)


PACK_FORMS = {"f16": 0, "f16_kperm": 1, "q4_nibbles": 2, "q4_scales": 3, "ln_fold": 4, "ln_fold_stats": 5, "gamma_beta_bias": 6, "table_f32": 7}


def pack_weight(W, wtype: int, N: int, K: int, form: str, gamma=None, beta=None, bias=None, stack3: bool = False) -> np.ndarray:
    Wb = np.ascontiguousarray(W)
    f32 = [None if a is None else np.ascontiguousarray(a, dtype=np.float32) for a in (gamma, beta, bias)]
    out = np.zeros((N + 127) // 128 * 128 * max(K, 16) * 4, dtype=np.uint8)
    n = test_lib().bert_hip_test_pack_weight(Wb.ctypes.data, wtype, N, K, PACK_FORMS[form] | (0x100 if stack3 else 0),
                                             *(None if a is None else a.ctypes.data for a in f32), out.ctypes.data, out.nbytes)
    if n < 0:
        raise RuntimeError(f"bert_hip_test_pack_weight failed: {n}")
    return out[:n].copy()


def shard_bounds(cu_seqlens: np.ndarray, n_shards: int) -> List[int]:
    cu = np.ascontiguousarray(cu_seqlens, dtype=np.int32)
    out = np.zeros(n_shards + 1, dtype=np.int32)
    test_lib().bert_hip_test_shard_bounds(_i32p(cu), len(cu) - 1, n_shards, _i32p(out))
    return out.tolist()


def build_windows(cu_seqlens: np.ndarray, device: bool = False) -> List[tuple]:
    cu = np.ascontiguousarray(cu_seqlens, dtype=np.int32)
    out = np.zeros(2 * max(len(cu) - 1, 1), dtype=np.int32)
    f = test_lib().bert_hip_test_build_windows_device if device else test_lib().bert_hip_test_build_windows
    n = f(_i32p(cu), len(cu) - 1, _i32p(out))
    if n < 0:
        raise RuntimeError("bert_hip_test_build_windows_device failed")
    return [(int(out[2 * i]), int(out[2 * i + 1])) for i in range(n)]


def set_window_slots(slots: int) -> int:
    return int(test_lib().bert_hip_test_set_window_slots(slots))


@contextlib.contextmanager
def test_pad(pattern16: int, pattern32: int):
    L = test_lib()
    L.bert_hip_test_set_pad(pattern16, pattern32)
    try:
        yield
    finally:
        L.bert_hip_test_set_pad(0, 0)


def max_windows(n_sentences: int, n_tokens: int) -> int:
    return int(test_lib().bert_hip_test_max_windows(n_sentences, n_tokens))


def dispatch_stub(tokens: np.ndarray, cu_seqlens: np.ndarray, n_shards: int, H: int = 4, throw: bool = False) -> np.ndarray:
    tokens = np.ascontiguousarray(tokens, dtype=np.int32)
    cu = np.ascontiguousarray(cu_seqlens, dtype=np.int32)
    out = np.full((len(cu) - 1, abs(H)), np.nan, dtype=np.float32)
    r = test_lib().bert_hip_test_dispatch(_i32p(tokens), _i32p(cu), len(cu) - 1, n_shards, -H if throw else H, _f32p(out))
    if r != 0:
        raise RuntimeError(f"bert_hip_test_dispatch failed: {r}")
    return out


def shard_threads_created() -> int:
    return int(test_lib().bert_hip_test_shard_threads_created())


def parse_devices(spec: Optional[bytes], n_devices: int, current: int = 0):
    devs = np.zeros(max(n_devices, 1), dtype=np.int32)
    err = C.create_string_buffer(512)
    n = test_lib().bert_hip_test_parse_devices(spec, n_devices, current, _i32p(devs), err, len(err))
    return (None, err.value.decode()) if n < 0 else (devs[:n].tolist(), None)


def gather_runs(cu_seqlens: np.ndarray, tokens_per_run: int) -> List[int]:
    cu = np.ascontiguousarray(cu_seqlens, dtype=np.int32)
    out = np.zeros(len(cu), dtype=np.int32)
    n = test_lib().bert_hip_test_gather_runs(_i32p(cu), len(cu) - 1, tokens_per_run, _i32p(out))
    return out[:n].tolist()


def encode_groups(n_inputs: int) -> List[int]:
    out = np.zeros(1024, dtype=np.int32)
    n = test_lib().bert_hip_test_encode_groups(n_inputs, _i32p(out), len(out))
    assert n <= len(out)
    return out[:n].tolist()


def tokenize_pack(model: "BertModel", texts: Sequence[bytes], n_threads: int, counts=None):
    n, N = len(texts), model.n_max_tokens
    arr = (C.c_char_p * n)(*texts)
    cnt = np.zeros(n, dtype=np.int32)
    cu = np.full(n + 1, -1, dtype=np.int32)
    packed = np.full(n * N, -1, dtype=np.int32)
    given = None if counts is None else np.ascontiguousarray(counts, dtype=np.int32)
    n_ok = test_lib().bert_hip_test_tokenize_pack(model.ctx, n_threads, n, arr, None if given is None else _i32p(given), _i32p(cnt),
                                                  _i32p(cu), _i32p(packed), len(packed))
    if n_ok < 0:
        raise RuntimeError("bert_hip_test_tokenize_pack failed")
    return n_ok, cnt.tolist(), cu[:n_ok + 1].tolist(), packed[:cu[n_ok]].tolist()


def _f32p(a: np.ndarray):
    return a.ctypes.data_as(C.POINTER(C.c_float))


def _i32p(a: np.ndarray):
    return a.ctypes.data_as(C.POINTER(C.c_int32))


class BertModel:

    def __init__(self, fname: str, tokenizer_only: bool = False, test_routes: bool = False):
        self.lib = test_lib() if test_routes else lib()
        load = self.lib.bert_hip_load_tokenizer if tokenizer_only else self.lib.bert_load_from_file
        self.ctx = load(fname.encode("utf-8"))
        if not self.ctx:
            raise RuntimeError(f"bert_load_from_file('{fname}') failed (see stderr)")
        self.n_embd = self.lib.bert_n_embd(self.ctx)
        self.n_max_tokens = self.lib.bert_n_max_tokens(self.ctx)
        self.n_layer = self.lib.bert_hip_n_layer(self.ctx)
        self.n_vocab = self.lib.bert_hip_n_vocab(self.ctx)

    def close(self):
        if getattr(self, "ctx", None):
            self.lib.bert_free(self.ctx)
            self.ctx = None

    def __del__(self):
        try:
            self.close()
        except Exception:
            pass

    def tokenize(self, text: str | bytes, n_max_tokens: Optional[int] = None) -> List[int]:
        n_max = n_max_tokens or self.n_max_tokens
        buf = (C.c_int32 * max(n_max, 2))()
        n = C.c_int32(0)
        data = text if isinstance(text, bytes) else text.encode("utf-8")
        self.lib.bert_tokenize(self.ctx, data, buf, C.byref(n), n_max)
        return list(buf[: n.value])

    def tokenize_batch(self, texts: Sequence[str | bytes], n_threads: int = 6) -> List[List[int]]:
        n, N = len(texts), self.n_max_tokens
        arr = (C.c_char_p * n)(*[t if isinstance(t, bytes) else t.encode("utf-8") for t in texts])
        toks = np.zeros((n, N), dtype=np.int32)
        cnt = np.zeros(n, dtype=np.int32)
        if self.lib.bert_hip_tokenize_batch(self.ctx, n_threads, n, arr, _i32p(toks), _i32p(cnt)) != 0:
            raise RuntimeError("bert_hip_tokenize_batch failed")
        return [toks[i, : cnt[i]].tolist() for i in range(n)]

    def id_to_token(self, i: int) -> bytes:
        return self.lib.bert_vocab_id_to_token(self.ctx, i)

    def eval(self, tokens: Sequence[int], n_threads: int = 6) -> np.ndarray:
        toks = np.ascontiguousarray(tokens, dtype=np.int32)
        out = np.full(self.n_embd, np.nan, dtype=np.float32)
        self.lib.bert_eval(self.ctx, n_threads, _i32p(toks), len(toks), _f32p(out))
        return out

    def eval_batch(self, sentences: Sequence[Sequence[int]], n_threads: int = 6, scattered: bool = False) -> np.ndarray:
        B = len(sentences)
        arrs = [np.ascontiguousarray(s, dtype=np.int32) for s in sentences]
        wide = np.full((B, 2 * self.n_embd + 3 if scattered else self.n_embd), np.nan, dtype=np.float32)
        out = wide[:, : self.n_embd]
        tok_ptrs = (C.POINTER(C.c_int32) * B)(*[_i32p(a) for a in arrs])
        lens = np.array([len(a) for a in arrs], dtype=np.int32)
        out_ptrs = (C.POINTER(C.c_float) * B)(*[C.cast(wide[i].ctypes.data, C.POINTER(C.c_float)) for i in range(B)])
        self.lib.bert_eval_batch(self.ctx, n_threads, B, tok_ptrs, _i32p(lens), out_ptrs)
        if scattered:
            assert np.isnan(wide[:, self.n_embd:]).all()
        return np.ascontiguousarray(out)

    def encode(self, text: str, n_threads: int = 6) -> np.ndarray:
        out = np.full(self.n_embd, np.nan, dtype=np.float32)
        self.lib.bert_encode(self.ctx, n_threads, text.encode("utf-8"), _f32p(out))
        return out

    def encode_batch(self, texts: Sequence[str], n_threads: int = 6, batch_size: int = 16) -> np.ndarray:
        n = len(texts)
        out = np.full((n, self.n_embd), np.nan, dtype=np.float32)
        out_ptrs = (C.POINTER(C.c_float) * n)(*[_f32p(out[i]) for i in range(n)])
        txt = (C.c_char_p * n)(*[t.encode("utf-8") for t in texts])
        self.lib.bert_encode_batch(self.ctx, n_threads, batch_size, n, txt, out_ptrs)
        return out

    def eval_packed(self, tokens: np.ndarray, cu_seqlens: np.ndarray, out: Optional[np.ndarray] = None) -> np.ndarray:
        tokens = np.ascontiguousarray(tokens, dtype=np.int32)
        cu = np.ascontiguousarray(cu_seqlens, dtype=np.int32)
        B = len(cu) - 1
        if out is None:
            out = np.full((B, self.n_embd), np.nan, dtype=np.float32)
        assert out.dtype == np.float32 and out.flags.c_contiguous and out.shape == (B, self.n_embd)
        r = self.lib.bert_hip_eval_packed(self.ctx, _i32p(tokens), _i32p(cu), B, _f32p(out))
        if r != 0:
            raise RuntimeError(f"bert_hip_eval_packed failed: {r}")
        return out

    def n_devices(self) -> int:
        return self.lib.bert_hip_n_devices(self.ctx)

    def tokenize_long(self, text: str | bytes) -> List[int]:
        data = text if isinstance(text, bytes) else text.encode("utf-8")
        n = self.lib.bert_hip_tokenize_long(self.ctx, data, None, 0)
        if n < 0:
            raise RuntimeError(f"bert_hip_tokenize_long failed: {n}")
        ids = np.zeros(n, dtype=np.int32)
        assert self.lib.bert_hip_tokenize_long(self.ctx, data, _i32p(ids), n) == n
        return ids.tolist()

    def plan_windows(self, n_tokens: int, window: Optional[int] = None, stride: Optional[int] = None) -> List[int]:
        window, stride = self.long_defaults(window, stride)
        return plan_windows(n_tokens, window, stride)

    def long_defaults(self, window: Optional[int] = None, stride: Optional[int] = None):
        if window is None:
            window = min(self.n_max_tokens, 128)
        if stride is None:
            stride = max(1, 3 * (window - 2) // 4)
        return int(window), int(stride)

    def eval_packed_grouped(self, tokens: np.ndarray, cu_seqlens: np.ndarray, group_cu: np.ndarray, out: Optional[np.ndarray] = None) -> np.ndarray:
        tokens = np.ascontiguousarray(tokens, dtype=np.int32)
        cu = np.ascontiguousarray(cu_seqlens, dtype=np.int32)
        g = np.ascontiguousarray(group_cu, dtype=np.int32)
        if out is None:
            out = np.full((len(g) - 1, self.n_embd), np.nan, dtype=np.float32)
        assert out.dtype == np.float32 and out.flags.c_contiguous and out.shape == (len(g) - 1, self.n_embd)
        r = self.lib.bert_hip_eval_packed_grouped(self.ctx, _i32p(tokens), _i32p(cu), len(cu) - 1, _i32p(g), len(g) - 1, _f32p(out))
# ... 614 lines not shown
```

Baseline: 346,400 sentences/s.

## Emit embedding LayerNorm output directly in MFMA lane order for one-launch model

Adds an embed+LayerNorm kernel that writes its output in the lane-ordered residual layout used by the fused one-launch model kernel. The first layer's attention phase then loads operand fragments straight from that buffer, and the tail no longer has to reorder row-major x into lane order on layer 0. This removes the in-kernel relayout on the first layer and simplifies the B-fragment LDS reads. The cost is a new kernel and new shape constraints, and one-launch is now disabled when those constraints are not met.

New measurement: 350,100 sentences/s, median of 6. 1.01x the previous value.

```diff
diff --git a/bert.cpp_amd/csrc/engine.h b/bert.cpp_amd/csrc/engine.h
--- a/bert.cpp_amd/csrc/engine.h
+++ b/bert.cpp_amd/csrc/engine.h
@@ -76,6 +76,7 @@
         Route route = Route::LAYERED;
         bool build_windows = false;
         const int *n_windows_dev = nullptr;
+        bool embed_lanes = false;
         std::vector<LayerPlan> layers;
     };
     Plan plan(const int32_t *d_tokens, const int32_t *d_cu, int B, int T, int max_len, float *d_out, hipStream_t s, float *d_hidden,
diff --git a/bert.cpp_amd/csrc/engine.hip b/bert.cpp_amd/csrc/engine.hip
--- a/bert.cpp_amd/csrc/engine.hip
+++ b/bert.cpp_amd/csrc/engine.hip
@@ -137,8 +137,13 @@
     if (p.route == Route::F32) ok = forward_f32(p, err);
     else {
         const int H = hp_.n_embd;
-        timed("embed_ln", 0.0, s, [&] { launch_embed_ln(w_->word_emb.p, w_->type_emb.p, w_->pos_emb.p, w_->table_type, w_->ln_e_w.as<float>(), w_->ln_e_b.as<float>(),
-                                                        d_tokens, d_cu, B, T, H, hp_.n_vocab, max_len, x_.as<half_t>(), s); });
+        if (p.embed_lanes)
+            timed("embed_ln", 0.0, s, [&] { ok = launch_embed_ln_lanes(w_->word_emb.p, w_->type_emb.p, w_->pos_emb.p, w_->table_type, w_->ln_e_w.as<float>(), w_->ln_e_b.as<float>(),
+                                                                       d_tokens, d_cu, B, T, H, hp_.n_vocab, max_len, y_.as<half_t>(), s); });
+        else
+            timed("embed_ln", 0.0, s, [&] { launch_embed_ln(w_->word_emb.p, w_->type_emb.p, w_->pos_emb.p, w_->table_type, w_->ln_e_w.as<float>(), w_->ln_e_b.as<float>(),
+                                                            d_tokens, d_cu, B, T, H, hp_.n_vocab, max_len, x_.as<half_t>(), s); });
+        if (!ok) { err = "embed_ln: no lane-order kernel for this shape"; return -1; }
         tap(p, 0);
         if (p.build_windows)
             timed("build_windows", 0.0, s, [&] { launch_build_windows(d_cu, B, windows_.as<int2>(), status_.as<int>() + 1, slots, s); });
@@ -188,6 +193,7 @@
     const bool fused_windows = p.layers[0].qkv2, latency_call = opt_.latency && T <= opt_.latency_tokens;
     one_launch = one_launch && fused_windows && opt_.one_launch && opt_.tail && !latency_call;
     const bool full_windows = (long long)B * 128 == T;
+    if (full_windows && !embed_ln_lanes_supported(w_->table_type, H, T, max_len)) one_launch = false;
     const int spw = qkv_attention2_sentences_per_window(max_len, slots);
     if (!d_windows && fused_windows &&
         (4ll * ((B + spw - 1) / spw) * 128 > 5 * ((long long)T + (long long)(slots / 2) * B) || (one_launch && opt_.one_launch == 2 && spw > 1 && !full_windows))) {
@@ -202,6 +208,7 @@
     const bool skinny = latency_call && opt_.tail && opt_.qkv2 && !opt_.gemm_naive && !opt_.attn_naive && max_len <= 128 && (dh == 32 || dh == 64) &&
                         skinny_layer_supported(L0.qkv.w, L0.o.w, L0.ffi.w, L0.ffo.w) && qkv2_shape0;
     p.route = skinny ? Route::LATENCY : one_launch && one_launch_pays ? Route::ONE_LAUNCH : fold ? Route::FOLDED : Route::LAYERED;
+    p.embed_lanes = p.route == Route::ONE_LAUNCH && full_windows;
     return p;
 }
 
diff --git a/bert.cpp_amd/csrc/kernels.h b/bert.cpp_amd/csrc/kernels.h
--- a/bert.cpp_amd/csrc/kernels.h
+++ b/bert.cpp_amd/csrc/kernels.h
@@ -71,6 +71,10 @@
 void launch_embed_ln(const void *word, const void *type, const void *pos, int table_type, const float *gamma,
                      const float *beta, const int32_t *tokens, const int32_t *cu_seqlens, int n_sentences, int T,
                      int H, int n_vocab, int max_len, half_t *out, hipStream_t stream);
+bool embed_ln_lanes_supported(int table_type, int H, int T, int max_len);
+bool launch_embed_ln_lanes(const void *word, const void *type, const void *pos, int table_type, const float *gamma,
+                           const float *beta, const int32_t *tokens, const int32_t *cu_seqlens, int n_sentences, int T,
+                           int H, int n_vocab, int max_len, half_t *xres, hipStream_t stream);
 
 void launch_layernorm(half_t *x, const float *gamma, const float *beta, int T, int H, hipStream_t stream);
 
diff --git a/bert.cpp_amd/csrc/layer_tail.hip b/bert.cpp_amd/csrc/layer_tail.hip
--- a/bert.cpp_amd/csrc/layer_tail.hip
+++ b/bert.cpp_amd/csrc/layer_tail.hip
@@ -84,7 +84,7 @@
 template <int NT, int WT, bool RAGGED, bool HANDOVER, bool CTXREGS = false, bool XRES_IN = false, bool XRES_OUT = false>
 __device__ __forceinline__ void layer_tail_body(const TailArgs &a, char *smem, const int tok0, const int rows, const int tid,
                                                 [[maybe_unused]] f16x8 (&xnext)[8 * NT], [[maybe_unused]] const f16x8 *cf = nullptr,
-                                                [[maybe_unused]] half_t *xres = nullptr, const bool lane_in = false, const bool lane_out = false) {
+                                                [[maybe_unused]] half_t *xres = nullptr, const bool lane_out = false) {
     static_assert(!(HANDOVER && RAGGED), "a ragged window's rows are packed: its lanes are not the window phase's slots");
     static_assert(!(CTXREGS && RAGGED), "a ragged window's rows are packed: its lanes are not the attention waves' queries");
     static_assert(!((XRES_IN || XRES_OUT) && (RAGGED || WT != GW_F16)), "lane order: full windows (a pair owns its 32 rows), f16 weights");
@@ -137,20 +137,6 @@
     if constexpr (XRES_IN) {
         char *const xb = (char *)(xres + (size_t)tok_w * H);
         const unsigned xl = (unsigned)lane * 16u;
-        if (!lane_in) {
-            const half_t *xr = a.x + (size_t)row_l * H + role * 64 + 4 * hi;
-#pragma unroll
-            for (int b = 0; b < NBH; ++b)
-#pragma unroll
-                for (int s = 0; s < 2; ++s) {
-                    const f16x4 lo = *(const f16x4 *)(xr + (b >> 1) * 128 + (b & 1) * 32 + 16 * s), up = *(const f16x4 *)(xr + (b >> 1) * 128 + (b & 1) * 32 + 16 * s + 8);
-                    f16x8 v;
-#pragma unroll
-                    for (int e = 0; e < 4; ++e) { v[e] = lo[e]; v[4 + e] = up[e]; }
-                    *(f16x8 *)(xb + (2 * (4 * (b >> 1) + 2 * role + (b & 1)) + s) * 1024 + xl) = v;
-                }
-            asm volatile("s_waitcnt vmcnt(0)" ::: "memory");
-        }
 #pragma unroll
         for (int b = 0; b < NBH; ++b)
 #pragma unroll
@@ -294,12 +280,18 @@
     __builtin_amdgcn_s_waitcnt(0xc07f);
     static_for<P>([&](auto p_tag) __attribute__((always_inline)) {
         constexpr int p = decltype(p_tag)::value, n3 = p / NT, q = p % NT, p2 = p + 2;
-        const unsigned bA = aR + (unsigned)(slot * LT_TILE + role * 8192), bB = bA + 3 * LT_TILE;
+        constexpr int OB = XRES_IN ? 3 * LT_TILE : 0;
+        const unsigned bA = aR + (unsigned)(slot * LT_TILE + role * 8192), bB = bA + (3 * LT_TILE - OB);
         f16x8 Fa[4], Fb[4];
         auto rd = [&](unsigned base, int g2, f16x8 (&F)[4]) __attribute__((always_inline)) {
             const unsigned a0 = base ^ (unsigned)((2 * g2) << 5), a1 = base ^ (unsigned)((2 * g2 + 1) << 5);
             F[0] = frag_read<0>(a0); F[1] = frag_read<4096>(a0);
             F[2] = frag_read<0>(a1); F[3] = frag_read<4096>(a1);
+        };
+        auto rdB = [&](int g2, f16x8 (&F)[4]) __attribute__((always_inline)) {
+            const unsigned a0 = bB ^ (unsigned)((2 * g2) << 5), a1 = bB ^ (unsigned)((2 * g2 + 1) << 5);
+            F[0] = frag_read<OB>(a0); F[1] = frag_read<OB + 4096>(a0);
+            F[2] = frag_read<OB>(a1); F[3] = frag_read<OB + 4096>(a1);
         };
         auto mm = [&](f16x8 (&F)[4], int ks) __attribute__((always_inline)) {
             accp[n3 * 2 + 0] = mfma16(F[0], bf[ks], accp[n3 * 2 + 0]);
@@ -341,7 +333,7 @@
             bf[NQ - 4] = lds_read_b128<true, 0>(aEdge);
             bf[NQ - 3] = lds_read_b128<true, 1024>(aEdge);
         }
-        rd(bB, 0, Fa);
+        rdB(0, Fa);
         wait_frags<4>(Fb);
         if constexpr (CTX_LATE && q == NT - 1) { landed(bf[NQ - 4]); landed(bf[NQ - 3]); }
         mm(Fb, 8 * q + 2);
@@ -350,7 +342,7 @@
             bf[NQ - 2] = lds_read_b128<true, 2048>(aEdge);
             bf[NQ - 1] = lds_read_b128<true, 3072>(aEdge);
         }
-        rd(bB, 1, Fb);
+        rdB(1, Fb);
         if constexpr (Q4) { q4_turn(); __builtin_amdgcn_sched_barrier(0); }
         wait_frags<4 + QW>(Fa);
         mm(Fa, 8 * q + 4);
diff --git a/bert.cpp_amd/csrc/misc_kernels.hip b/bert.cpp_amd/csrc/misc_kernels.hip
--- a/bert.cpp_amd/csrc/misc_kernels.hip
+++ b/bert.cpp_amd/csrc/misc_kernels.hip
@@ -209,6 +209,88 @@
 #undef EMB
 }
 
+template <int TT, int NT>
+__global__ __launch_bounds__(512) void embed_ln_lanes_kernel(const void *word, const void *type, const void *pos,
+                                                             const float *__restrict__ gamma, const float *__restrict__ beta,
+                                                             const int32_t *__restrict__ tokens,
+                                                             const int32_t *__restrict__ cu_seqlens, int n_sentences, int H,
+                                                             int n_vocab, int max_len, half_t *__restrict__ xres) {
+    constexpr int NQ = 8 * NT, FS = 1024 + 16;
+    __shared__ __attribute__((aligned(16))) char S[NQ * FS];
+    const int lane = threadIdx.x & 63, wave = __builtin_amdgcn_readfirstlane(threadIdx.x >> 6);
+    const int tok0 = blockIdx.x * 32, b = tok0 >> 7;
+    const bool whole = b < n_sentences && cu_seqlens[b] == 128 * b && cu_seqlens[b + 1] == 128 * b + 128;
+#pragma unroll
+    for (int i = 0; i < 4; ++i) {
+        const int l31 = wave * 4 + i, t = tok0 + l31;
+        int p = t & 127;
+        if (!whole) {
+            int lo = 0, hi = n_sentences;
+            while (hi - lo > 1) {
+                const int mid = (lo + hi) >> 1;
+                if (cu_seqlens[mid] <= t) lo = mid; else hi = mid;
+            }
+            p = t - cu_seqlens[lo];
+        }
+        p = min(p, max_len - 1);
+        int id = tokens[t];
+        id = id < 0 ? 0 : (id >= n_vocab ? n_vocab - 1 : id);
+        const int e0 = 8 * lane;
+        float v[8];
+        float sum = 0.f;
+#pragma unroll
+        for (int k = 0; k < 8; ++k) v[k] = 0.f;
+        if (e0 < H) {
+            float w[8], ty[8], ps[8];
+            table_run8<TT>(word, H, id, e0, w);
+            table_run8<TT>(type, H, 0, e0, ty);
+            table_run8<TT>(pos, H, p, e0, ps);
+#pragma unroll
+            for (int k = 0; k < 8; ++k) { v[k] = ps[k] + (ty[k] + w[k]); sum += v[k]; }
+        }
+        const float mean = wave_sum_f32(sum) / H;
+        float sq = 0.f;
+        if (e0 < H)
+#pragma unroll
+            for (int k = 0; k < 8; ++k) { v[k] -= mean; sq += v[k] * v[k]; }
+        const float rstd = 1.0f / sqrtf(wave_sum_f32(sq) / H + 1e-5f);
+        if (e0 < H) {
+            const float4 g0 = *(const float4 *)(gamma + e0), g1 = *(const float4 *)(gamma + e0 + 4);
+            const float4 b0 = *(const float4 *)(beta + e0), b1 = *(const float4 *)(beta + e0 + 4);
+            const float gg[8] = {g0.x, g0.y, g0.z, g0.w, g1.x, g1.y, g1.z, g1.w};
+            const float bb[8] = {b0.x, b0.y, b0.z, b0.w, b1.x, b1.y, b1.z, b1.w};
+            f16x8 o;
+#pragma unroll
+            for (int k = 0; k < 8; ++k) o[k] = (_Float16)(gg[k] * (v[k] * rstd) + bb[k]);
+            char *const d = S + (lane >> 1) * FS + 8 * (lane & 1) + 16 * l31;
+            *(f16x4 *)d = f16x4{o[0], o[1], o[2], o[3]};
+            *(f16x4 *)(d + 16 * 32) = f16x4{o[4], o[5], o[6], o[7]};
+        }
+    }
+    __syncthreads();
+    char *const out = (char *)(xres + (size_t)tok0 * H);
+#pragma unroll
+    for (int q = wave; q < NQ; q += 8) *(f16x8 *)(out + q * 1024 + lane * 16) = *(const f16x8 *)(S + q * FS + lane * 16);
+}
+
+bool embed_ln_lanes_supported(int table_type, int H, int T, int max_len) {
+    return T > 0 && T % 128 == 0 && (H == 256 || H == 384) && table_type >= 0 && table_type <= 3 && max_len > 0;
+}
+
+bool launch_embed_ln_lanes(const void *word, const void *type, const void *pos, int table_type, const float *gamma,
+                           const float *beta, const int32_t *tokens, const int32_t *cu_seqlens, int n_sentences, int T,
+                           int H, int n_vocab, int max_len, half_t *xres, hipStream_t stream) {
+    if (!embed_ln_lanes_supported(table_type, H, T, max_len) || n_sentences <= 0) return false;
+#define EMBL(TT) do { \
+        if (H == 256) BERT_LAUNCH((embed_ln_lanes_kernel<TT, 2>), dim3(T / 32), dim3(512), 0, stream, word, type, pos, gamma, beta, tokens, \
+                                  cu_seqlens, n_sentences, H, n_vocab, max_len, xres); \
+        else BERT_LAUNCH((embed_ln_lanes_kernel<TT, 3>), dim3(T / 32), dim3(512), 0, stream, word, type, pos, gamma, beta, tokens, \
+                         cu_seqlens, n_sentences, H, n_vocab, max_len, xres); } while (0)
+    if (table_type == 0) EMBL(0); else if (table_type == 1) EMBL(1); else if (table_type == 2) EMBL(2); else EMBL(3);
+#undef EMBL
+    return true;
+}
+
 template <int NJ>
 __global__ __launch_bounds__(256) void layernorm_kernel(half_t *x, const float *gamma, const float *beta, int T, int H) {
     const int t = blockIdx.x * 4 + (threadIdx.x >> 6), lane = threadIdx.x & 63;
diff --git a/bert.cpp_amd/csrc/model_kernel.hip b/bert.cpp_amd/csrc/model_kernel.hip
--- a/bert.cpp_amd/csrc/model_kernel.hip
+++ b/bert.cpp_amd/csrc/model_kernel.hip
@@ -59,22 +59,22 @@
     };
     MK_STAMP(0);
     const int n_layer = rows > 0 ? m.n_layer : 0;
-    auto window_phase = [&](const ModelLayerArgs &L, auto xregs_tag, const f16x8 *xf, f16x8 *cf) __attribute__((always_inline)) {
+    auto window_phase = [&](const ModelLayerArgs &L, auto first_tag, const f16x8 *xf, f16x8 *cf) __attribute__((always_inline)) {
         const int tid = thread_id();
         Qkv2Args q;
         q.x = m.x; q.w = L.wqkv; q.qs = nullptr; q.sc = nullptr; q.bias = L.bqkv; q.cu = m.cu; q.groups = RAGGED ? m.groups : nullptr; q.n_groups = nullptr;
         q.out = m.ctx; q.n_head = m.n_head; q.n_sent = m.n_sent; q.spw = 1; q.slot_mask = m.slot_mask;
-        qkv_attention2_body<2 * NT, NT, GW_F16, !RAGGED, decltype(xregs_tag)::value, !RAGGED>(q, smem, window, tid, xf, cf);
-    };
-    auto tail_phase = [&](const ModelLayerArgs &L, f16x8 (&xf)[8 * NT], const f16x8 *cf, [[maybe_unused]] const bool lane_in,
-                          [[maybe_unused]] const bool lane_out) __attribute__((always_inline)) {
+        constexpr bool FIRST = decltype(first_tag)::value;
+        qkv_attention2_body<2 * NT, NT, GW_F16, !RAGGED, !RAGGED, !RAGGED, !RAGGED && FIRST>(q, smem, window, tid, xf, cf, RAGGED ? nullptr : m.xres);
+    };
+    auto tail_phase = [&](const ModelLayerArgs &L, f16x8 (&xf)[8 * NT], const f16x8 *cf, [[maybe_unused]] const bool lane_out) __attribute__((always_inline)) {
         const int tid = thread_id();
         TailArgs t;
         t.ctx = m.ctx; t.x = m.x; t.wo = L.wo; t.w1p = L.w1p; t.w2p = L.w2p;
         t.wo_qs = t.w1_qs = t.w2_qs = nullptr; t.wo_sc = t.w1_sc = t.w2_sc = nullptr;
         t.bo = L.bo; t.g1 = L.g1; t.be1 = L.be1; t.b1 = L.b1; t.b2 = L.b2; t.g2 = L.g2; t.be2 = L.be2; t.out = m.x; t.I = m.I;
         if constexpr (RAGGED) layer_tail_body<NT, GW_F16, true, false, false>(t, smem, tok0, rows, tid, xf, cf);
-        else layer_tail_body<NT, GW_F16, false, true, true, true, true>(t, smem, tok0, rows, tid, xf, cf, m.xres, lane_in, lane_out);
+        else layer_tail_body<NT, GW_F16, false, true, true, true, true>(t, smem, tok0, rows, tid, xf, cf, m.xres, lane_out);
     };
     auto hand_over = [&]() __attribute__((always_inline)) {
         __builtin_amdgcn_fence(__ATOMIC_RELEASE, "workgroup");
@@ -87,21 +87,21 @@
             window_phase(m.layer[l], std::false_type{}, nullptr, nullptr);
             hand_over();
             MK_STAMP(1 + 2 * l);
-            tail_phase(m.layer[l], none, nullptr, false, false);
+            tail_phase(m.layer[l], none, nullptr, false);
             hand_over();
             MK_STAMP(2 + 2 * l);
         }
     } else {
         f16x8 cf[8 * NT];
-        if (n_layer > 0) window_phase(m.layer[0], std::false_type{}, nullptr, cf);
+        if (n_layer > 0) window_phase(m.layer[0], std::true_type{}, nullptr, cf);
         for (int l = 0; l < n_layer; ++l) {
             hand_over();
             MK_STAMP(1 + 2 * l);
             f16x8 xf[8 * NT];
-            tail_phase(m.layer[l], xf, cf, l > 0, l + 1 < n_layer);
+            tail_phase(m.layer[l], xf, cf, l + 1 < n_layer);
             hand_over();
             MK_STAMP(2 + 2 * l);
-            if (l + 1 < n_layer) window_phase(m.layer[l + 1], std::true_type{}, xf, cf);
+            if (l + 1 < n_layer) window_phase(m.layer[l + 1], std::false_type{}, xf, cf);
             else {
 #pragma unroll
                 for (int q = 0; q < 8 * NT; ++q) asm volatile("" : "=v"(cf[q]));
diff --git a/bert.cpp_amd/csrc/qkv_attention2.hip b/bert.cpp_amd/csrc/qkv_attention2.hip
--- a/bert.cpp_amd/csrc/qkv_attention2.hip
+++ b/bert.cpp_amd/csrc/qkv_attention2.hip
@@ -52,11 +52,13 @@
 
 }
 
-template <int KT, int GB, int WT, bool FULL = false, bool XREGS = false, bool CTXREGS = false>
+template <int KT, int GB, int WT, bool FULL = false, bool XREGS = false, bool CTXREGS = false, bool XLANES = false>
 __device__ __forceinline__ void qkv_attention2_body(const Qkv2Args &a, char *smem, const int window, const int tid,
                                                     [[maybe_unused]] const f16x8 *xf = nullptr,
-                                                    [[maybe_unused]] f16x8 *cf = nullptr) {
+                                                    [[maybe_unused]] f16x8 *cf = nullptr,
+                                                    [[maybe_unused]] const half_t *xlanes = nullptr) {
     static_assert(FULL || !XREGS, "fragments handed over in registers: full windows only");
+    static_assert(XREGS || !XLANES, "lane order in: the register form's body, full windows only");
     static_assert(!CTXREGS || (FULL && WT == GW_F16), "the context in registers: full windows, f16 weights");
     constexpr int NCF = 4 * KT;
     constexpr bool Q4 = WT != GW_F16;
@@ -125,7 +127,13 @@
 
     if (wave >= 4) {
         f16x8 bf[4 * KT];
-        if constexpr (XREGS) {
+        if constexpr (XLANES) {
+            const char *const xb = (const char *)(xlanes + ((size_t)window * Q2_WIN + blk * 32) * H);
+            const unsigned xl = (unsigned)lane * 16u;
+#pragma unroll
+            for (int ks = 0; ks < 4 * KT; ++ks)
+                asm volatile("global_load_dwordx4 %0, %1, %2 offset:%3" : "=v"(bf[ks]) : "v"(xl), "s"(xb + (ks >> 2) * 4096), "n"((ks & 3) * 1024));
+        } else if constexpr (XREGS) {
 #pragma unroll
             for (int ks = 0; ks < 4 * KT; ++ks) bf[ks] = xf[ks];
         } else {
@@ -202,6 +210,10 @@
         asm volatile("s_waitcnt vmcnt(%0) lgkmcnt(0)\n\ts_barrier" : : "n"(Q4 ? 0 : PPS) : "memory");
 #pragma unroll
         for (int ks = 0; ks < 4 * KT; ++ks) asm volatile("" : "+v"(bf[ks]));
+        if constexpr (XLANES) {
+#pragma unroll
+            for (int ks = 0; ks < 4 * KT; ++ks) bf[ks] = result_to_operand_fragment(bf[ks]);
+        }
         if constexpr (Q4) {
 #pragma unroll
             for (int i = 0; i < NRAW; ++i) q4_request(min(1, n_head - 1), 0, i);
diff --git a/bert.cpp_amd/pybert.py b/bert.cpp_amd/pybert.py
--- a/bert.cpp_amd/pybert.py
+++ b/bert.cpp_amd/pybert.py
@@ -37,7 +37,7 @@
     "bert_hip_test_gemm", "bert_hip_test_gemm_lnfold", "bert_hip_test_attention", "bert_hip_test_qkv_attention",
     "bert_hip_test_layer_tail", "bert_hip_test_skinny_tail", "bert_hip_test_skinny_qkv", "bert_hip_test_shard_bounds", "bert_hip_test_build_windows",
     "bert_hip_test_build_windows_device", "bert_hip_test_max_windows", "bert_hip_test_set_window_slots", "bert_hip_test_set_pad",
-    "bert_hip_test_dispatch", "bert_hip_test_shard_threads_created", "bert_hip_test_embed_ln", "bert_hip_test_pool_normalize",
+    "bert_hip_test_dispatch", "bert_hip_test_shard_threads_created", "bert_hip_test_embed_ln", "bert_hip_test_embed_ln_lanes", "bert_hip_test_pool_normalize",
     "bert_hip_test_pool", "bert_hip_test_layernorm",
     "bert_hip_test_f32_gemm", "bert_hip_test_f32_attention", "bert_hip_test_f32_layernorm", "bert_hip_test_f32_embed_ln", "bert_hip_test_f32_pool",
     "bert_hip_test_model_digest", "bert_hip_test_pack_weight", "bert_hip_test_parse_devices", "bert_hip_test_gather_runs",
@@ -191,6 +191,8 @@
     L.bert_hip_test_skinny_qkv.argtypes = [i32, i32, vp, vp, vp, vp, vp, i32, vp, C.c_uint32, vp, vp]
     L.bert_hip_test_embed_ln.restype = i32
     L.bert_hip_test_embed_ln.argtypes = [i32, i32, i32, i32, vp, vp, vp, vp, vp, i32p, i32p, i32, i32, vp]
+    L.bert_hip_test_embed_ln_lanes.restype = i32
+    L.bert_hip_test_embed_ln_lanes.argtypes = L.bert_hip_test_embed_ln.argtypes
     L.bert_hip_test_layernorm.restype = i32
     L.bert_hip_test_layernorm.argtypes = [i32, i32, vp, vp, vp, vp]
     L.bert_hip_test_pool_normalize.restype = i32
@@ -249,18 +251,25 @@
     return L
 
 
-def test_embed_ln(table_type: int, word_bytes, type_bytes, pos_bytes, H: int, gamma, beta, tokens, cu_seqlens, max_len: int = 0) -> np.ndarray:
+def test_embed_ln(table_type: int, word_bytes, type_bytes, pos_bytes, H: int, gamma, beta, tokens, cu_seqlens, max_len: int = 0, lanes: bool = False) -> np.ndarray:
     wb, tb, pb = (np.ascontiguousarray(a) for a in (word_bytes, type_bytes, pos_bytes))
     rb = {0: 4 * H, 1: 2 * H, 2: H // 32 * 18, 3: H // 32 * 20}[table_type]
     g = np.ascontiguousarray(gamma, dtype=np.float32); b = np.ascontiguousarray(beta, dtype=np.float32)
     toks = np.ascontiguousarray(tokens, dtype=np.int32); cu = np.ascontiguousarray(cu_seqlens, dtype=np.int32)
     assert len(toks) == int(cu[-1]) and tb.nbytes == 2 * rb and g.shape == (H,) and b.shape == (H,)
     out = np.zeros((len(toks), H), dtype=np.float16)
-    r = test_lib().bert_hip_test_embed_ln(table_type, H, wb.nbytes // rb, pb.nbytes // rb, wb.ctypes.data, tb.ctypes.data, pb.ctypes.data,
-                                          g.ctypes.data, b.ctypes.data, _i32p(toks), _i32p(cu), len(cu) - 1, max_len, out.ctypes.data)
-    if r != 0:
-        raise RuntimeError(f"bert_hip_test_embed_ln failed: {r}")
+    entry = getattr(test_lib(), "bert_hip_test_embed_ln_lanes" if lanes else "bert_hip_test_embed_ln")
+    r = entry(table_type, H, wb.nbytes // rb, pb.nbytes // rb, wb.ctypes.data, tb.ctypes.data, pb.ctypes.data,
+              g.ctypes.data, b.ctypes.data, _i32p(toks), _i32p(cu), len(cu) - 1, max_len, out.ctypes.data)
+    if lanes and r == -2:
+        return None
+    if r != 0:
+        raise RuntimeError(f"bert_hip_test_embed_ln{'_lanes' if lanes else ''} failed: {r}")
     return out
+
+
+def test_embed_ln_lanes(table_type: int, word_bytes, type_bytes, pos_bytes, H: int, gamma, beta, tokens, cu_seqlens, max_len: int = 0):
+    return test_embed_ln(table_type, word_bytes, type_bytes, pos_bytes, H, gamma, beta, tokens, cu_seqlens, max_len, lanes=True)
 
 
 def test_layernorm(x: np.ndarray, gamma, beta) -> np.ndarray:
```
